# dwu4/fhe-si

Measured on AMD Instinct MI355X. Metric: homomorphic ciphertext-mults/sec (incl. relinearize) at n=2^14, logQ=512, higher is better.
Workload: dtype u32 (every transformed row is a row of 4-byte residues modulo a prime below 2^30: tensor half over primes of 30 bits, key switch over four of 30; coefficients are u64 limbs)

## Files before the change

fhe-si_amd/binding.py:

```python
from __future__ import annotations

import ctypes as C
import os
import subprocess
import sys

import numpy as np

_DIR = os.path.dirname(os.path.abspath(__file__))
_CSRC = os.path.join(_DIR, "csrc")
_SO = os.environ.get("FHESI_LIB") or os.path.join(_CSRC, "libfhesi_hip.so")

OP_ADD, OP_SUB, OP_MUL, OP_DIV, OP_SET = 0, 1, 2, 3, 4

ABI_SYMBOLS = [
    "fhesi_last_error", "fhesi_device_count", "fhesi_ctx_create", "fhesi_ctx_destroy", "fhesi_ctx_m", "fhesi_ctx_phim",
    "fhesi_ctx_nprimes", "fhesi_ctx_prime", "fhesi_ctx_zms_idx", "fhesi_ctx_phi_m", "fhesi_ctx_sync", "fhesi_ctx_stream",
    "fhesi_timer_start", "fhesi_timer_stop", "fhesi_cmod_fft", "fhesi_cmod_ifft", "fhesi_dcrt_alloc", "fhesi_dcrt_free",
    "fhesi_dcrt_copy", "fhesi_dcrt_index_set", "fhesi_dcrt_equal", "fhesi_dcrt_upload_row", "fhesi_dcrt_download_row",
    "fhesi_dcrt_device_ptr", "fhesi_dcrt_from_poly", "fhesi_dcrt_to_poly", "fhesi_dcrt_op", "fhesi_dcrt_op_scalar",
    "fhesi_dcrt_automorph", "fhesi_dcrt_add_primes", "fhesi_dcrt_remove_primes", "fhesi_dcrt_from_scrt", "fhesi_dcrt_to_scrt",
    "fhesi_rows_ntt_fwd_dev", "fhesi_rows_ntt_inv_dev", "fhesi_rows_op_dev", "fhesi_ksk_create", "fhesi_ksk_free",
    "fhesi_ksk_upload", "fhesi_ksk_device_ptr", "fhesi_ksk_bytes", "fhesi_ct_mul_relin_batch", "fhesi_ct_mul_relin_batch_dev",
    "fhesi_ct_mul_dev", "fhesi_apply_key_switch_dev", "fhesi_dev_alloc", "fhesi_dev_free", "fhesi_dev_upload", "fhesi_dev_download",
    "fhesi_dev_copy", "fhesi_prof_enable", "fhesi_prof_read",
    "fhesi_ct_add_dev", "fhesi_ct_mul_long_dev", "fhesi_rows_mul_long_dev", "fhesi_ct_automorph_dev", "fhesi_ct_automorph_key_switch_dev",
    "fhesi_ct_gather_dev", "fhesi_ct_mul_sum_relin_dev", "fhesi_encrypt_batch", "fhesi_decrypt_batch", "fhesi_dcrt_exp", "fhesi_selftest_aux32",
    "fhesi_ctx_set_option", "fhesi_ctx_get_option", "fhesi_ctx_copy_options", "fhesi_host_alloc", "fhesi_host_free", "fhesi_ksk_key_bits", "fhesi_prof_kernel_name", "fhesi_ksk_mark_dirty", "fhesi_ksk_upload_dev",
    "fhesi_dcrt_add_primes_and_scale", "fhesi_dcrt_scale_down_to_set",
    "fhesi_keyswitch_init_batch", "fhesi_ksk_download", "fhesi_comm_init_all", "fhesi_comm_from_rccl", "fhesi_comm_destroy", "fhesi_comm_rank",
    "fhesi_comm_size", "fhesi_ksk_broadcast", "fhesi_comm_broadcast_dev", "fhesi_comm_exchange", "fhesi_comm_exchange_begin", "fhesi_comm_exchange_end", "fhesi_comm_allreduce_rows", "fhesi_scrt_alloc", "fhesi_scrt_from_poly", "fhesi_scrt_to_poly", "fhesi_scrt_op_scalar", "fhesi_dcrt_assign_scrt", "fhesi_scrt_assign_dcrt",
    "fhesi_ksk_form", "fhesi_ct_add_const_dev", "fhesi_ct_mul_poly_dev",
    "fhesi_encrypt_batch_seeded", "fhesi_keyswitch_init_batch_seeded", "fhesi_dcrt_sample",
    "fhesi_abi_version", "fhesi_host_stage_release",
    "fhesi_slots_plan", "fhesi_slots_create", "fhesi_slots_free", "fhesi_slots_info", "fhesi_slots_exponents", "fhesi_slots_embed", "fhesi_slots_decode",
    "fhesi_slots_embed_dev", "fhesi_slots_decode_dev", "fhesi_encrypt_slots_batch_seeded", "fhesi_decrypt_slots_batch", "fhesi_encrypt_noise_batch_seeded",
    "fhesi_slots_plan_pow2", "fhesi_slots_create_pow2", "fhesi_slots_shape", "fhesi_slots_set_path",
]
ABI_VERSION = 7
PROF_CLASSES = {"ntt_fwd": 0, "ntt_inv": 1, "rns_reduce": 2, "tensor": 3, "crt": 4, "digits": 5, "dot": 6, "ew": 7, "ntt_fwd_digits_main": 8}


class FhesiError(RuntimeError):
    pass


def library_path() -> str:
    return _SO


def build_library(force: bool = False) -> str:
    srcs = [os.path.join(_CSRC, f) for f in os.listdir(_CSRC) if f.endswith((".hip", ".cpp", ".h", ".inc"))]
    srcs.append(os.path.join(os.path.dirname(_DIR), "include", "fhesi_hip.h"))
    stale = force or not os.path.exists(_SO) or any(os.path.getmtime(s) > os.path.getmtime(_SO) for s in srcs)
    if stale:
        subprocess.check_call(["make", "-C", _CSRC, "-j8"], stdout=subprocess.DEVNULL)
    return _SO


_lib = None
_vp, _i32, _i64, _u64 = C.c_void_p, C.c_int32, C.c_int64, C.c_uint64


def _load():
    global _lib
    if _lib is not None:
        return _lib
    if not os.path.exists(_SO):
        raise FhesiError(f"HIP extension not built: {_SO} is missing (run __graft_entry__.build())")
    if "torch" not in sys.modules and not os.environ.get("FHESI_NO_TORCH_PRELOAD"):
        try:
            import torch
        except Exception:
            pass
    lib = C.CDLL(_SO)
    lib.fhesi_last_error.restype = C.c_char_p
    have = lib.fhesi_abi_version() if hasattr(lib, "fhesi_abi_version") else None
    if have != ABI_VERSION:
        raise FhesiError(f"{_SO} has ABI revision {have}, this binding was written against {ABI_VERSION}: rebuild (make -C fhe-si_amd/csrc)")
    sig = {
        "fhesi_device_count": [_vp],
        "fhesi_ctx_create": [_vp, _i64, _i32, _vp, _vp, _i32],
        "fhesi_ctx_destroy": [_vp],
        "fhesi_ctx_prime": [_vp, _i32, _vp, _vp],
        "fhesi_ctx_zms_idx": [_vp, _vp],
        "fhesi_ctx_phi_m": [_vp, _vp],
        "fhesi_ctx_sync": [_vp],
        "fhesi_timer_start": [_vp],
        "fhesi_timer_stop": [_vp, _vp],
        "fhesi_cmod_fft": [_vp, _i32, _vp, _i32, _i64, _vp],
        "fhesi_cmod_ifft": [_vp, _i32, _vp, _vp],
        "fhesi_dcrt_alloc": [_vp, _vp, _i32, _vp],
        "fhesi_dcrt_free": [_vp],
        "fhesi_dcrt_copy": [_vp, _vp],
        "fhesi_dcrt_index_set": [_vp, _vp, _vp],
        "fhesi_dcrt_equal": [_vp, _vp, _vp],
        "fhesi_dcrt_upload_row": [_vp, _i32, _vp],
        "fhesi_dcrt_download_row": [_vp, _i32, _vp],
        "fhesi_dcrt_from_poly": [_vp, _vp, _i32, _i64],
        "fhesi_dcrt_to_poly": [_vp, _vp, _i32, _i32, _vp, _i32],
        "fhesi_dcrt_op": [_vp, _vp, _i32],
        "fhesi_dcrt_op_scalar": [_vp, _vp, _i32, _i32],
        "fhesi_dcrt_automorph": [_vp, _i64],
        "fhesi_dcrt_exp": [_vp, _i64],
        "fhesi_selftest_aux32": [_vp],
        "fhesi_dcrt_add_primes": [_vp, _vp, _i32],
        "fhesi_dcrt_remove_primes": [_vp, _vp, _i32],
        "fhesi_dcrt_from_scrt": [_vp, _vp],
        "fhesi_dcrt_to_scrt": [_vp, _vp],
        "fhesi_rows_ntt_fwd_dev": [_vp, _vp, _i64],
        "fhesi_rows_ntt_inv_dev": [_vp, _vp, _i64],
        "fhesi_rows_op_dev": [_vp, _vp, _vp, _i64, _i32],
        "fhesi_ksk_create": [_vp, _i32, _i32, _vp],
        "fhesi_ksk_free": [_vp],
        "fhesi_ksk_upload": [_vp, _vp],
        "fhesi_ct_mul_relin_batch": [_vp, _vp, _i32, _u64, _i32, _vp, _vp, _vp, _i32, _i64],
        "fhesi_ct_mul_relin_batch_dev": [_vp, _vp, _i32, _u64, _i32, _vp, _vp, _vp, _i32, _i64],
        "fhesi_ct_mul_dev": [_vp, _u64, _vp, _vp, _i32, _i64, _vp],
        "fhesi_apply_key_switch_dev": [_vp, _vp, _i32, _i32, _vp, _i64, _vp, _i32],
        "fhesi_ct_add_dev": [_vp, _i32, _vp, _vp, _i32, _i32, _i64],
        "fhesi_ct_mul_long_dev": [_vp, _i32, _vp, _i64, _i32, _i32, _i64],
        "fhesi_rows_mul_long_dev": [_vp, _vp, _i64, _i64],
        "fhesi_ct_automorph_dev": [_vp, _i64, _vp, _i32, _i32, _i64, _vp, _i32],
        "fhesi_ct_automorph_key_switch_dev": [_vp, _vp, _i32, _i32, _i64, _vp, _i32, _i64, _vp, _i32],
        "fhesi_ct_gather_dev": [_vp, _vp, _vp, _i64, _i64, _vp],
        "fhesi_ct_mul_sum_relin_dev": [_vp, _vp, _i32, _u64, _i32, _vp, _i32, _vp, _vp, _vp, _i64, _vp],
        "fhesi_encrypt_batch": [_vp, _vp, _vp, _i32, _u64, _vp, _vp, _i64, _vp, _i32],
        "fhesi_decrypt_batch": [_vp, _vp, _i32, _u64, _vp, _i32, _i64, _vp],
        "fhesi_dev_alloc": [_vp, C.c_size_t, _vp],
        "fhesi_dev_free": [_vp, _vp],
        "fhesi_dev_upload": [_vp, _vp, _vp, C.c_size_t],
        "fhesi_dev_download": [_vp, _vp, _vp, C.c_size_t],
        "fhesi_dev_copy": [_vp, _vp, _vp, C.c_size_t],
        "fhesi_prof_enable": [_vp, _i32],
        "fhesi_prof_read": [_vp, _i32, _vp, _vp, _vp],
        "fhesi_prof_kernel_name": [_vp, _i32, _vp, C.c_size_t],
        "fhesi_ctx_set_option": [_vp, C.c_char_p, _i64],
        "fhesi_ctx_get_option": [_vp, C.c_char_p, _vp],
        "fhesi_ctx_copy_options": [_vp, _vp],
        "fhesi_host_alloc": [_vp, C.c_size_t, _vp],
        "fhesi_host_free": [_vp, _vp],
        "fhesi_host_stage_release": [_vp],
        "fhesi_ksk_key_bits": [_vp, _vp, _vp],
        "fhesi_ksk_mark_dirty": [_vp],
        "fhesi_comm_init_all": [_i32, _vp, _vp],
        "fhesi_comm_from_rccl": [_vp, _vp],
        "fhesi_comm_destroy": [_vp],
        "fhesi_ksk_broadcast": [_vp, _vp, _i32],
        "fhesi_comm_broadcast_dev": [_vp, _vp, _vp, C.c_size_t, _i32],
        "fhesi_comm_exchange": [_vp, _vp, _vp, _vp],
        "fhesi_comm_exchange_begin": [_vp, _vp, _vp, _vp],
        "fhesi_comm_exchange_end": [_vp, _vp],
        "fhesi_comm_allreduce_rows": [_vp, _vp, _vp, _i64],
        "fhesi_ksk_download": [_vp, _vp],
        "fhesi_keyswitch_init_batch": [_vp, _vp, _i32, _vp, _i32, _i32, _vp, _i32, _vp],
        "fhesi_scrt_alloc": [_vp, _vp, _i32, _vp],
        "fhesi_scrt_from_poly": [_vp, _vp, _i32, _i64],
        "fhesi_scrt_to_poly": [_vp, _vp, _i32, _vp, _i32],
        "fhesi_scrt_op_scalar": [_vp, _vp, _i32, _i32],
        "fhesi_dcrt_assign_scrt": [_vp, _vp],
        "fhesi_scrt_assign_dcrt": [_vp, _vp, _vp, _i32],
        "fhesi_dcrt_add_primes_and_scale": [_vp, _vp, _i32, _u64, _vp],
        "fhesi_dcrt_scale_down_to_set": [_vp, _vp, _i32, _u64],
        "fhesi_ksk_upload_dev": [_vp, _vp],
        "fhesi_ksk_form": [_vp, _vp, _vp, _vp],
        "fhesi_encrypt_batch_seeded": [_vp, _vp, _vp, _i32, _u64, _u64, _u64, _vp, _i64, _vp, _i32],
        "fhesi_keyswitch_init_batch_seeded": [_vp, _vp, _i32, _vp, _i32, _i32, _u64, _u64, _u64],
        "fhesi_dcrt_sample": [_vp, _i32, _i64, _u64, _u64],
        "fhesi_ct_add_const_dev": [_vp, _i32, _u64, _vp, _i32, _i32, _i64, _vp, _i32],
        "fhesi_ct_mul_poly_dev": [_vp, _i32, _vp, _i32, _i32, _i64, _vp, _i32],
        "fhesi_slots_plan": [_i64, _u64, _i64, _vp, _vp, _vp, _vp, _vp],
        "fhesi_slots_create": [_vp, _u64, _i64, _vp],
        "fhesi_slots_free": [_vp],
        "fhesi_slots_info": [_vp, _vp, _vp, _vp, _vp],
        "fhesi_slots_exponents": [_vp, _vp],
        "fhesi_slots_embed": [_vp, _vp, _i64, _i32, _i64, _vp],
        "fhesi_slots_decode": [_vp, _vp, _i64, _i64, _i32, _vp],
        "fhesi_slots_embed_dev": [_vp, _vp, _i64, _i32, _i64, _vp],
        "fhesi_slots_decode_dev": [_vp, _vp, _i64, _i64, _i32, _vp],
        "fhesi_encrypt_slots_batch_seeded": [_vp, _vp, _vp, _vp, _i32, _u64, _u64, _vp, _i64, _i32, _i64, _vp, _i32],
        "fhesi_decrypt_slots_batch": [_vp, _vp, _vp, _i32, _vp, _i32, _i64, _i64, _i32, _vp],
        "fhesi_encrypt_noise_batch_seeded": [_vp, _vp, _vp, _vp, _i32, _u64, _u64, _i64, _vp, _i32],
        "fhesi_slots_plan_pow2": [_i64, _u64, _i64, _vp, _vp, _vp, _vp, _vp, _vp],
        "fhesi_slots_create_pow2": [_vp, _u64, _i64, _vp],
        "fhesi_slots_shape": [_vp, _vp, _vp, _vp],
        "fhesi_slots_set_path": [_vp, _i32],
    }
    for name, args in sig.items():
        fn = getattr(lib, name)
        fn.argtypes = args
        fn.restype = C.c_int
    for name in ("fhesi_ctx_m", "fhesi_ctx_phim"):
        getattr(lib, name).argtypes = [_vp]
        getattr(lib, name).restype = _i64
    lib.fhesi_ctx_nprimes.argtypes = [_vp]
    lib.fhesi_ctx_nprimes.restype = _i32
    for name in ("fhesi_ctx_stream", "fhesi_dcrt_device_ptr", "fhesi_ksk_device_ptr"):
        getattr(lib, name).argtypes = [_vp]
        getattr(lib, name).restype = _vp
    for name in ("fhesi_comm_rank", "fhesi_comm_size"):
        getattr(lib, name).argtypes = [_vp]
        getattr(lib, name).restype = _i32
    lib.fhesi_ksk_bytes.argtypes = [_vp]
    lib.fhesi_ksk_bytes.restype = C.c_size_t
    _lib = lib
    return lib


def _ck(rc: int):
    if rc != 0:
        raise FhesiError(_load().fhesi_last_error().decode())


def _p(a: np.ndarray):
    return a.ctypes.data_as(_vp)


class Backend:
    @staticmethod
    def lib():
        return _load()

    @staticmethod
    def device_count() -> int:
        n = _i32(0)
        _ck(_load().fhesi_device_count(C.byref(n)))
        return n.value


class DevBuf:

    def __init__(self, ctx: "Context", nbytes: int):
        self.ctx, self.nbytes = ctx, nbytes
        self.ptr = _vp()
        _ck(_load().fhesi_dev_alloc(ctx.h, nbytes, C.byref(self.ptr)))

    def upload(self, arr: np.ndarray):
        arr = np.ascontiguousarray(arr)
        assert arr.nbytes <= self.nbytes
        _ck(_load().fhesi_dev_upload(self.ctx.h, self.ptr, _p(arr), arr.nbytes))
        return self

    def download(self, shape, dtype=np.uint64) -> np.ndarray:
        out = np.empty(shape, dtype=dtype)
        assert out.nbytes <= self.nbytes
        _ck(_load().fhesi_dev_download(self.ctx.h, _p(out), self.ptr, out.nbytes))
        return out

    def free(self):
        if self.ptr:
            _load().fhesi_dev_free(self.ctx.h, self.ptr)
            self.ptr = _vp()

    def __del__(self):
        try:
            self.free()
        except Exception:
            pass


class Context:

    def __init__(self, m: int, primes, roots, device: int = 0):
        q = np.array([int(x) for x in primes], dtype=np.uint64)
        r = np.array([int(x) for x in roots], dtype=np.uint64)
        self.h = _vp()
        _ck(_load().fhesi_ctx_create(C.byref(self.h), m, len(q), _p(q), _p(r), device))
        self.m, self.primes, self.roots = m, [int(x) for x in q], [int(x) for x in r]
        self.L = len(self.primes)
        self.phim = _load().fhesi_ctx_phim(self.h)

    def close(self):
        if getattr(self, "h", None):
            _load().fhesi_ctx_destroy(self.h)
            self.h = None

    def __del__(self):
        try:
            self.close()
        except Exception:
            pass

    def sync(self):
        _ck(_load().fhesi_ctx_sync(self.h))

    def zms_idx(self) -> np.ndarray:
        out = np.zeros(self.m, dtype=np.int32)
        _ck(_load().fhesi_ctx_zms_idx(self.h, _p(out)))
        return out

    def phi_m(self) -> np.ndarray:
        out = np.zeros(self.phim + 1, dtype=np.int64)
        _ck(_load().fhesi_ctx_phi_m(self.h, _p(out)))
        return out

    def timer_start(self):
        _ck(_load().fhesi_timer_start(self.h))

    def timer_stop(self) -> float:
        ms = C.c_float(0)
        _ck(_load().fhesi_timer_stop(self.h, C.byref(ms)))
        return ms.value

    def prof_enable(self, on: bool = True):
        _ck(_load().fhesi_prof_enable(self.h, int(on)))

    def prof_read(self, cls: str):
        n, u, ms = _i64(0), C.c_double(0), C.c_double(0)
        _ck(_load().fhesi_prof_read(self.h, PROF_CLASSES[cls], C.byref(n), C.byref(u), C.byref(ms)))
        return n.value, u.value, ms.value

    def prof_kernel_name(self, cls: str) -> str:
        buf = C.create_string_buffer(512)
        _ck(_load().fhesi_prof_kernel_name(self.h, PROF_CLASSES[cls], buf, 512))
        return buf.value.decode()

    def set_option(self, name: str, value: int):
        _ck(_load().fhesi_ctx_set_option(self.h, name.encode(), int(value)))

    def get_option(self, name: str) -> int:
        v = _i64(0)
        _ck(_load().fhesi_ctx_get_option(self.h, name.encode(), C.byref(v)))
        return v.value

    def selftest_aux32(self):
        _ck(_load().fhesi_selftest_aux32(self.h))

    def dev_copy(self, dst_ptr: int, src_ptr: int, nbytes: int):
        _ck(_load().fhesi_dev_copy(self.h, _vp(dst_ptr), _vp(src_ptr), nbytes))

    def cmod_fft(self, prime: int, limbs: np.ndarray) -> np.ndarray:
        limbs = np.ascontiguousarray(limbs, dtype=np.uint64)
        y = np.zeros(self.phim, dtype=np.uint64)
        _ck(_load().fhesi_cmod_fft(self.h, prime, _p(limbs), limbs.shape[1], limbs.shape[0], _p(y)))
        return y

    def cmod_ifft(self, prime: int, y: np.ndarray) -> np.ndarray:
        y = np.ascontiguousarray(y, dtype=np.uint64)
        x = np.zeros(self.phim, dtype=np.uint64)
        _ck(_load().fhesi_cmod_ifft(self.h, prime, _p(y), _p(x)))
        return x

    def alloc(self, nbytes: int) -> DevBuf:
        return DevBuf(self, nbytes)

    def upload(self, arr: np.ndarray) -> DevBuf:
        arr = np.ascontiguousarray(arr)
        return DevBuf(self, max(arr.nbytes, 8)).upload(arr)

    def rows_ntt_fwd(self, buf: DevBuf, count: int):
        _ck(_load().fhesi_rows_ntt_fwd_dev(self.h, buf.ptr, count))

    def rows_ntt_inv(self, buf: DevBuf, count: int):
        _ck(_load().fhesi_rows_ntt_inv_dev(self.h, buf.ptr, count))

    def rows_op(self, dst: DevBuf, src: DevBuf, count: int, op: int):
        _ck(_load().fhesi_rows_op_dev(self.h, dst.ptr, src.ptr, count, op))

    def ct_mul_dev(self, p: int, a: DevBuf, b: DevBuf, nlimbs: int, count: int, tprod: DevBuf):
        _ck(_load().fhesi_ct_mul_dev(self.h, p, a.ptr, b.ptr, nlimbs, count, tprod.ptr))

    def apply_key_switch_dev(self, ksk: "KeySwitchMatrix", logQ: int, tprod: DevBuf, count: int, out: DevBuf, nlimbs: int, decomp_bytes: int = 3):
        _ck(_load().fhesi_apply_key_switch_dev(self.h, ksk.h, logQ, decomp_bytes, tprod.ptr, count, out.ptr, nlimbs))

    def encrypt_batch(self, pk0: "DoubleCRT", pk1: "DoubleCRT", logQ: int, p: int, rand: np.ndarray, msg: np.ndarray, out: DevBuf, nlimbs: int):
        rand = np.ascontiguousarray(rand, dtype=np.int64)
        msg = np.ascontiguousarray(msg, dtype=np.int64)
        assert rand.shape[0] == msg.shape[0] and rand.shape[1] == 3
        _ck(_load().fhesi_encrypt_batch(self.h, pk0.h, pk1.h, logQ, p, _p(rand), _p(msg), msg.shape[0], out.ptr, nlimbs))

    def encrypt_batch_seeded(self, pk0: "DoubleCRT", pk1: "DoubleCRT", logQ: int, p: int, seed: int, first_index: int, msg: np.ndarray, out: DevBuf, nlimbs: int):
        msg = np.ascontiguousarray(msg, dtype=np.int64)
        _ck(_load().fhesi_encrypt_batch_seeded(self.h, pk0.h, pk1.h, logQ, p, seed, first_index, _p(msg), msg.shape[0], out.ptr, nlimbs))

    def decrypt_batch(self, sk1: "DoubleCRT", logQ: int, p: int, ct: DevBuf, nlimbs: int, count: int) -> np.ndarray:
        msg = np.zeros((count, self.phim), dtype=np.int64)
        _ck(_load().fhesi_decrypt_batch(self.h, sk1.h, logQ, p, ct.ptr, nlimbs, count, _p(msg)))
        return msg

    def ct_add_dev(self, logQ: int, dst: DevBuf, src: DevBuf, nparts: int, nlimbs: int, count: int):
        _ck(_load().fhesi_ct_add_dev(self.h, logQ, dst.ptr, src.ptr, nparts, nlimbs, count))

    def ct_mul_long_dev(self, logQ: int, ct: DevBuf, l: int, nparts: int, nlimbs: int, count: int):
        _ck(_load().fhesi_ct_mul_long_dev(self.h, logQ, ct.ptr, l, nparts, nlimbs, count))

    def ct_add_const_dev(self, logQ: int, p: int, ct: DevBuf, nparts: int, nlimbs: int, count: int, poly: np.ndarray):
        poly = np.ascontiguousarray(poly, dtype=np.int64).reshape(-1, self.phim)
        _ck(_load().fhesi_ct_add_const_dev(self.h, logQ, p, ct.ptr, nparts, nlimbs, count, _p(poly), poly.shape[0]))

    def ct_mul_poly_dev(self, logQ: int, ct: DevBuf, nparts: int, nlimbs: int, count: int, poly: np.ndarray):
        poly = np.ascontiguousarray(poly, dtype=np.int64).reshape(-1, self.phim)
        _ck(_load().fhesi_ct_mul_poly_dev(self.h, logQ, ct.ptr, nparts, nlimbs, count, _p(poly), poly.shape[0]))

    def rows_mul_long_dev(self, rows: DevBuf, l: int, count: int):
        _ck(_load().fhesi_rows_mul_long_dev(self.h, rows.ptr, l, count))

    def ct_automorph_dev(self, k: int, src: DevBuf, nparts: int, nlimbs_in: int, count: int, out: DevBuf, nlimbs_out: int):
        _ck(_load().fhesi_ct_automorph_dev(self.h, k, src.ptr, nparts, nlimbs_in, count, out.ptr, nlimbs_out))

    def ct_automorph_key_switch_dev(self, ksk: "KeySwitchMatrix", logQ: int, k: int, src: DevBuf, nlimbs_in: int, count: int, out: DevBuf,
                                    nlimbs: int, decomp_bytes: int = 3):
        _ck(_load().fhesi_ct_automorph_key_switch_dev(self.h, ksk.h, logQ, decomp_bytes, k, src.ptr, nlimbs_in, count, out.ptr, nlimbs))

    def ct_gather_dev(self, pool: DevBuf, idx, words: int, out: DevBuf):
        ia = np.ascontiguousarray(idx, dtype=np.int32)
        _ck(_load().fhesi_ct_gather_dev(self.h, pool.ptr, _p(ia), len(ia), words, out.ptr))

    def ct_mul_sum_relin_dev(self, ksk: "KeySwitchMatrix", logQ: int, p: int, pool: DevBuf, nlimbs: int, a_idx, b_idx, seg, out: DevBuf,
                             decomp_bytes: int = 3):
        ia, ib = np.ascontiguousarray(a_idx, dtype=np.int32), np.ascontiguousarray(b_idx, dtype=np.int32)
        sg = np.ascontiguousarray(seg, dtype=np.int32)
        assert len(ia) == len(ib) == int(sg[-1]) and sg[0] == 0
        _ck(_load().fhesi_ct_mul_sum_relin_dev(self.h, ksk.h, logQ, p, decomp_bytes, pool.ptr, nlimbs, _p(ia), _p(ib), _p(sg), len(sg) - 1, out.ptr))

    def ct_mul_relin_dev(self, ksk: "KeySwitchMatrix", logQ: int, p: int, a: DevBuf, b: DevBuf, out: DevBuf, nlimbs: int, count: int, decomp_bytes: int = 3):
        _ck(_load().fhesi_ct_mul_relin_batch_dev(self.h, ksk.h, logQ, p, decomp_bytes, a.ptr, b.ptr, out.ptr, nlimbs, count))

    def ct_mul_relin(self, ksk: "KeySwitchMatrix", logQ: int, p: int, a: np.ndarray, b: np.ndarray, decomp_bytes: int = 3, out: np.ndarray = None) -> np.ndarray:
        a = np.ascontiguousarray(a, dtype=np.uint64)
        b = np.ascontiguousarray(b, dtype=np.uint64)
        if out is None:
            out = np.empty_like(a)
        elif out.shape != a.shape or out.dtype != np.uint64 or not out.flags.c_contiguous:
            raise ValueError("out must be a C-contiguous uint64 array of the operands' shape")
        _ck(_load().fhesi_ct_mul_relin_batch(self.h, ksk.h, logQ, p, decomp_bytes, _p(a), _p(b), _p(out), a.shape[-1], a.shape[0]))
        return out

    def host_array(self, shape, dtype=np.uint64) -> np.ndarray:
        n = int(np.prod(shape)) * np.dtype(dtype).itemsize
        ptr = _vp()
        _ck(_load().fhesi_host_alloc(self.h, n, C.byref(ptr)))
        buf = (C.c_char * max(n, 1)).from_address(ptr.value)
        arr = np.frombuffer(buf, dtype=dtype, count=int(np.prod(shape))).reshape(shape)
        import weakref
        lib, addr = _load(), ptr.value
        weakref.finalize(buf, lambda: lib.fhesi_host_free(None, C.c_void_p(addr)))
        return arr

    def release_host_staging(self):
        _ck(_load().fhesi_host_stage_release(self.h))


def slots_plan(m: int, p: int, generator: int) -> dict:
    total, usable, rho0, naux = _i64(0), _i64(0), _u64(0), _i32(0)
    _ck(_load().fhesi_slots_plan(m, p, generator, C.byref(total), C.byref(usable), C.byref(rho0), C.byref(naux), None))
    e = np.zeros(total.value, dtype=np.int32)
    _ck(_load().fhesi_slots_plan(m, p, generator, None, None, None, None, _p(e)))
    return {"total": total.value, "usable": usable.value, "rho0": rho0.value, "aux_primes": naux.value, "exps": e}


def slots_plan_pow2(m: int, p: int, generator: int) -> dict:
    total, rows, cols, rho0, path = _i64(0), _i64(0), _i64(0), _u64(0), _i32(0)
    _ck(_load().fhesi_slots_plan_pow2(m, p, generator, C.byref(total), C.byref(rows), C.byref(cols), C.byref(rho0), C.byref(path), None))
    e = np.zeros(total.value, dtype=np.int32)
    _ck(_load().fhesi_slots_plan_pow2(m, p, generator, None, None, None, None, None, _p(e)))
    return {"total": total.value, "rows": rows.value, "cols": cols.value, "rho0": rho0.value, "path": path.value, "exps": e}


class SlotSpace:

    def __init__(self, ctx: "Context", p: int, generator: int, _two_rows: bool = False):
        self.ctx, self.p, self.generator = ctx, p, generator
        self.h = _vp()
        _ck((_load().fhesi_slots_create_pow2 if _two_rows else _load().fhesi_slots_create)(ctx.h, p, generator, C.byref(self.h)))
        total, usable, rho0, naux = _i64(0), _i64(0), _u64(0), _i32(0)
        _ck(_load().fhesi_slots_info(self.h, C.byref(total), C.byref(usable), C.byref(rho0), C.byref(naux)))
        self.total, self.usable, self.rho0, self.aux_primes = total.value, usable.value, rho0.value, naux.value
        self._shape()

    @classmethod
    def pow2(cls, ctx: "Context", p: int, generator: int) -> "SlotSpace":
        return cls(ctx, p, generator, _two_rows=True)

    def _shape(self):
        rows, cols, path = _i64(0), _i64(0), _i32(0)
        _ck(_load().fhesi_slots_shape(self.h, C.byref(rows), C.byref(cols), C.byref(path)))
        self.rows, self.cols, self.path = rows.value, cols.value, path.value

    def set_path(self, path: int):
        _ck(_load().fhesi_slots_set_path(self.h, path))
# ... 363 lines not shown
```

fhe-si_amd/csrc/capi_ctx.hip:

```cpp
#include "capi_common.h"

int ws_reserve(fhesi_ctx* ctx, int slot, size_t bytes, void** out) {
  if (ctx->ws_bytes[slot] < bytes) {
    if (ctx->ws[slot]) { HIP_TRY(hipStreamSynchronize(ctx->stream)); HIP_TRY(hipFree(ctx->ws[slot])); ctx->ws[slot] = nullptr; ctx->ws_bytes[slot] = 0; }
    size_t want = bytes + (bytes >> 3) + 4096;
    if (hipMalloc(&ctx->ws[slot], want) != hipSuccess) {
      (void)hipGetLastError();
      ctx->ws[slot] = nullptr;
      if (hipMalloc(&ctx->ws[slot], bytes) != hipSuccess) {
        (void)hipGetLastError();
        ctx->ws[slot] = nullptr;
        ctx->ws_oom = true;
        FHESI_FAIL("workspace slot %d: hipMalloc of %zu bytes failed", slot, bytes);
      }
      want = bytes;
    }
    ctx->ws_bytes[slot] = want;
  }
  *out = ctx->ws[slot];
  if (ctx->ws_poison && bytes) HIP_TRY(hipMemsetAsync(ctx->ws[slot], 0xA5, bytes, ctx->stream));
  return 0;
}

int upload_idx(fhesi_ctx* ctx, const std::vector<int>& idx, int** d_out) {
  bool identity = (int)idx.size() == ctx->L;
  for (size_t i = 0; identity && i < idx.size(); ++i) identity = idx[i] == (int)i;
  if (identity) { *d_out = nullptr; return 0; }
  void* p;
  FHESI_TRY(ws_reserve(ctx, 3, idx.size() * sizeof(int) + 64, &p));
  HIP_TRY(hipMemcpyAsync(p, idx.data(), idx.size() * sizeof(int), hipMemcpyHostToDevice, ctx->stream));
  HIP_TRY(hipStreamSynchronize(ctx->stream));
  *d_out = (int*)p;
  return 0;
}

extern "C" int32_t fhesi_abi_version(void) { return FHESI_ABI_VERSION; }
extern "C" int fhesi_device_count(int32_t* count) {
  int c = 0;
  hipError_t e = hipGetDeviceCount(&c);
  if (e != hipSuccess) { *count = 0; FHESI_FAIL("hipGetDeviceCount failed: %s", hipGetErrorString(e)); }
  *count = c;
  return 0;
}

static void build_tile_order(const std::vector<Shoup2>& tw, int logn, std::vector<Shoup2>& twt) {
  const i64 n = 1ll << logn;
  const int R = logn - 10;
  twt.assign(n, Shoup2{0, 0});
  for (int i = 0; i < 32; ++i) twt[i] = tw[i];
  for (int u = 0; u < 5; ++u)
    for (int x = 0; x < (1 << u); ++x)
      for (int p1 = 0; p1 < 32; ++p1) twt[32 + ((1 << u) - 1 + x) * 32 + p1] = tw[(1 << (5 + u)) + (p1 << u) + x];
  for (int u = 0; u < R; ++u)
    for (int x = 0; x < (1 << u); ++x)
      for (int jl = 0; jl < 1024; ++jl) twt[1024 + (i64)((1 << u) - 1 + x) * 1024 + jl] = tw[(1 << (10 + u)) + ((i64)hm::brv(jl, 10) << u) + x];
}
static void to_q63(std::vector<Shoup2>& t, u64 q) {
  for (auto& e : t) e.wp = hm::shoup63(e.w, q);
}

thread_local bool g_fhesi_internal_ctx = false;

struct OptDesc { const char* name; const char* env; size_t off; bool wide; };
static const OptDesc kOptions[] = {
  {"ks_direct", "FHESI_KS_DIRECT", offsetof(CtxOptions, ks_direct), false},
  {"ks_residues", "FHESI_KS_RESIDUES", offsetof(CtxOptions, ks_residues), false},
  {"ks_aux60", "FHESI_KS_AUX60", offsetof(CtxOptions, ks_aux60), false},
  {"crt_exact", "FHESI_CRT_EXACT", offsetof(CtxOptions, crt_exact), false},
  {"crt_skip_cleanup", "FHESI_CRT_SKIP_CLEANUP", offsetof(CtxOptions, crt_skip_cleanup), false},
  {"lanes", "FHESI_LANES", offsetof(CtxOptions, lanes), false},
  {"stagger", "FHESI_STAGGER", offsetof(CtxOptions, stagger), false},
  {"batch_chunk", "FHESI_BATCH_CHUNK", offsetof(CtxOptions, batch_chunk), true},
  {"wave_operands", "FHESI_WAVE_OPERANDS", offsetof(CtxOptions, wave_operands), true},
  {"wave_single", "FHESI_WAVE_SINGLE", offsetof(CtxOptions, wave_single), false},
  {"tensor32", "FHESI_TENSOR32", offsetof(CtxOptions, tensor32), false},
  {"tensor_bits", "FHESI_TENSOR_BITS", offsetof(CtxOptions, tensor_bits), false},
  {"dot32_k4", "FHESI_DOT32_K4", offsetof(CtxOptions, dot32_k4), false},
  {"parts_words", "FHESI_PARTS_WORDS", offsetof(CtxOptions, parts_words), false},
  {"automorph_rows", "FHESI_AUTOMORPH_ROWS", offsetof(CtxOptions, automorph_rows), false},
  {"ks_long_keys", "FHESI_KS_LONG_KEYS", offsetof(CtxOptions, ks_long_keys), false},
  {"host_chunk", "FHESI_HOST_CHUNK", offsetof(CtxOptions, host_chunk), true},
  {"host_threads", "FHESI_HOST_THREADS", offsetof(CtxOptions, host_threads), false},
};
static void opt_store(CtxOptions* o, const OptDesc& d, long long v) {
  if (d.wide) *(long long*)((char*)o + d.off) = v; else *(int*)((char*)o + d.off) = (int)v;
}
static long long opt_load(const CtxOptions* o, const OptDesc& d) {
  return d.wide ? *(const long long*)((const char*)o + d.off) : (long long)*(const int*)((const char*)o + d.off);
}
extern "C" int fhesi_ctx_set_option(fhesi_ctx* c, const char* name, int64_t value) {
  if (!c || !name) FHESI_FAIL("set_option: null argument");
  for (const OptDesc& d : kOptions)
    if (!strcmp(d.name, name)) { opt_store(&c->opt, d, value); return 0; }
  FHESI_FAIL("set_option: unknown option '%s'", name);
}
extern "C" int fhesi_ctx_get_option(const fhesi_ctx* c, const char* name, int64_t* value) {
  if (!c || !name || !value) FHESI_FAIL("get_option: null argument");
  for (const OptDesc& d : kOptions)
    if (!strcmp(d.name, name)) { *value = opt_load(&c->opt, d); return 0; }
  FHESI_FAIL("get_option: unknown option '%s'", name);
}
extern "C" int fhesi_ctx_copy_options(fhesi_ctx* dst, const fhesi_ctx* src) {
  if (!dst || !src) FHESI_FAIL("copy_options: null argument");
  dst->opt = src->opt;
  return 0;
}

extern "C" int fhesi_ctx_create(fhesi_ctx** out, int64_t m, int32_t nprimes, const uint64_t* q, const uint64_t* root, int32_t device) {
  if (!out) FHESI_FAIL("null output pointer");
  *out = nullptr;
  if (m < 2 || m > (g_fhesi_internal_ctx ? (1 << 23) : (1 << 20))) FHESI_FAIL("FHEcontext: m undefined or larger than 2^20");
  if (nprimes < 1 || nprimes > 64) FHESI_FAIL("FHEcontext: number of primes %d outside [1,64]", nprimes);
  for (int i = 0; i < nprimes; ++i) {
    if (q[i] >= (1ull << 60)) FHESI_FAIL("AddPrime: prime %d does not fit 60 bits (NTL_SP_NBITS)", i);
    if (!hm::is_prime(q[i])) FHESI_FAIL("AddPrime: modulus %d (%llu) is not prime", i, (unsigned long long)q[i]);
    if (q[i] % (2 * (u64)m) != 1) FHESI_FAIL("AddPrime: prime %d (%llu) is not 1 mod 2m", i, (unsigned long long)q[i]);
    for (int j = 0; j < i; ++j)
      if (q[j] == q[i]) FHESI_FAIL("AddPrime: prime %d (%llu) already in chain", i, (unsigned long long)q[i]);
    if (!hm::is_primitive_2m_root(root[i], m, q[i])) FHESI_FAIL("Cmodulus: root %d is not a primitive 2m-th root of unity mod q", i);
  }
  int ndev = 0;
  HIP_TRY(hipGetDeviceCount(&ndev));
  if (device < 0 || device >= ndev) FHESI_FAIL("device %d not available (%d visible)", device, ndev);
  HIP_TRY(hipSetDevice(device));

  fhesi_ctx* c = new fhesi_ctx();
  for (const OptDesc& d : kOptions)
    if (const char* e = getenv(d.env)) opt_store(&c->opt, d, atoll(e));
  c->device = device;
  c->m = m;
  c->L = nprimes;
  c->q.assign(q, q + nprimes);
  c->root.assign(root, root + nprimes);
  c->zms_idx = hm::zms_idx(m, &c->phim);
  c->phi = hm::cyclotomic(m);
  c->pow2 = (m & (m - 1)) == 0 && m >= 4;
  c->logn = c->pow2 ? hm::ilog2_ceil(c->phim) : 0;
  if (!c->pow2 && 2 * c->phim - 1 <= 64 * kAux32N) {
    if (m % 2 == 0 && (m / 2) % 2 == 1 && hm::is_prime((u64)(m / 2))) c->lin_q = m / 2;
    else if (m % 2 == 1 && m > 2 && hm::is_prime((u64)m)) { c->lin_q = m; c->lin_prime = true; }
    if (c->lin_q) {
      c->lin_lg = 14;
      while (((i64)1 << c->lin_lg) < 2 * c->phim - 1) ++c->lin_lg;
      if (const char* e = getenv("FHESI_LIN_LG")) { const int want = atoi(e); if (want > c->lin_lg && want <= 20) c->lin_lg = want; }
    }
  }
  if (const char* e = getenv("FHESI_WS_POISON")) c->ws_poison = atoi(e) != 0;
  HIP_TRY(hipStreamCreateWithFlags(&c->stream, hipStreamNonBlocking));
  HIP_TRY(hipStreamCreateWithFlags(&c->lane_stream, hipStreamNonBlocking));
  HIP_TRY(hipEventCreateWithFlags(&c->ev_fork, hipEventDisableTiming));
  HIP_TRY(hipEventCreateWithFlags(&c->ev_join, hipEventDisableTiming));
  HIP_TRY(hipEventCreateWithFlags(&c->ev_mid, hipEventDisableTiming));
  HIP_TRY(hipEventCreate(&c->ev0));
  HIP_TRY(hipEventCreate(&c->ev1));

  const i64 n = c->phim;
  c->pc.resize(nprimes);
  for (int i = 0; i < nprimes; ++i) {
    PrimeConst& pc = c->pc[i];
    const u64 Q = q[i];
    pc.q = Q;
    pc.two_q = 2 * Q;
    int k = 64 - __builtin_clzll(Q);
    pc.bar_k = (u32)k;
    pc.bar_mu = (u64)((((u128)1) << (2 * k)) / Q);
    pc.r64 = (u64)(((u128)1 << 64) % Q);
    pc.r64_sh = hm::shoup(pc.r64, Q);
    pc.one_sh = hm::shoup(1, Q);
    pc.q_tile = Q >= (1ull << 48) ? Q : Q * (((1ull << 60) - 1) / Q);
    pc.one_q63 = hm::shoup63(1, pc.q_tile);
    {
      const u64 qh = pc.q_tile >> 32;
      const int b = 64 - __builtin_clzll(qh);
      pc.norm_m = (u32)((((u128)1) << (31 + b)) / (qh + 1));
    }
    if (Q < (1ull << 48)) c->has_small_prime = true; else c->n_big_primes++;
    pc.ninv = pc.ninv_sh = pc.ninv_w = pc.ninv_w_sh = 0;
  }
  if (c->pow2) {
    const int lg = c->logn;
    std::vector<Shoup2> twf((size_t)nprimes * n), twi((size_t)nprimes * n);
    for (int i = 0; i < nprimes; ++i) {
      const u64 Q = q[i];
      const u64 psi = hm::mulmod(root[i], root[i], Q), ipsi = hm::invmod(psi, Q);
      std::vector<u64> pw(n), ipw(n);
      pw[0] = ipw[0] = 1;
      for (i64 e = 1; e < n; ++e) { pw[e] = hm::mulmod(pw[e - 1], psi, Q); ipw[e] = hm::mulmod(ipw[e - 1], ipsi, Q); }
      for (i64 j = 0; j < n; ++j) {
        const u64 e = hm::brv((u64)j, lg);
        twf[(size_t)i * n + j] = {pw[e], hm::shoup(pw[e], Q)};
        twi[(size_t)i * n + j] = {ipw[e], hm::shoup(ipw[e], Q)};
      }
      PrimeConst& pc = c->pc[i];
      pc.ninv = hm::invmod((u64)n % Q, Q);
      pc.ninv_sh = hm::shoup(pc.ninv, Q);
      pc.ninv_w = hm::mulmod(pc.ninv, n > 1 ? twi[(size_t)i * n + 1].w : 1, Q);
      pc.ninv_w_sh = hm::shoup(pc.ninv_w, Q);
      pc.ninv_q63 = hm::shoup63(pc.ninv, pc.q_tile);
      pc.ninv_w_q63 = hm::shoup63(pc.ninv_w, pc.q_tile);
    }
    const size_t tb = twf.size() * sizeof(Shoup2);
    HIP_TRY(hipMalloc(&c->d_tw_fwd, tb));
    HIP_TRY(hipMalloc(&c->d_tw_inv, tb));
    HIP_TRY(hipMemcpy(c->d_tw_fwd, twf.data(), tb, hipMemcpyHostToDevice));
    HIP_TRY(hipMemcpy(c->d_tw_inv, twi.data(), tb, hipMemcpyHostToDevice));
    if (lg >= 11 && lg <= 14) {
      std::vector<Shoup2> all_f((size_t)nprimes * n), all_i((size_t)nprimes * n), one, tmp;
      for (int i = 0; i < nprimes; ++i) {
        one.assign(twf.begin() + (size_t)i * n, twf.begin() + (size_t)(i + 1) * n);
        build_tile_order(one, lg, tmp);
        to_q63(tmp, c->pc[i].q_tile);
        std::copy(tmp.begin(), tmp.end(), all_f.begin() + (size_t)i * n);
        one.assign(twi.begin() + (size_t)i * n, twi.begin() + (size_t)(i + 1) * n);
        build_tile_order(one, lg, tmp);
        to_q63(tmp, c->pc[i].q_tile);
        std::copy(tmp.begin(), tmp.end(), all_i.begin() + (size_t)i * n);
      }
      HIP_TRY(hipMalloc(&c->d_twt_fwd, tb));
      HIP_TRY(hipMalloc(&c->d_twt_inv, tb));
      HIP_TRY(hipMemcpy(c->d_twt_fwd, all_f.data(), tb, hipMemcpyHostToDevice));
      HIP_TRY(hipMemcpy(c->d_twt_inv, all_i.data(), tb, hipMemcpyHostToDevice));
    }
    if (lg >= 15 && lg <= 17) {
      const int s0 = lg - 14, nsub = 1 << s0;
      const i64 n1 = 1 << 14;
      std::vector<Shoup2> all_f((size_t)nprimes * n1), all_i((size_t)nprimes * n), all_fs((size_t)nprimes * n), tail((size_t)nprimes * n, Shoup2{0, 0}),
          fold((size_t)nprimes * nsub), one(n1), tmp;
      for (int i = 0; i < nprimes; ++i) {
        const u64 Q = q[i];
// ... 187 lines not shown
```

fhe-si_amd/csrc/fhesi_internal.h:

```cpp
#pragma once
#include <hip/hip_runtime.h>
#include <cstdint>
#include <cstdio>
#include <map>
#include <string>
#include <atomic>
#include <vector>

typedef uint64_t u64;
typedef int64_t i64;
typedef unsigned int u32;
typedef unsigned __int128 u128;

void fhesi_set_error(const char* fmt, ...);
#define FHESI_FAIL(...) do { fhesi_set_error(__VA_ARGS__); return 1; } while (0)
#define HIP_TRY(expr) do { hipError_t e__ = (expr); if (e__ != hipSuccess) { fhesi_set_error("%s failed: %s (%s:%d)", #expr, hipGetErrorString(e__), __FILE__, __LINE__); return 1; } } while (0)
#define FHESI_OP_SET_ 4
#define FHESI_WS_SLOTS 13
#define FHESI_TRY(expr) do { int r__ = (expr); if (r__) return r__; } while (0)

struct PrimeConst {
  u64 q;
  u64 two_q;
  u64 bar_mu;
  u32 bar_k;
  u32 norm_m;
  u64 one_sh;
  u64 ninv, ninv_sh;
  u64 ninv_w, ninv_w_sh;
  u64 r64, r64_sh;
  u64 one_q63;
  u64 ninv_q63, ninv_w_q63;
  u64 q_tile;
};

struct Shoup2 { u64 w, wp; };

struct CrtTables {
  int nidx = 0, W = 0;
  std::vector<int> idx;
  u64* d_blob = nullptr;
  int* d_idx = nullptr;
  Shoup2* d_pow64 = nullptr;
  Shoup2* d_pinv = nullptr;
  u64* d_P = nullptr;
  u64* d_halfP = nullptr;
  u64* d_M = nullptr;
  u64* d_cinv = nullptr;
  mutable unsigned char* d_flags = nullptr;
  mutable size_t flags_cap = 0;
};

struct BluesteinTables;
struct fhesi_aux32;

enum { PROF_NTT_FWD = 0, PROF_NTT_INV = 1, PROF_RNS = 2, PROF_TENSOR = 3, PROF_CRT = 4, PROF_DIGITS = 5, PROF_DOT = 6, PROF_EW = 7, PROF_NTT_FWD_DIGITS_MAIN = 8, PROF_NCLASS = 9 };
struct ProfRec { int cls; double units; hipEvent_t e0, e1; };

struct CtxOptions {
  long long host_chunk = 0;
  int host_threads = 0;
  int ks_long_keys = 0;
  int ks_direct = 0;
  int ks_residues = 0;
  int ks_aux60 = 0;
  int crt_exact = 0;
  int crt_skip_cleanup = 0;
  int lanes = 1;
  int stagger = 0;
  long long batch_chunk = 0;
  long long wave_operands = 0;
  int wave_single = 1;
  int automorph_rows = 0;
  int tensor32 = 1;
  int tensor_bits = 30;
  int dot32_k4 = 1;
  int parts_words = 1;
};

struct fhesi_ctx {
  CtxOptions opt;
  int live_handles = 0;
  int device = 0;
  hipStream_t stream = nullptr;
  hipEvent_t ev0 = nullptr, ev1 = nullptr;
  i64 m = 0, phim = 0;
  int L = 0;
  bool pow2 = false;
  int n_big_primes = 0;
  bool has_small_prime = false;
  int logn = 0;
  i64 lin_q = 0;
  bool lin_prime = false;
  int lin_lg = 0;
  std::vector<u64> q, root;
  std::vector<int> zms_idx;
  std::vector<i64> phi;
  std::vector<PrimeConst> pc;
  PrimeConst* d_pc = nullptr;
  Shoup2* d_tw_fwd = nullptr;
  Shoup2* d_tw_inv = nullptr;
  Shoup2* d_twt_fwd = nullptr;
  Shoup2* d_twt_inv = nullptr;
  Shoup2* d_twt_fwd_sub = nullptr;
  Shoup2* d_head_tw = nullptr;
  Shoup2* d_tail_fwd = nullptr;
  Shoup2* d_sub_fold = nullptr;
  int* d_zms_idx = nullptr;
  int* d_zms_list = nullptr;
  BluesteinTables* blue = nullptr;
  fhesi_aux32* aux32 = nullptr;
  struct fhesi_tensor32* tensor32 = nullptr;
  std::map<std::vector<long long>, std::pair<int, std::vector<uint32_t>>> t32_memo;
  std::map<std::vector<int>, CrtTables*> crt_cache;
  std::map<int, Shoup2*> pow64_cache;
  std::map<std::vector<u64>, u64*> scalar_cache;
  hipStream_t lane_stream = nullptr;
  void* lane_ws[FHESI_WS_SLOTS] = {};
  size_t lane_ws_bytes[FHESI_WS_SLOTS] = {};
  hipEvent_t ev_fork = nullptr, ev_join = nullptr, ev_mid = nullptr;
  bool ws_poison = false;
  bool ws_oom = false;
  const int* op_idx = nullptr;
  long long op_idx_n = 0, op_idx_done = 0;
  bool mark_mid = false;
  struct HostStage* host_stage = nullptr;
  bool prof_on = false;
  std::vector<ProfRec> prof;
  const void* prof_fn[16] = {};
  void* ws[FHESI_WS_SLOTS] = {};
  size_t ws_bytes[FHESI_WS_SLOTS] = {};
};

struct fhesi_dcrt {
  fhesi_ctx* ctx = nullptr;
  std::vector<int> idx;
  u64* d_rows = nullptr;
  bool coeff_form = false;
};

struct fhesi_ksk {
  fhesi_ctx* ctx = nullptr;
  int ncomp = 0, ndigits = 0;
  u64* d_rows = nullptr;
  size_t bytes = 0;
  u64* d_aux = nullptr;
  size_t aux_bytes = 0;
  u64* d_aux_consts = nullptr;
  bool aux_valid = false, aux_suborder = false;
  int aux_mode = 0;
  int last_form = -1;
  int aux_rows = 0, aux_limb_bits = 0, aux_logQ = 0;
  bool aux_centred = false;
  int aux_key_bits = 0;
  int aux_long_opt = 0;
  bool aux32 = false;
  i64 aux_fold = 0;
  u64* d_limb_consts = nullptr;
};
struct KsLimbPlan { int W = 0, LQ = 0, B = 0, NLB = 0, mbits = 0; bool a32 = false; };
bool ks_limb_plan(const fhesi_ctx* ctx, const CrtTables* t, int ncol, int digit_bits, int logQ, KsLimbPlan* plan, const u32* p32 );
int launch_ks_recombine(fhesi_ctx* ctx, const CrtTables* t, const fhesi_ksk* k, const u64* d_o , i64 npolys, u64* d_out, int nl_out, bool tail_pending = false);
bool ks_recombine_takes_tail(const fhesi_ctx* ctx, const CrtTables* t, const fhesi_ksk* k);
int aux32_tail_consts(fhesi_ctx* ctx, uint32_t (*tw)[2], uint32_t (*twp)[2]);
void aux32_free(fhesi_ctx* ctx);
void tensor32_free(fhesi_ctx* ctx);
void host_stage_free(fhesi_ctx* ctx);
bool tensor32_applies(const fhesi_ctx* ctx, u64 p, int nlimbs, int logQ);
int launch_tensor32(fhesi_ctx* ctx, u64 p, const u64* d_a, const u64* d_b, int nlimbs, int logQ, i64 count, u64* d_parts , bool parts_wm = false);
bool tensor32_sum_applies(const fhesi_ctx* ctx, u64 p, int nlimbs, int logQ, i64 gmax);
int tensor32_sum_begin(fhesi_ctx* ctx, u64 p, int nlimbs, int logQ, i64 gmax);
size_t tensor32_sum_bytes(const fhesi_ctx* ctx, i64 ngroups);
int tensor32_sum_pass(fhesi_ctx* ctx, const u64* d_ops, i64 nua, i64 nub, const int* d_slot_a, const int* d_slot_b, const int* d_seg, i64 ng, i64 nterms, bool accumulate, void* d_sum);
int tensor32_sum_finish(fhesi_ctx* ctx, void* d_sum, i64 ng, u64* d_parts, bool parts_wm = false);
const u32* aux32_primes(fhesi_ctx* ctx);
int launch_ntt32_fwd(fhesi_ctx* ctx, u32* d_rows, i64 count, int nslots, int a0);
int launch_ntt32_inv(fhesi_ctx* ctx, u32* d_rows, i64 count, int nslots, int a0, bool mont , bool tail = true );
constexpr i64 kDigitSubCt = 64;
int launch_ntt32_fwd_digits(fhesi_ctx* ctx, const u64* d_parts, int nl, int digit_bits, int nd, i64 npolys, u32* d_out ,
                            i64 sub_units , bool wm = false );
int ks32_build(fhesi_ctx* ctx, fhesi_ksk* k, const u64* d_kint, int W, int B, int NLB, void* d_tmp , bool centred = false );
int ks32_key_bits(fhesi_ctx* ctx, const u64* d_kint , i64 count, int W, int* nbits );
bool aux32_applies(const fhesi_ctx* ctx);
i64 aux32_row_len(const fhesi_ctx* ctx);
static const i64 kAux32N = 1 << 14;
int launch_dot32(fhesi_ctx* ctx, fhesi_ksk* k, const u32* d_dig , int ncol, i64 count, u32* d_out , bool* mont );
enum { KS_MODE_DIRECT = 0, KS_MODE_LIMB32 = 1 , KS_MODE_LIMB60 = 2 , KS_MODE_RESIDUE60 = 3  };
int ksaux_mode(fhesi_ctx* ctx, const CrtTables* t, int ncol, int digit_bits, int logQ);
int ksaux_build(fhesi_ctx* ctx, fhesi_ksk* k, int digit_bits, int logQ, int mode);
int launch_dot_aux(fhesi_ctx* ctx, const fhesi_ksk* k, const u64* d_dig , int ncol, i64 count, u64* d_out );
int launch_aux_crt(fhesi_ctx* ctx, const fhesi_ksk* k, const u64* d_o , u64* d_dst , i64 nrows);

int ws_reserve(fhesi_ctx* ctx, int slot, size_t bytes, void** out);

struct ProfScope {
  fhesi_ctx* c; int idx = -1;
  ProfScope(fhesi_ctx* ctx, int cls, double units) : c(ctx) {
    if (!c->prof_on) return;
    ProfRec r; r.cls = cls; r.units = units;
    if (hipEventCreate(&r.e0) != hipSuccess || hipEventCreate(&r.e1) != hipSuccess) return;
    hipEventRecord(r.e0, c->stream);
    c->prof.push_back(r); idx = (int)c->prof.size() - 1;
  }
  ~ProfScope() { if (idx >= 0) hipEventRecord(c->prof[idx].e1, c->stream); }
};

static inline void prof_kernel(fhesi_ctx* ctx, int cls, const void* host_stub) { if (ctx->prof_on) ctx->prof_fn[cls] = host_stub; }
#define PROF_KERNEL(ctx, cls, ...) prof_kernel((ctx), (cls), (const void*)&__VA_ARGS__)

namespace hm {
u64 mulmod(u64 a, u64 b, u64 q);
u64 powmod(u64 a, u64 e, u64 q);
u64 invmod(u64 a, u64 q);
bool is_prime(u64 n);
u64 shoup(u64 w, u64 q);
u64 shoup63(u64 w, u64 q);
u64 brv(u64 x, int bits);
int ilog2_ceil(i64 n);
std::vector<int> zms_idx(i64 m, i64* phim);
std::vector<i64> cyclotomic(i64 m);
std::vector<i64> cyclotomic_cofactor(i64 m);
bool is_primitive_2m_root(u64 root, i64 m, u64 q);
u64 bn_mod(const u64* limbs, int nlimbs, u64 q);
std::vector<u64> bn_mul_small(const std::vector<u64>& a, u64 b);
struct SlotSpace {
  i64 m = 0, phim = 0, usable = 0;
  u64 p = 0, g = 0, rho0 = 0;
  int kind = 0;
  i64 q = 0, s = 0;
  int naux = 1;
  std::vector<int> exps, slot_of_exp;
  int rows = 1;
  bool direct = false;
};
const char* slot_space(i64 m, u64 p, i64 g, SlotSpace* out);
const char* slot_space_pow2(i64 m, u64 p, i64 g, SlotSpace* out);
}

struct fhesi_slots {
  fhesi_ctx* ctx = nullptr;
  hm::SlotSpace S;
  fhesi_ctx* aux = nullptr;
  i64 N = 0;
  u64 P[2] = {0, 0};
  Shoup2* d_pre = nullptr;
  Shoup2* d_post = nullptr;
  u64* d_bhat = nullptr;
  int* d_exps = nullptr;
  int* d_slot_of_exp = nullptr;
  bool orderfree = false;
  struct Tw { u32 w, wp; };
  Tw* d_p2tw = nullptr;
  u32* d_p2pos = nullptr;
  Tw p2ninv = {0, 0}, p2ninv_w1 = {0, 0};
};
int slots_build(fhesi_slots* s);
void slots_release(fhesi_slots* s);
int slots_pow2_build(fhesi_slots* s);
int slots_pow2_run(fhesi_slots* s, bool embed, const i64* d_in, i64* d_out, i64 nvals, i64 take, i64 count);
int slots_embed_rows(fhesi_slots* s, const i64* d_vals, i64 nvals, bool only_usable, i64 count, i64* d_msg);
int slots_decode_rows(fhesi_slots* s, const i64* d_msg, i64 count, i64 nvals, bool only_usable, i64* d_vals);
int slots_noise_rows(fhesi_slots* s, u64 seed, u64 first, i64 count, i64* d_vals );

int launch_ntt_fwd(fhesi_ctx* ctx, u64* d_rows, i64 count, int nslots, const int* d_prime_of_slot, bool bitrev = true);
int launch_ntt_inv(fhesi_ctx* ctx, u64* d_rows, i64 count, int nslots, const int* d_prime_of_slot, bool bitrev = true);
bool ntt_orderfree_two_pass(const fhesi_ctx* ctx);
int launch_ntt_fwd_head(fhesi_ctx* ctx, u64* d_rows, i64 count, int nslots, const int* d_prime_of_slot);
int launch_ntt_sub(fhesi_ctx* ctx, bool fwd, u64* d_rows, i64 count, int nslots, const int* d_prime_of_slot);
int launch_ntt_inv_tail_inplace(fhesi_ctx* ctx, u64* d_rows, i64 count, int nslots, const int* d_prime_of_slot);
int launch_ntt_fwd_digits(fhesi_ctx* ctx, const u64* d_parts_limbmajor, int nl, int logQ, int digit_bits, int nd, i64 npolys,
                          u64* d_out_rows , int slot0 = 0, int nslot = 0 , int layout_slots = 0 );

int launch_ew_op(fhesi_ctx* ctx, u64* d_dst, const u64* d_src, i64 count, int nslots, const int* d_prime_of_slot, int op);
int launch_ew_exp(fhesi_ctx* ctx, u64* d_dst, const u64* d_exps , i64 count, int nslots, const int* d_prime_of_slot, unsigned* d_zero_flag );
int launch_ew_scalar(fhesi_ctx* ctx, u64* d_dst, const u64* d_scalars , i64 count, int nslots, const int* d_prime_of_slot, int op);
int launch_tensor2x2(fhesi_ctx* ctx, const u64* d_a , const u64* d_b , u64* d_t , i64 count);
int launch_dot_accum(fhesi_ctx* ctx, const u64* d_key , const u64* d_dig , int ncol, i64 count,
                     u64* d_out , int slot0 = 0, int nslot = 0 , bool dig_suborder = false);
bool ntt_digits_suborder(const fhesi_ctx* ctx, int digit_bits);
int launch_tensor_sum(fhesi_ctx* ctx, const u64* d_ca, const u64* d_cb, const int* d_slot_a, const int* d_slot_b, const int* d_seg, i64 ngroups, bool accumulate,
                      u64* d_out , double nproducts);
int launch_scrt_const(fhesi_ctx* ctx, u64* d_rows, const u64* d_scalars , int nslots, const int* d_prime_of_slot, int op );
int launch_automorph(fhesi_ctx* ctx, u64* d_dst, const u64* d_src, i64 nrows, i64 k);
int launch_rows_equal(fhesi_ctx* ctx, const u64* a, const u64* b, i64 nwords, int* equal);

int launch_ct_add(fhesi_ctx* ctx, u64* d_dst, const u64* d_src, i64 ncoeffs, int nl, int logQ);
int launch_ct_mul_long(fhesi_ctx* ctx, u64* d_ct, i64 ncoeffs, int nl, int logQ, i64 l);
int launch_sample_encrypt(fhesi_ctx* ctx, i64* d_rnd , i64 count, u64 seed, u64 first);
int launch_sample_keygen(fhesi_ctx* ctx, u64* d_a, i64* d_err, i64 ncol, int nl, int logQ, u64 seed, u64 pub_seed, u64 first);
int launch_sample_poly(fhesi_ctx* ctx, i64* d_poly , int kind , i64 param, u64 seed, u64 obj);
int launch_ct_add_const(fhesi_ctx* ctx, u64* d_ct , const i64* d_poly , int npoly, int nparts, int nl, int logQ, u64 p, i64 count);
int launch_ct_automorph_parts(fhesi_ctx* ctx, const u64* d_in , int nl_in, i64 npolys, i64 kk, int logQ, u64* d_parts , int nlq);
int launch_gather(fhesi_ctx* ctx, const u64* d_pool, const int* d_idx, i64 count, i64 words, u64* d_out);
int launch_segment_sum(fhesi_ctx* ctx, const u64* d_in, const int* d_seg, i64 ngroups, int ncomp, u64* d_out);
int launch_encrypt_combine(fhesi_ctx* ctx, const u64* d_rows , const u64* d_pk , i64 count, u64* d_out );
int launch_add_scaled_msg(fhesi_ctx* ctx, u64* d_ct, const i64* d_msg, const u64* d_delta, i64 count, int nl, int logQ);
int launch_decrypt_dot(fhesi_ctx* ctx, const u64* d_rows , const u64* d_t , i64 count, u64* d_out );
int launch_decrypt_round(fhesi_ctx* ctx, const u64* d_z, i64 total, int nw, int logQ, u64 p, i64* d_out);

int launch_rows_mul_bcast(fhesi_ctx* ctx, u64* d_dst , const u64* d_a , const u64* d_t , i64 ncols);
int launch_keygen_combine(fhesi_ctx* ctx, const u64* d_bcoef, int wb, const u64* d_scoef, int ws, const i64* d_err, i64 ncols, int nd, int digit_bits, int nl, int logQ, u64* d_out);

int get_crt_tables(fhesi_ctx* ctx, const std::vector<int>& idx, CrtTables** out);
int launch_rns_reduce(fhesi_ctx* ctx, const u64* d_limbs, int nlimbs, i64 ncoeffs, i64 count, int npoly, const u64* scalar_mul,
                      u64* d_rows, int nslots, const int* d_prime_of_slot);
int launch_crt(fhesi_ctx* ctx, const CrtTables* t, const u64* d_rows, int nslots_layout, const int* d_slot_of, i64 npolys, int mode, int positive,
               int logQ, u64* d_out, int nl_out);
int launch_modswitch_delta(fhesi_ctx* ctx, const u64* d_delta, int W, const u64* consts_host , u64 p, u64 u, u64* d_e);
int launch_digits(fhesi_ctx* ctx, const u64* d_parts, int nl, int logQ, int digit_bits, int nd, i64 npolys, u64* d_rows, u64 only_below_q = 0);

int bluestein_init(fhesi_ctx* ctx);
void bluestein_destroy(fhesi_ctx* ctx);
int launch_bluestein_fwd(fhesi_ctx* ctx, u64* d_rows, i64 count, int nslots, const int* prime_of_slot_host);
int launch_bluestein_inv(fhesi_ctx* ctx, u64* d_rows, i64 count, int nslots, const int* prime_of_slot_host);

#if defined(__HIPCC__)
__device__ __forceinline__ u64 d_mulhi(u64 a, u64 b) { return __umul64hi(a, b); }

__device__ __forceinline__ u64 d_shoup_lazy(u64 y, u64 w, u64 wp, u64 q) {
  u64 Q = d_mulhi(y, wp);
  return y * w - Q * q;
}
// ... 23 lines not shown
```

fhe-si_amd/csrc/kernels_tensor32.hip:

```cpp
#include "fhesi_internal.h"
#include "ntt32_core.inc"
#include <cmath>

struct T32Config {
  u64 lift = 0;
  int nl = 0, logQ = 0, NP = 0, R = 28, WT = 0;
  bool generic = false;
  T32Primes pr;
  u32* d_rns = nullptr;
  Tw32* d_cinv = nullptr;
  u32* d_inv57 = nullptr;
  u32* d_Mw = nullptr;
  ~T32Config() { hipFree(d_rns); hipFree(d_cinv); hipFree(d_inv57); hipFree(d_Mw); }
};
struct fhesi_tensor32 {
  int S = 0;
  int bits = 30;
  std::vector<u32> primes;
  std::vector<Tw32> head, tail;
  std::vector<Tw32> head1;
  Tw32* d_fwd = nullptr;
  Tw32* d_inv = nullptr;
  Tw32* d_ht = nullptr;
  u32* d_p = nullptr;
  Tw32* d_hs = nullptr;
  std::vector<T32Config*> cfgs;
  T32Config* cur = nullptr;
};

void tensor32_free(fhesi_ctx* ctx) {
  fhesi_tensor32* x = ctx->tensor32;
  if (!x) return;
  for (T32Config* c : x->cfgs) delete c;
  hipFree(x->d_fwd); hipFree(x->d_inv); hipFree(x->d_ht); hipFree(x->d_p); hipFree(x->d_hs);
  delete x;
  ctx->tensor32 = nullptr;
}

typedef std::vector<u64> Big;
static Big big_mul_small(const Big& a, u64 b) { return hm::bn_mul_small(a, b); }
static u64 big_mod_small(const Big& a, u64 q) { u128 r = 0; for (size_t i = a.size(); i-- > 0;) r = ((r << 64) | a[i]) % q; return (u64)r; }
static u32 big_word(const Big& a, int l, int R) {
  const int bit = R * l, w = bit >> 6, o = bit & 63;
  u64 v = (size_t)w < a.size() ? a[w] >> o : 0;
  if (o + R > 64 && (size_t)w + 1 < a.size()) v |= a[w + 1] << (64 - o);
  return (u32)(v & (((u64)1 << R) - 1));
}

static constexpr int T32_WT_512 = 38, T32_R_512 = 28;
static constexpr int T32_WT_1024 = 82, T32_R_1024 = 26;
static constexpr int T32_GEN_NW = 24, T32_GEN_NWX = 40;

struct T32Plan { int NP = 0; bool generic = false; };
static T32Plan t32_plan_search(const fhesi_ctx* ctx, u64 p, int nlimbs, int logQ, i64 gmax, std::vector<u32>* primes);
static T32Plan t32_plan(const fhesi_ctx* ctx, u64 p, int nlimbs, int logQ, i64 gmax, std::vector<u32>* primes) {
  int gbits = 0;
  while (((i64)1 << gbits) < gmax) ++gbits;
  auto& memo = const_cast<fhesi_ctx*>(ctx)->t32_memo;
  const std::vector<long long> key{(long long)p, nlimbs, logQ, gbits, ctx->opt.tensor32, ctx->opt.tensor_bits};
  auto it = memo.find(key);
  if (it == memo.end()) {
    std::vector<u32> pr;
    const T32Plan pl = t32_plan_search(ctx, p, nlimbs, logQ, gmax, &pr);
    it = memo.emplace(key, std::make_pair(pl.NP * 2 + (pl.generic ? 1 : 0), std::move(pr))).first;
  }
  if (primes) *primes = it->second.second;
  T32Plan pl;
  pl.NP = it->second.first >> 1; pl.generic = it->second.first & 1;
  return pl;
}
static T32Plan t32_plan_search(const fhesi_ctx* ctx, u64 p, int nlimbs, int logQ, i64 gmax, std::vector<u32>* primes) {
  T32Plan pl;
  if (!ctx->opt.tensor32 || p < 2 || nlimbs < 1 || nlimbs > 16 || 64 * nlimbs < logQ || gmax < 1) return pl;
  const bool lin = ctx->lin_q != 0;
  if (!lin && !(ctx->pow2 && (ctx->logn == A32_LOGN || ctx->logn == A32_LOGN + 1))) return pl;
  const int lg = lin ? ctx->lin_lg : ctx->logn;
  const bool compiled = !lin && (logQ == 512 || logQ == 1024);
  if (!compiled && (logQ < 64 || logQ > 512)) return pl;
  int pbits = 0, gbits = 0, cbits = 0;
  while (pbits < 64 && (p >> pbits)) ++pbits;
  while (((i64)1 << gbits) < gmax) ++gbits;
  while (((i64)1 << cbits) < ctx->phim) ++cbits;
  const double TB = 2.0 * (logQ - 1) + pbits + cbits + 1 + gbits + (lin ? 2 : 0);
  double chain = 0;
  for (int i = 0; i < ctx->L; ++i) chain += std::log2((double)ctx->q[i]);
  if (chain < TB + 1.5) return pl;
  const int maxp = (compiled && logQ == 1024) ? T32_MAXP : 62;
  const int pb = ctx->opt.tensor_bits == 29 ? 29 : 30;
  const double margin = pb == 29 ? 1.5 : 3.5;
  double have = 0;
  int np = 0;
  for (u64 k = ((u64)1 << (pb - 1 - lg)) - 1; k > ((u64)1 << (pb - 2 - lg)) && have < TB + margin; --k) {
    const u64 cand = (k << (lg + 1)) + 1;
    if (cand > ((u64)1 << pb) - ((u64)1 << 15) + 1 || !hm::is_prime(cand)) continue;
    if (np == maxp) return pl;
    if (primes) primes->push_back((u32)cand);
    have += std::log2((double)cand);
    ++np;
  }
  if (have < TB + margin) return pl;
  const double room = compiled ? (logQ == 512 ? (double)T32_R_512 * T32_WT_512 : (double)T32_R_1024 * T32_WT_1024) : 28.0 * ((have + 8) / 28 + 2);
  if (have > room - 8) return pl;
  pl.NP = np;
  pl.generic = !compiled;
  return pl;
}
bool tensor32_applies(const fhesi_ctx* ctx, u64 p, int nlimbs, int logQ) { return t32_plan(ctx, p, nlimbs, logQ, 1, nullptr).NP > 0; }
bool tensor32_sum_applies(const fhesi_ctx* ctx, u64 p, int nlimbs, int logQ, i64 gmax) {
  return t32_plan(ctx, p, nlimbs, logQ, gmax, nullptr).NP > 0;
}

static int t32_ring(fhesi_ctx* ctx, const std::vector<u32>& primes) {
  fhesi_tensor32* x = ctx->tensor32;
  const int pb = !primes.empty() && primes[0] < (1u << 29) ? 29 : 30;
  if (x && x->bits != pb) {
    HIP_TRY(hipStreamSynchronize(ctx->stream));
    if (ctx->lane_stream) HIP_TRY(hipStreamSynchronize(ctx->lane_stream));
    tensor32_free(ctx);
    x = nullptr;
  }
  if (!x) { x = new fhesi_tensor32(); x->S = (ctx->lin_q ? ctx->lin_lg : ctx->logn) - A32_LOGN; x->bits = pb; ctx->tensor32 = x; }
  if (x->primes.size() >= primes.size()) return 0;
  HIP_TRY(hipStreamSynchronize(ctx->stream));
  if (ctx->lane_stream) HIP_TRY(hipStreamSynchronize(ctx->lane_stream));
  const int S = x->S, lg = A32_LOGN + S, NP = (int)primes.size(), NS = 1 << S;
  if (S < 0 || S > 6) FHESI_FAIL("tensor32: rows of 2^%d", lg);
  const int HSN = A32_HSN(S);
  std::vector<Tw32> hs(S >= 3 ? (size_t)NP * 2 * HSN : 0, Tw32{0, 0});
  const i64 n = (i64)A32_N << S;
  const size_t per_prime = (size_t)A32_N << S;
  std::vector<Tw32> hf((size_t)NP * per_prime, Tw32{0, 0}), hi((size_t)NP * per_prime, Tw32{0, 0}), ff((size_t)n), fi((size_t)n), ht((size_t)NP * A32_HT, Tw32{0, 0});
  x->head.assign(NP, Tw32{0, 0}); x->tail.assign(NP, Tw32{0, 0}); x->head1.assign((size_t)NP * 2, Tw32{0, 0});
  for (int a = 0; a < NP; ++a) {
    const u64 p = primes[a];
    u64 psi = 0;
    for (u64 gq = 2; gq < 1000 && !psi; ++gq) {
      const u64 cand = hm::powmod(gq, (p - 1) / (2 * (u64)n), p);
      if (hm::powmod(cand, (u64)n, p) == p - 1) psi = cand;
    }
    if (!psi) FHESI_FAIL("tensor32: no 2n-th root");
    const u64 ipsi = hm::invmod(psi, p);
    auto tw = [&](u64 w) { return Tw32{(u32)w, (u32)((w << 32) / p)}; };
    auto fwd_form = [](Tw32 t) { return Tw32{0u - t.w, t.wp}; };
    a32_bitrev_powers(p, psi, lg, ff); a32_bitrev_powers(p, ipsi, lg, fi);
    if (!S) {
      std::transform(ff.begin(), ff.end(), hf.begin() + (size_t)a * per_prime, fwd_form);
      std::copy(fi.begin(), fi.end(), hi.begin() + (size_t)a * per_prime);
    } else {
      for (int h = 0; h < NS; ++h)
        for (u64 mp = 1; mp < (u64)A32_N; mp <<= 1)
          for (u64 ip = 0; ip < mp; ++ip) {
            hf[((size_t)a * NS + h) * A32_N + mp + ip] = fwd_form(ff[(mp << S) + h * mp + ip]);
            hi[((size_t)a * NS + h) * A32_N + mp + ip] = fi[(mp << S) + h * mp + ip];
          }
      x->head[a] = ff[1]; x->tail[a] = fi[1];
      if (S == 2) {
        x->head1[(size_t)a * 2] = ff[2]; x->head1[(size_t)a * 2 + 1] = ff[3];
        const u64 inv2 = (p + 1) / 2;
        Tw32* c = &ht[(size_t)a * A32_HT];
        c[0] = ff[1]; c[1] = ff[2]; c[2] = ff[3];
        c[4] = tw(inv2); c[5] = tw(hm::mulmod(fi[2].w, inv2, p)); c[6] = tw(hm::mulmod(fi[3].w, inv2, p)); c[7] = tw(hm::mulmod(fi[1].w, inv2, p));
      }
      if (S >= 3) {
        Tw32* f = &hs[(size_t)a * 2 * HSN];
        Tw32* b = f + HSN;
        for (int idx = 1; idx < NS; ++idx) { f[idx] = ff[idx]; b[idx] = fi[idx]; }
        const u64 c = hm::invmod((u64)NS % p, p), cm = hm::mulmod(c, ((u64)1 << 32) % p, p);
        b[NS] = tw(c); b[NS + 1] = tw(hm::mulmod(fi[1].w, c, p)); b[NS + 2] = tw(cm); b[NS + 3] = tw(hm::mulmod(fi[1].w, cm, p));
      }
    }
  }
  for (size_t a = 0; a < primes.size(); ++a) {
    const u64 p = primes[a], ninv = hm::invmod((u64)A32_N % p, p);
    for (int h = 0; h < NS; ++h) {
      Tw32* t0 = &hi[(a * NS + h) * A32_N];
      const u64 wn = hm::mulmod(t0[1].w, ninv, p);
      t0[0] = Tw32{(u32)ninv, (u32)((ninv << 32) / p)}; t0[1] = Tw32{(u32)wn, (u32)((wn << 32) / p)};
    }
  }
  hipFree(x->d_fwd); hipFree(x->d_inv); hipFree(x->d_ht); hipFree(x->d_p); hipFree(x->d_hs);
  x->d_fwd = x->d_inv = x->d_ht = x->d_hs = nullptr; x->d_p = nullptr;
  if (S >= 2) {
    if (hipMalloc(&x->d_ht, ht.size() * sizeof(Tw32)) != hipSuccess || hipMalloc(&x->d_p, (size_t)NP * sizeof(u32)) != hipSuccess) FHESI_FAIL("tensor32: hipMalloc failed");
    HIP_TRY(hipMemcpy(x->d_ht, ht.data(), ht.size() * sizeof(Tw32), hipMemcpyHostToDevice));
    HIP_TRY(hipMemcpy(x->d_p, primes.data(), (size_t)NP * sizeof(u32), hipMemcpyHostToDevice));
  }
  if (S >= 3) {
    if (hipMalloc(&x->d_hs, hs.size() * sizeof(Tw32)) != hipSuccess) FHESI_FAIL("tensor32: hipMalloc failed");
    HIP_TRY(hipMemcpy(x->d_hs, hs.data(), hs.size() * sizeof(Tw32), hipMemcpyHostToDevice));
  }
  a32_permute_phase_c(hf); a32_permute_phase_c(hi);
  if (hipMalloc(&x->d_fwd, hf.size() * sizeof(Tw32)) != hipSuccess || hipMalloc(&x->d_inv, hi.size() * sizeof(Tw32)) != hipSuccess) FHESI_FAIL("tensor32: hipMalloc failed");
  HIP_TRY(hipMemcpy(x->d_fwd, hf.data(), hf.size() * sizeof(Tw32), hipMemcpyHostToDevice));
  HIP_TRY(hipMemcpy(x->d_inv, hi.data(), hi.size() * sizeof(Tw32), hipMemcpyHostToDevice));
  x->primes = primes;
  return 0;
}

static int t32_config(fhesi_ctx* ctx, u64 lift, int nlimbs, int logQ, i64 gmax, T32Config** out) {
  std::vector<u32> primes;
  const T32Plan pl = t32_plan(ctx, lift, nlimbs, logQ, gmax, &primes);
  if (!pl.NP) FHESI_FAIL("tensor32: shape not supported");
  FHESI_TRY(t32_ring(ctx, primes));
  fhesi_tensor32* x = ctx->tensor32;
  for (T32Config* c : x->cfgs)
    if (c->lift == lift && c->nl == nlimbs && c->logQ == logQ && c->NP == pl.NP && c->generic == pl.generic) { *out = c; return 0; }
  const int NP = pl.NP, S = x->S;
  double have = 0;
  for (int a = 0; a < NP; ++a) have += std::log2((double)primes[a]);
  T32Config* c = new T32Config();
  c->lift = lift; c->nl = nlimbs; c->logQ = logQ; c->NP = NP; c->generic = pl.generic;
  c->R = pl.generic ? 28 : (logQ == 512 ? T32_R_512 : T32_R_1024);
  c->WT = pl.generic ? (int)((have + 8) / 28) + 2 : (logQ == 512 ? T32_WT_512 : T32_WT_1024);
  const int R = c->R, WT = c->WT, stride = (2 * nlimbs + 8 + 7) & ~7;
  std::vector<u32> rns((size_t)2 * NP * stride);
  for (int a = 0; a < NP; ++a) {
    const u64 p = primes[a];
    const u64 ninv = hm::invmod((u64)A32_N % p, p);
    c->pr.p[a] = (u32)p;
    c->pr.ninv[a] = (u32)ninv;
    c->pr.ninv_p[a] = (u32)((ninv << 32) / p);
    c->pr.mu61[a] = (u32)(((u64)1 << (32 + t32_shift((u32)p))) / p);
    for (int cls = 0; cls < 2; ++cls) {
      u32* e = &rns[((size_t)cls * NP + a) * stride];
      const u64 b32 = ((u64)1 << 32) % p;
      u64 cur = cls == 0 ? lift % p : 1;
      for (int k = 0; k < 2 * nlimbs; ++k) { e[k] = (u32)cur; cur = hm::mulmod(cur, b32, p); }
      e[2 * nlimbs] = (u32)((p - cur) % p);
      e[2 * nlimbs + 1] = (u32)b32;
      e[2 * nlimbs + 2] = c->pr.mu61[a];
      e[2 * nlimbs + 3] = (u32)p;
      e[2 * nlimbs + 4] = S == 2 ? x->head1[(size_t)a * 2].w : (S ? x->head[a].w : 0);
      e[2 * nlimbs + 5] = S == 2 ? x->head1[(size_t)a * 2].wp : (S ? x->head[a].wp : 0);
      e[2 * nlimbs + 6] = S == 2 ? x->head1[(size_t)a * 2 + 1].w : 0;
      e[2 * nlimbs + 7] = S == 2 ? x->head1[(size_t)a * 2 + 1].wp : 0;
    }
  }
  Big M{1};
  for (int a = 0; a < NP; ++a) M = big_mul_small(M, primes[a]);
  std::vector<Tw32> cinv((size_t)NP * 2);
  std::vector<u32> inv57(NP), Mw((size_t)(NP + 1) * WT + 64);
  for (int a = 0; a < NP; ++a) {
    Big Mi{1};
    for (int b = 0; b < NP; ++b) if (b != a) Mi = big_mul_small(Mi, primes[b]);
    const u64 p = primes[a];
    const u64 ci = hm::invmod(big_mod_small(Mi, p), p);
    auto tw = [&](u64 w) { return Tw32{(u32)w, (u32)((w << 32) / p)}; };
    if (S != 1) cinv[(size_t)a * 2] = cinv[(size_t)a * 2 + 1] = tw(ci);
    else {
      const u64 inv2 = (p + 1) / 2;
      cinv[(size_t)a * 2] = tw(hm::mulmod(ci, inv2, p));
      cinv[(size_t)a * 2 + 1] = tw(hm::mulmod(ci, hm::mulmod(x->tail[a].w, inv2, p), p));
    }
    inv57[a] = (u32)(((u64)1 << 57) / p);
    for (int l = 0; l < WT; ++l) Mw[(size_t)a * WT + l] = big_word(Mi, l, R);
  }
  {
    Big N(M);
    N.resize((R * WT + 63) / 64 + 1, 0);
    u64 carry = 1;
    for (auto& w : N) { const u64 v = ~w + carry; carry = (carry && v == 0) ? 1 : 0; w = v; }
    for (int l = 0; l < WT; ++l) Mw[(size_t)NP * WT + l] = big_word(N, l, R);
  }
  auto up = [&](void** d, const void* h, size_t bytes) -> bool {
    return hipMalloc(d, bytes) == hipSuccess && hipMemcpy(*d, h, bytes, hipMemcpyHostToDevice) == hipSuccess;
  };
  if (!up((void**)&c->d_rns, rns.data(), rns.size() * 4) || !up((void**)&c->d_cinv, cinv.data(), cinv.size() * sizeof(Tw32)) ||
      !up((void**)&c->d_inv57, inv57.data(), inv57.size() * 4) || !up((void**)&c->d_Mw, Mw.data(), Mw.size() * 4)) {
    delete c;
    FHESI_FAIL("tensor32: table upload failed");
  }
  x->cfgs.push_back(c);
  *out = c;
  return 0;
}

__device__ __forceinline__ u64 mad64s(u32 a, u32 b_uniform, u64 c) {
  u64 r, carry;
  asm("v_mad_u64_u32 %0, %1, %2, %3, %4" : "=v"(r), "=s"(carry) : "v"(a), "s"(b_uniform), "v"(c));
  return r;
}
template <int NL>
__device__ __forceinline__ u32 rns32_one(const u32 (&x)[2 * NL], u32 neg, const u32* __restrict__ t) {
  const u32 r32 = t[2 * NL + 1], mu = t[2 * NL + 2], p = t[2 * NL + 3];
  u64 acc = 0;
  int room = 4;
#pragma unroll
  for (int k = 0; k < 2 * NL; ++k) {
    if (room == 0) { acc = mad64s((u32)(acc >> 32), r32, (u64)(u32)acc); room = 3; }
    acc = mad64s(x[k], t[k], acc);
    --room;
  }
  acc = mad64s(neg, t[2 * NL], acc);
  acc = mad64s((u32)(acc >> 32), r32, (u64)(u32)acc);
  const u32 sh = t32_shift(p);
  if (r32 >= (1u << (sh - 1))) acc = mad64s((u32)(acc >> 32), r32, (u64)(u32)acc);
  const u32 q = __umulhi((u32)(acc >> sh), mu);
  return (u32)acc - q * p;
}
template <int NL, int HEAD, bool PAIRED>
__global__ void __launch_bounds__(256) rns32_reduce_kernel(const u64* __restrict__ a, const u64* __restrict__ b, i64 na2, i64 n_src, i64 nrow, u32* __restrict__ rows, int NP,
                                                            const u32* __restrict__ tab, const int* __restrict__ idx_a = nullptr, const int* __restrict__ idx_b = nullptr, int dup = 0) {
  __shared__ __attribute__((aligned(16))) u64 sl[NL * 256];
  const i64 poly = blockIdx.y;
  int cls;
  const u64* __restrict__ src;
  if (PAIRED) {
    const i64 ct = poly >> 2; const int jp = (int)(poly & 3); cls = jp >> 1;
    const i64 cs = idx_a ? (i64)(cls ? idx_b : idx_a)[ct] : ct;
    src = (cls ? b : a) + (cs * 2 + (jp & 1)) * n_src * NL;
  }
  else { cls = poly >= na2; src = cls ? b + (poly - na2) * n_src * NL : a + poly * n_src * NL; }
  const i64 j0 = (i64)blockIdx.x * 256;
  const int tid = threadIdx.x;
  u32* __restrict__ o = rows + poly * NP * nrow + j0 + tid;
  const int i_first = (int)((i64)blockIdx.z * NP / gridDim.z), i_last = (int)((i64)(blockIdx.z + 1) * NP / gridDim.z);
  if (j0 >= n_src) {
    for (int i = i_first; i < i_last; ++i) {
      o[(i64)i * nrow] = 0;
      if (dup || HEAD != 0) o[(i64)i * nrow + A32_N] = 0;
      if constexpr (HEAD == 2) { o[(i64)i * nrow + 2 * A32_N] = 0; o[(i64)i * nrow + 3 * A32_N] = 0; }
    }
    return;
  }
  const i64 avail = (n_src - j0) * NL;
  u32 x[2 * NL], x1[HEAD != 0 ? 2 * NL : 1];
  const u64* __restrict__ sblk = src + j0 * NL;
  if (avail >= 256 * NL) {
#pragma unroll
    for (int it = 0; it < NL; ++it) {
      const int e = it * 256 + tid;
      sl[(e % NL) * 256 + e / NL] = sblk[e];
    }
  } else {
#pragma unroll
    for (int it = 0; it < NL; ++it) {
      const int e = it * 256 + tid;
      sl[(e % NL) * 256 + e / NL] = e < avail ? sblk[e] : 0;
    }
  }
  __syncthreads();
#pragma unroll
  for (int k = 0; k < NL; ++k) { const u64 v = sl[k * 256 + tid]; x[2 * k] = (u32)v; x[2 * k + 1] = (u32)(v >> 32); }
  if constexpr (HEAD != 0) {
    __syncthreads();
    const i64 avail1 = HEAD == 2 ? (n_src - (j0 + A32_N)) * NL : (i64)256 * NL;
#pragma unroll
    for (int it = 0; it < NL; ++it) {
      const int e = it * 256 + tid;
      sl[(e % NL) * 256 + e / NL] = e < avail1 ? src[(j0 + A32_N) * NL + e] : 0;
    }
    __syncthreads();
#pragma unroll
    for (int k = 0; k < NL; ++k) { const u64 v = sl[k * 256 + tid]; x1[2 * k] = (u32)v; x1[2 * k + 1] = (u32)(v >> 32); }
  }
  const u32 neg = x[2 * NL - 1] >> 31;
  u32 neg1 = 0;
  if constexpr (HEAD != 0) neg1 = x1[2 * NL - 1] >> 31;
  constexpr int STRIDE = (2 * NL + 8 + 7) & ~7;
#pragma unroll 2
  for (int i = i_first; i < i_last; ++i) {
    const u32* __restrict__ t = tab + ((i64)cls * NP + i) * STRIDE;
    const u32 r0 = rns32_one<NL>(x, neg, t);
    if constexpr (HEAD == 0) {
      __builtin_nontemporal_store(r0, &o[(i64)i * nrow]);
      if (dup) __builtin_nontemporal_store(r0, &o[(i64)i * nrow + A32_N]);
    }
    else {
      const u32 p = t[2 * NL + 3], twop = 2 * p;
      const u32 r1 = rns32_one<NL>(x1, neg1, t);
      const u32 X = r0 >= twop ? r0 - twop : r0;
      const u32 T = mul_lazy32(r1, Tw32{t[2 * NL + 4], t[2 * NL + 5]}, p);
      o[(i64)i * nrow] = X + T;
      o[(i64)i * nrow + A32_N] = X + twop - T;
      if constexpr (HEAD == 2) {
        const u32 Tb = mul_lazy32(r1, Tw32{t[2 * NL + 6], t[2 * NL + 7]}, p);
        o[(i64)i * nrow + 2 * A32_N] = X + Tb;
        o[(i64)i * nrow + 3 * A32_N] = X + twop - Tb;
      }
    }
  }
}

__global__ void __launch_bounds__(256) tensor_sum32_kernel(const u32* __restrict__ ra, const u32* __restrict__ rb, const int* __restrict__ slot_a,
                                                           const int* __restrict__ slot_b, const int* __restrict__ seg, int accumulate, u32* __restrict__ out,
                                                           i64 nrow, int NP, T32Primes pr) {
  const int g = blockIdx.z, l = blockIdx.y;
  const u32 p = pr.p[l], mu = pr.mu61[l], twop = 2 * p, sh = t32_shift(p);
  const u32 r32 = (u32)((((u64)1) << 32) % p);
  const i64 rs = (i64)NP * nrow;
  const i64 j = (i64)blockIdx.x * blockDim.x + threadIdx.x;
  u32* o0 = out + (((i64)g * 3 + 0) * NP + l) * nrow + j;
  const int t0 = seg[g], t1 = seg[g + 1];
  auto red = [&](u64 v) -> u32 {
    v = (u64)(u32)(v >> 32) * r32 + (u32)v;
    v = (u64)(u32)(v >> 32) * r32 + (u32)v;
    const u32 q = __umulhi((u32)(v >> sh), mu);
    const u32 r = (u32)v - q * p;
    return r >= twop ? r - twop : r;
  };
  u64 r0 = 0, r1 = 0, r2 = 0;
  if (accumulate) { r0 = o0[0]; r1 = o0[rs]; r2 = o0[2 * rs]; }
  int t = t0;
  for (; t + 4 <= t1; t += 4) {
    u32 a0[4], a1[4], b0[4], b1[4];
#pragma unroll
    for (int u = 0; u < 4; ++u) {
      const u32* a = ra + (((i64)slot_a[t + u] * 2) * NP + l) * nrow + j;
      const u32* b = rb + (((i64)slot_b[t + u] * 2) * NP + l) * nrow + j;
      a0[u] = a[0]; a1[u] = a[rs]; b0[u] = b[0]; b1[u] = b[rs];
    }
#pragma unroll
    for (int u = 0; u < 4; ++u) {
      r0 += (u64)a0[u] * b0[u];
      r1 += (u64)a0[u] * b1[u] + (u64)a1[u] * b0[u];
      r2 += (u64)a1[u] * b1[u];
    }
    r0 = red(r0); r1 = red(r1); r2 = red(r2);
  }
  for (; t < t1; ++t) {
    const u32* a = ra + (((i64)slot_a[t] * 2) * NP + l) * nrow + j;
    const u32* b = rb + (((i64)slot_b[t] * 2) * NP + l) * nrow + j;
    const u32 a0 = a[0], a1 = a[rs], b0 = b[0], b1 = b[rs];
    r0 += (u64)a0 * b0;
// ... 57 lines not shown
  int undecided = 0;
  if (!EXACT) undecided = (G == 0x7fffffffffffffffull) ? 1 : 0;
  u64 c = G >> 63;
  u64* __restrict__ o = out + poly * (LQ / 64) * n + j;
  u32* __restrict__ o32 = reinterpret_cast<u32*>(out) + poly * (LQ / 32) * n + j;
#pragma unroll
  for (int i = 0; i < LQ / 64; ++i) {
    u64 v = limb(LQ + 64 * i);
    v += c;
    c = (c && v == 0) ? 1 : 0;
    if (wm) { o32[(i64)(2 * i) * n] = (u32)v; o32[(i64)(2 * i + 1) * n] = (u32)(v >> 32); }
    else o[(i64)i * n] = v;
  }
  if (!EXACT) {
    const int any = __syncthreads_or(undecided);
    if (threadIdx.x == 0) flags[wg] = any ? 1 : 0;
  }
}

template <int NWMAX, bool EXACT, int S, int FOLD>
__global__ void __launch_bounds__(128) crt32_scale_generic_kernel(const u32* __restrict__ rows, i64 nrow, i64 n_out, i64 fold_off, int NP, int LQ, int J0, int NW, int WT,
                                                                   T32Primes pr, const Tw32* __restrict__ cinv, const u32* __restrict__ inv57, const u32* __restrict__ Mw,
                                                                   u64* __restrict__ out, unsigned char* __restrict__ flags, int wm) {
  constexpr int R = 28;
  __shared__ u32 xs[NWMAX * 128];
  const size_t wg = (size_t)blockIdx.y * gridDim.x + blockIdx.x;
  if (EXACT && !flags[wg]) return;
  const i64 poly = blockIdx.y;
  const i64 j = (i64)blockIdx.x * blockDim.x + threadIdx.x;
  const bool active = j < n_out;
  const u32* __restrict__ src = rows + poly * NP * nrow;
  u64 acc[NWMAX];
#pragma unroll
  for (int l = 0; l < NWMAX; ++l) acc[l] = 0;
  u32 fsum = 0;
  if (active) {
    constexpr int NT = FOLD ? 3 : 1;
    u32 eb[NT];
    bool up[NT], ok[NT], neg[NT];
    {
      const i64 e[3] = {j, j + fold_off, fold_off - 1};
      const bool ng[3] = {false, FOLD == 1, FOLD == 2 || !(j & 1)};
#pragma unroll
      for (int k = 0; k < NT; ++k) {
        ok[k] = e[k] < nrow;
        const u32 idx = ok[k] ? (u32)e[k] : 0u;
        up[k] = S && idx >= (u32)A32_N;
        eb[k] = S ? (idx & (u32)(A32_N - 1)) : idx;
        neg[k] = ng[k];
      }
    }
#pragma unroll 2
    for (int i = 0; i < NP; ++i) {
      const u32 p = pr.p[i], twop = 2 * p;
      const u32* __restrict__ ri = src + (i64)i * nrow;
      u32 y;
      if (S) {
        u32 A[NT], B[NT];
#pragma unroll
        for (int k = 0; k < NT; ++k) { A[k] = ri[eb[k]]; B[k] = ri[eb[k] + A32_N]; }
        auto red2 = [&](u32 v) -> u32 { return min(v, v - twop); };
        u32 lo = 0, hi = 0;
#pragma unroll
        for (int k = 0; k < NT; ++k) {
          const u32 t = up[k] ? A[k] + p - B[k] : A[k] + B[k];
          const u32 v = ok[k] ? (neg[k] ? twop - t : t) : 0u;
          if (k == 0) { lo = up[0] ? 0u : v; hi = up[0] ? v : 0u; }
          else { lo = red2(lo + (up[k] ? 0u : v)); hi = red2(hi + (up[k] ? v : 0u)); }
        }
        if (NT == 1) { lo = red2(lo); hi = red2(hi); }
        y = mul_lazy32(lo, cinv[2 * i], p) + mul_lazy32(hi, cinv[2 * i + 1], p);
        y = min(y, y - twop);
        y = min(y, y - p);
      } else {
        u32 r = ri[eb[0]];
        if (FOLD) {
          const u32 b = ok[1] ? ri[eb[1]] : 0u, c = ri[eb[2]];
          if (FOLD == 1) r = r + (p - b) + (neg[2] ? p - c : c);
          else r = r + b + (p - c);
        }
        y = mul_lazy32(r, cinv[2 * i], p);
        y = y >= p ? y - p : y;
      }
      fsum += __umulhi(y, inv57[i]);
      const u32* __restrict__ Mi = Mw + (i64)i * WT + J0;
#pragma unroll
      for (int l = 0; l < NWMAX; ++l) acc[l] += (u64)y * Mi[l];
    }
    const u32 kappa = (fsum + (1u << 24)) >> 25;
    const u32* __restrict__ Nm = Mw + (i64)NP * WT + J0;
    u64 carry = 0;
#pragma unroll
    for (int l = 0; l < NWMAX; ++l)
      if (l < NW) {
        const u64 v = acc[l] + (u64)kappa * Nm[l] + carry;
        xs[l * 128 + threadIdx.x] = (u32)(v & 0xfffffffull);
        carry = v >> R;
      }
  }
  int undecided = 0;
  if (active) {
    auto word = [&](int l) -> u64 { return (l >= 0 && l < NW) ? (u64)xs[l * 128 + threadIdx.x] : 0ull; };
    auto limb = [&](int B) -> u64 {
      const int l0 = B / R - J0, o = B % R;
      u64 v = word(l0) >> o;
      v |= word(l0 + 1) << (R - o);
      v |= word(l0 + 2) << (2 * R - o);
      if (3 * R - o < 64) v |= word(l0 + 3) << (3 * R - o);
      return v;
    };
    const u64 G = limb(LQ - 64);
    if (!EXACT) undecided = (G == 0x7fffffffffffffffull) ? 1 : 0;
    u64 c = G >> 63;
    const int nlq = (LQ + 63) >> 6;
    u64* __restrict__ o = out + poly * nlq * n_out + j;
    u32* __restrict__ o32 = reinterpret_cast<u32*>(out) + poly * (2 * nlq) * n_out + j;
    for (int i = 0; i < nlq; ++i) {
      u64 v = limb(LQ + 64 * i);
      v += c;
      c = (c && v == 0) ? 1 : 0;
      const int bits_left = LQ - 64 * i;
      if (bits_left < 64) v &= ((u64)1 << bits_left) - 1;
      if (wm) { o32[(i64)(2 * i) * n_out] = (u32)v; o32[(i64)(2 * i + 1) * n_out] = (u32)(v >> 32); }
      else o[(i64)i * n_out] = v;
    }
  }
  if (!EXACT) {
    const int any = __syncthreads_or(undecided);
    if (threadIdx.x == 0) flags[wg] = any ? 1 : 0;
  }
}

static i64 t32_nrow(const fhesi_ctx* ctx) { return (i64)A32_N << ctx->tensor32->S; }
template <int NL>
static int t32_launch_rns(fhesi_ctx* ctx, const T32Config* c, const u64* d_a, const u64* d_b, i64 npolys, i64 na2, bool paired, u32* d_r) {
  const int S = ctx->tensor32->S;
  const i64 nrow = t32_nrow(ctx), n_src = ctx->phim;
  const unsigned zs = npolys * (A32_N / 256) >= 2048 ? 1u : (npolys * (A32_N / 256) >= 1024 ? 2u : 5u);
  const dim3 grid((unsigned)((S >= 3 ? nrow : (i64)A32_N) / 256), (unsigned)npolys, zs);
  const int* ia = paired && ctx->op_idx ? ctx->op_idx + ctx->op_idx_done : nullptr;
  const int* ib = ia ? ia + ctx->op_idx_n : nullptr;
  const int dup = S == 1 && ctx->lin_q ? 1 : 0;
  if (S >= 2 && !ctx->lin_q) FHESI_FAIL("tensor32: rows of 2^16 and longer exist for the padded linear-convolution rings only");
#define T32_GO(HEAD, PAIRED) do { PROF_KERNEL(ctx, PROF_RNS, rns32_reduce_kernel<NL, HEAD, PAIRED>); \
    rns32_reduce_kernel<NL, HEAD, PAIRED><<<grid, 256, 0, ctx->stream>>>(d_a, d_b, na2, n_src, nrow, d_r, c->NP, c->d_rns, ia, ib, dup); } while (0)
  if (S >= 3) { if (paired) T32_GO(0, true); else T32_GO(0, false); }
  else if (S == 2) { if (paired) T32_GO(2, true); else T32_GO(2, false); }
  else if (S && !dup) { if (paired) T32_GO(1, true); else T32_GO(1, false); }
  else { if (paired) T32_GO(0, true); else T32_GO(0, false); }
#undef T32_GO
  HIP_TRY(hipGetLastError());
  return 0;
}
static int t32_rns(fhesi_ctx* ctx, const T32Config* c, const u64* d_a, const u64* d_b, i64 npolys, i64 na2, bool paired, u32* d_r) {
  ProfScope prof(ctx, PROF_RNS, (double)npolys);
#define T32_RNS(NL) case NL: return t32_launch_rns<NL>(ctx, c, d_a, d_b, npolys, na2, paired, d_r);
  switch (c->nl) {
    T32_RNS(1) T32_RNS(2) T32_RNS(3) T32_RNS(4) T32_RNS(5) T32_RNS(6) T32_RNS(7) T32_RNS(8) T32_RNS(9) T32_RNS(10) T32_RNS(11) T32_RNS(12)
    T32_RNS(13) T32_RNS(14) T32_RNS(15) T32_RNS(16)
    default: break;
  }
#undef T32_RNS
  FHESI_FAIL("tensor32: %d limbs", c->nl);
}
static int t32_fwd(fhesi_ctx* ctx, const T32Config* c, u32* d_r, i64 npolys) {
  const fhesi_tensor32* x = ctx->tensor32;
  ProfScope prof(ctx, PROF_NTT_FWD, (double)(npolys * c->NP));
  if (npolys > 0x7fffffff) FHESI_FAIL("tensor32: too many rows per launch");
  const dim3 grid((unsigned)npolys, (unsigned)(c->NP << x->S));
#define T32_FWD_GO(SS, PB) do { PROF_KERNEL(ctx, PROF_NTT_FWD, (ntt32_fwd_kernel3<false, SS, false, T32Primes, true, false, PB>)); \
    ntt32_fwd_kernel3<false, SS, false, T32Primes, true, false, PB><<<grid, A32_T, 0, ctx->stream>>>(d_r, npolys, c->NP, 0, c->pr, x->d_fwd, Dig32Src{}, Aux32Head{}); } while (0)
  if (x->S >= 3) {
    const i64 nr = npolys * c->NP, step = (65535 / c->NP) * (i64)c->NP;
    for (i64 r0 = 0; r0 < nr; r0 += step) {
      const dim3 hg(A32_N / 256, (unsigned)std::min(step, nr - r0));
      u32* rp = d_r + (r0 << (A32_LOGN + x->S));
      if (x->S == 3) ntt32_headS_kernel<3><<<hg, 256, 0, ctx->stream>>>(rp, c->NP, 0, x->d_p, x->d_hs);
      else if (x->S == 4) ntt32_headS_kernel<4><<<hg, 256, 0, ctx->stream>>>(rp, c->NP, 0, x->d_p, x->d_hs);
      else if (x->S == 5) ntt32_headS_kernel<5><<<hg, 256, 0, ctx->stream>>>(rp, c->NP, 0, x->d_p, x->d_hs);
      else ntt32_headS_kernel<6><<<hg, 256, 0, ctx->stream>>>(rp, c->NP, 0, x->d_p, x->d_hs);
    }
    HIP_TRY(hipGetLastError());
  }
#define T32_FWD_S(PB) do { switch (x->S) { case 0: T32_FWD_GO(0, PB); break; case 1: T32_FWD_GO(1, PB); break; case 2: T32_FWD_GO(2, PB); break; case 3: T32_FWD_GO(3, PB); break; \
    case 4: T32_FWD_GO(4, PB); break; case 5: T32_FWD_GO(5, PB); break; default: T32_FWD_GO(6, PB); break; } } while (0)
  if (x->bits == 29) T32_FWD_S(29); else T32_FWD_S(30);
#undef T32_FWD_S
#undef T32_FWD_GO
  HIP_TRY(hipGetLastError());
  return 0;
}
template <int LQ, int R, int WT, int S>
static int t32_launch_crt(fhesi_ctx* ctx, const T32Config* c, const u32* d_t, i64 npolys, u64* d_parts, bool wm) {
  const i64 n = (i64)A32_N << S;
  const dim3 grid((unsigned)(n / 128), (unsigned)npolys);
  void* d_fl;
  FHESI_TRY(ws_reserve(ctx, 6, (size_t)grid.x * grid.y, &d_fl));
  unsigned char* fl = (unsigned char*)d_fl;
  PROF_KERNEL(ctx, PROF_CRT, (crt32_scale_kernel<LQ, false, R, WT, S>));
  crt32_scale_kernel<LQ, false, R, WT, S><<<grid, 128, 0, ctx->stream>>>(d_t, n, c->NP, c->pr, c->d_cinv, c->d_inv57, c->d_Mw, d_parts, fl, wm ? 1 : 0);
  HIP_TRY(hipGetLastError());
  if (!ctx->opt.crt_skip_cleanup) {
    crt32_scale_kernel<LQ, true, R, WT, S><<<grid, 128, 0, ctx->stream>>>(d_t, n, c->NP, c->pr, c->d_cinv, c->d_inv57, c->d_Mw, d_parts, fl, wm ? 1 : 0);
    HIP_TRY(hipGetLastError());
  }
  return 0;
}
static int t32_crt(fhesi_ctx* ctx, const T32Config* c, const u32* d_t, i64 npolys, u64* d_parts, bool wm) {
  const int S = ctx->tensor32->S, logQ = c->logQ;
  ProfScope prof(ctx, PROF_CRT, (double)npolys);
  if (!c->generic) {
    if (logQ == 512 && !S) return t32_launch_crt<512, T32_R_512, T32_WT_512, 0>(ctx, c, d_t, npolys, d_parts, wm);
    if (logQ == 512 && S) return t32_launch_crt<512, T32_R_512, T32_WT_512, 1>(ctx, c, d_t, npolys, d_parts, wm);
    if (logQ == 1024 && !S) return t32_launch_crt<1024, T32_R_1024, T32_WT_1024, 0>(ctx, c, d_t, npolys, d_parts, wm);
    return t32_launch_crt<1024, T32_R_1024, T32_WT_1024, 1>(ctx, c, d_t, npolys, d_parts, wm);
  }
  const i64 n_out = ctx->phim, nrow = t32_nrow(ctx);
  const int WU = (2 * logQ + 27) / 28;
  int J0 = (logQ - 64 - 38) / 28;
  if (logQ < 64 + 38) J0 = 0;
  const int NW = WU - J0;
  if (NW > T32_GEN_NW || WU > T32_GEN_NWX || WU > c->WT) FHESI_FAIL("tensor32: logQ=%d outside the generic CRT window", logQ);
  const dim3 grid((unsigned)((n_out + 127) / 128), (unsigned)npolys);
  void* d_fl;
  FHESI_TRY(ws_reserve(ctx, 6, (size_t)grid.x * grid.y, &d_fl));
  unsigned char* fl = (unsigned char*)d_fl;
  const int fold = !ctx->lin_q ? 0 : (ctx->lin_prime ? 2 : 1);
  const i64 off = ctx->lin_q;
#define T32_GEN_GO(NWM, SS, FF) do { \
    PROF_KERNEL(ctx, PROF_CRT, (crt32_scale_generic_kernel<NWM, false, SS, FF>)); \
    crt32_scale_generic_kernel<NWM, false, SS, FF><<<grid, 128, 0, ctx->stream>>>(d_t, nrow, n_out, off, c->NP, logQ, J0, NW, c->WT, c->pr, c->d_cinv, c->d_inv57, c->d_Mw, d_parts, fl, wm ? 1 : 0); \
    HIP_TRY(hipGetLastError()); \
    if (!ctx->opt.crt_skip_cleanup) { \
      crt32_scale_generic_kernel<T32_GEN_NWX, true, SS, FF><<<grid, 128, 0, ctx->stream>>>(d_t, nrow, n_out, off, c->NP, logQ, 0, WU, c->WT, c->pr, c->d_cinv, c->d_inv57, c->d_Mw, d_parts, fl, wm ? 1 : 0); \
      HIP_TRY(hipGetLastError()); \
    } } while (0)
  if (S >= 2) {
    const fhesi_tensor32* x = ctx->tensor32;
    const i64 nr = npolys * c->NP, step = (65535 / c->NP) * (i64)c->NP;
    for (i64 r0 = 0; r0 < nr; r0 += step) {
      const unsigned ny = (unsigned)std::min(step, nr - r0);
      u32* rp = const_cast<u32*>(d_t) + (r0 << (A32_LOGN + S));
      if (S == 2) ntt32_tail2_kernel<<<dim3(16, ny), 256, 0, ctx->stream>>>(rp, c->NP, 0, x->d_p, x->d_ht);
      else if (S == 3) ntt32_tailS_kernel<3><<<dim3(A32_N / 256, ny), 256, 0, ctx->stream>>>(rp, c->NP, 0, x->d_p, x->d_hs, 0);
      else if (S == 4) ntt32_tailS_kernel<4><<<dim3(A32_N / 256, ny), 256, 0, ctx->stream>>>(rp, c->NP, 0, x->d_p, x->d_hs, 0);
      else if (S == 5) ntt32_tailS_kernel<5><<<dim3(A32_N / 256, ny), 256, 0, ctx->stream>>>(rp, c->NP, 0, x->d_p, x->d_hs, 0);
      else ntt32_tailS_kernel<6><<<dim3(A32_N / 256, ny), 256, 0, ctx->stream>>>(rp, c->NP, 0, x->d_p, x->d_hs, 0);
    }
    HIP_TRY(hipGetLastError());
  }
#define T32_GEN_SF(NWM) do { \
    if (S != 1) { if (fold == 0) T32_GEN_GO(NWM, 0, 0); else if (fold == 1) T32_GEN_GO(NWM, 0, 1); else T32_GEN_GO(NWM, 0, 2); } \
    else { if (fold == 0) T32_GEN_GO(NWM, 1, 0); else if (fold == 1) T32_GEN_GO(NWM, 1, 1); else T32_GEN_GO(NWM, 1, 2); } } while (0)
  if (NW <= 16) T32_GEN_SF(16); else T32_GEN_SF(T32_GEN_NW);
#undef T32_GEN_SF
#undef T32_GEN_GO
  return 0;
}

int launch_tensor32(fhesi_ctx* ctx, u64 p, const u64* d_a, const u64* d_b, int nlimbs, int logQ, i64 count, u64* d_parts, bool parts_wm) {
  T32Config* c;
  FHESI_TRY(t32_config(ctx, p, nlimbs, logQ, 1, &c));
  if (!count) return 0;
  const fhesi_tensor32* x = ctx->tensor32;
  const int NP = c->NP, S = x->S;
  const i64 nrow = t32_nrow(ctx);
  void *d_r, *d_t;
  FHESI_TRY(ws_reserve(ctx, 5, (size_t)count * 4 * NP * nrow * 4, &d_r));
  FHESI_TRY(ws_reserve(ctx, 1, (size_t)count * 3 * NP * nrow * 4, &d_t));
  FHESI_TRY(t32_rns(ctx, c, d_a, d_b, count * 4, 0, true, (u32*)d_r));
  FHESI_TRY(t32_fwd(ctx, c, (u32*)d_r, count * 4));
  {
    ProfScope prof(ctx, PROF_NTT_INV, (double)(count * 3 * NP));
    const dim3 grid((unsigned)(count >= 8 ? ((count + 7) / 8) * 24 : count * 3), (unsigned)(NP << S));
    if (x->bits == 29) {
      PROF_KERNEL(ctx, PROF_NTT_INV, (ntt32_inv_kernel3<false, true, T32Primes, 29>));
      ntt32_inv_kernel3<false, true, T32Primes, 29><<<grid, A32_T, 0, ctx->stream>>>((u32*)d_t, count * 3, NP, 0, c->pr, x->d_inv, S, (const u32*)d_r);
    } else {
      PROF_KERNEL(ctx, PROF_NTT_INV, (ntt32_inv_kernel3<false, true, T32Primes>));
      ntt32_inv_kernel3<false, true, T32Primes><<<grid, A32_T, 0, ctx->stream>>>((u32*)d_t, count * 3, NP, 0, c->pr, x->d_inv, S, (const u32*)d_r);
    }
    HIP_TRY(hipGetLastError());
  }
  return t32_crt(ctx, c, (const u32*)d_t, count * 3, d_parts, parts_wm);
}

int tensor32_sum_begin(fhesi_ctx* ctx, u64 p, int nlimbs, int logQ, i64 gmax) {
  T32Config* c;
  FHESI_TRY(t32_config(ctx, p, nlimbs, logQ, gmax, &c));
  ctx->tensor32->cur = c;
  return 0;
}
size_t tensor32_sum_bytes(const fhesi_ctx* ctx, i64 ngroups) { return (size_t)ngroups * 3 * ctx->tensor32->cur->NP * t32_nrow(ctx) * 4; }
int tensor32_sum_pass(fhesi_ctx* ctx, const u64* d_ops, i64 nua, i64 nub, const int* d_slot_a, const int* d_slot_b, const int* d_seg, i64 ng, i64 nterms, bool accumulate, void* d_sum) {
  const T32Config* c = ctx->tensor32->cur;
  const i64 nrow = t32_nrow(ctx), n = ctx->phim;
  void* d_r;
  FHESI_TRY(ws_reserve(ctx, 0, (size_t)(nua + nub) * 2 * c->NP * nrow * 4, &d_r));
  const u64* d_b = d_ops + (size_t)nua * 2 * n * c->nl;
  FHESI_TRY(t32_rns(ctx, c, d_ops, d_b, (nua + nub) * 2, nua * 2, false, (u32*)d_r));
  FHESI_TRY(t32_fwd(ctx, c, (u32*)d_r, (nua + nub) * 2));
  const u32* ra = (const u32*)d_r;
  const u32* rb = ra + (size_t)nua * 2 * c->NP * nrow;
  ProfScope prof(ctx, PROF_TENSOR, (double)nterms);
  PROF_KERNEL(ctx, PROF_TENSOR, tensor_sum32_kernel);
  for (i64 done = 0; done < ng; done += 65535) {
    const i64 cnt = ng - done < 65535 ? ng - done : 65535;
    dim3 grid((unsigned)(nrow / 256), (unsigned)c->NP, (unsigned)cnt);
    tensor_sum32_kernel<<<grid, 256, 0, ctx->stream>>>(ra, rb, d_slot_a, d_slot_b, d_seg + done, accumulate ? 1 : 0, (u32*)d_sum + (size_t)done * 3 * c->NP * nrow, nrow, c->NP, c->pr);
  }
  HIP_TRY(hipGetLastError());
  return 0;
}
int tensor32_sum_finish(fhesi_ctx* ctx, void* d_sum, i64 ng, u64* d_parts, bool parts_wm) {
  const T32Config* c = ctx->tensor32->cur;
  const fhesi_tensor32* x = ctx->tensor32;
  {
    ProfScope prof(ctx, PROF_NTT_INV, (double)(ng * 3 * c->NP));
    const dim3 grid((unsigned)(ng * 3), (unsigned)(c->NP << x->S));
    if (x->bits == 29) {
      PROF_KERNEL(ctx, PROF_NTT_INV, (ntt32_inv_kernel3<false, false, T32Primes, 29>));
      ntt32_inv_kernel3<false, false, T32Primes, 29><<<grid, A32_T, 0, ctx->stream>>>((u32*)d_sum, ng * 3, c->NP, 0, c->pr, x->d_inv, x->S, nullptr);
    } else {
      PROF_KERNEL(ctx, PROF_NTT_INV, (ntt32_inv_kernel3<false, false, T32Primes>));
      ntt32_inv_kernel3<false, false, T32Primes><<<grid, A32_T, 0, ctx->stream>>>((u32*)d_sum, ng * 3, c->NP, 0, c->pr, x->d_inv, x->S, nullptr);
    }
    HIP_TRY(hipGetLastError());
  }
  return t32_crt(ctx, c, (const u32*)d_sum, ng * 3, d_parts, parts_wm);
}
```

fhe-si_amd/csrc/ntt32_core.inc:

```
#pragma once

struct Tw32 { u32 w, wp; };
struct Aux32Primes { u32 p[4]; u32 ninv[4], ninv_p[4]; u64 pinv64[4] , r64[4] , r48[4] ;
                     u32 mont[4] , ninv_m[4], ninv_m_p[4] ;
                     u32 ninv_mw[4][4], ninv_mw_p[4][4] ; };

struct Aux32Head { Tw32 head[4], tail_sum[4], tail_dif[4];
                   Tw32 head1[4][2]; };
static constexpr int A32_HT = 8;
static constexpr int T32_MAXP = 76;
struct T32Primes { u32 p[T32_MAXP], ninv[T32_MAXP], ninv_p[T32_MAXP], mu61[T32_MAXP]; };
__host__ __device__ __forceinline__ u32 t32_shift(u32 p) { return (p >> 29) ? 29u : 28u; }
struct fhesi_aux32 {
  Aux32Primes pr;
  Aux32Head hd;
  int S = 0;
  Tw32* d_fwd = nullptr;
  Tw32* d_inv = nullptr;
  Tw32* d_ht = nullptr;
  u32* d_p = nullptr;
  Tw32* d_hs = nullptr;
};

static constexpr int A32_LOGN = 14, A32_N = 1 << A32_LOGN, A32_T = 512, A32_P = 592;
// ... 98 lines not shown
#pragma unroll
      for (int j = 0; j < t; ++j) {
        const int h = 2 * i * t + j;
        const u32 x = v[h] >= twop ? v[h] - twop : v[h];
        const u32 T = mul_lazy32(v[h + t], w, p);
        v[h] = x + T; v[h + t] = x + twop - T;
      }
    }
  }
}
template <int S>
static __global__ void __launch_bounds__(256) ntt32_headS_kernel(u32* __restrict__ rows, int nslots, int a0, const u32* __restrict__ p_arr, const Tw32* __restrict__ hs) {
  const i64 row = blockIdx.y;
  const int a = a0 + (int)(row % nslots);
  const u32 p = p_arr[a];
  u32* g = rows + (row << (A32_LOGN + S));
  const i64 e = (i64)blockIdx.x * blockDim.x + threadIdx.x;
  u32 v[1 << S];
#pragma unroll
  for (int h = 0; h < (1 << S); ++h) v[h] = g[(i64)h * A32_N + e];
  a32_head_net<S>(v, hs + (i64)a * 2 * A32_HSN(S), p);
#pragma unroll
  for (int h = 0; h < (1 << S); ++h) g[(i64)h * A32_N + e] = v[h];
}
template <int S>
static __global__ void __launch_bounds__(256) ntt32_tailS_kernel(u32* __restrict__ rows, int nslots, int a0, const u32* __restrict__ p_arr, const Tw32* __restrict__ hs, int mont) {
  const i64 row = blockIdx.y;
  const int a = a0 + (int)(row % nslots);
  const u32 p = p_arr[a], twop = 2 * p;
  const Tw32* __restrict__ tw = hs + ((i64)a * 2 + 1) * A32_HSN(S);
  u32* g = rows + (row << (A32_LOGN + S));
  const i64 e = (i64)blockIdx.x * blockDim.x + threadIdx.x;
  u32 v[1 << S];
#pragma unroll
  for (int h = 0; h < (1 << S); ++h) v[h] = g[(i64)h * A32_N + e];
#pragma unroll
  for (int s = S - 1; s >= 1; --s) {
    const int t = 1 << (S - 1 - s);
#pragma unroll
    for (int i = 0; i < (1 << s); ++i) {
      const Tw32 w = tw[(1 << s) + i];
#pragma unroll
      for (int j = 0; j < t; ++j) {
        const int h = 2 * i * t + j;
        const u32 x = v[h], y = v[h + t];
        const u32 sm = x + y;
        v[h] = min(sm, sm - twop);
        v[h + t] = mul_lazy32(x + twop - y, w, p);
      }
    }
  }
  const Tw32 c = tw[(1 << S) + (mont ? 2 : 0)], wc = tw[(1 << S) + (mont ? 3 : 1)];
#pragma unroll
  for (int j = 0; j < (1 << (S - 1)); ++j) {
    const u32 x = v[j], y = v[j + (1 << (S - 1))];
    u32 r0 = mul_lazy32(x + y, c, p), r1 = mul_lazy32(x + twop - y, wc, p);
    v[j] = min(r0, r0 - p); v[j + (1 << (S - 1))] = min(r1, r1 - p);
  }
#pragma unroll
  for (int h = 0; h < (1 << S); ++h) g[(i64)h * A32_N + e] = v[h];
}

__device__ __forceinline__ u32 ld32(const u32* __restrict__ base, u32 boff) { asm("" : "+v"(boff)); return *(const u32*)((const char*)base + boff); }
__device__ __forceinline__ void st32(u32* __restrict__ base, u32 boff, u32 v) {
  asm("" : "+v"(boff));
  __builtin_nontemporal_store(v, (u32*)((char*)base + boff));
}
struct Dig32Src { const u64* parts; int nl, digit_bits, nd; u32 n_src; u32 sub_units = 0 ;
                  u32 nd_inv = 0, sub_inv = 0 ; };

__host__ __device__ __forceinline__ u32 div32_inv(u32 d) { return d > 1 ? (u32)(((u64)1 << 32) / d) : 0xffffffffu; }
__device__ __forceinline__ u32 div32(u32 x, u32 d, u32 inv) {
  const u32 q = (u32)(((u64)x * inv) >> 32);
  return x - q * d >= d ? q + 1 : q;
}

template <int S, bool WM>
static __global__ void __launch_bounds__(256) dig32_headS_kernel(Dig32Src ds, u32* __restrict__ dst, Aux32Primes pr, const Tw32* __restrict__ hs) {
  const i64 c = blockIdx.y;
  const i64 e = (i64)blockIdx.x * blockDim.x + threadIdx.x;
  const i64 poly = div32((u32)c, (u32)ds.nd, ds.nd_inv);
  const u32 d = (u32)c - (u32)poly * (u32)ds.nd;
  const u32 bit = d * (u32)ds.digit_bits, g0 = bit >> 5, sh = bit & 31;
  const u32 nbyt = (u32)ds.digit_bits >> 3, bo = sh >> 3;
  u32 sel = 0;
#pragma unroll
  for (u32 i = 0; i < 4; ++i) sel |= (i < nbyt ? bo + i : 0x0cu) << (8 * i);
  const u32* __restrict__ p32 = reinterpret_cast<const u32*>(ds.parts);
  constexpr u32 ES = WM ? 1 : 2;
  auto wrow = [&](u32 g) -> const u32* { return WM ? p32 + (poly * (2 * ds.nl) + g) * (i64)ds.n_src : p32 + (((poly * ds.nl + (g >> 1)) * (i64)ds.n_src) << 1) + (g & 1); };
  const u32* __restrict__ w0 = wrow(g0);
  const bool two = (sh + ds.digit_bits > 32) && (int)((g0 + 1) >> 1) < ds.nl;
  const u32* __restrict__ w1 = two ? wrow(g0 + 1) : w0;
  u32 dig[1 << S];
#pragma unroll
  for (int h = 0; h < (1 << S); ++h) {
    const i64 el = (i64)h * A32_N + e;
    u32 v = 0;
    if (el < (i64)ds.n_src) v = __builtin_amdgcn_perm(two ? w1[el * ES] : 0u, w0[el * ES], sel);
    dig[h] = v;
  }
#pragma unroll 1
  for (int a = 0; a < 4; ++a) {
    u32 v[1 << S];
#pragma unroll
    for (int h = 0; h < (1 << S); ++h) v[h] = dig[h];
    a32_head_net<S>(v, hs + (i64)a * 2 * A32_HSN(S), pr.p[a]);
    u32* g = dst + ((c * 4 + a) << (A32_LOGN + S));
#pragma unroll
    for (int h = 0; h < (1 << S); ++h) g[(i64)h * A32_N + e] = v[h];
  }
}
static constexpr int A32_HR = 16;
static inline void a32_bitrev_powers(u64 p, u64 psi, int lg, std::vector<Tw32>& out) {
  const u64 n = (u64)1 << lg;
  u64 w = 1;
  for (u64 e = 0; e < n; ++e) { out[hm::brv(e, lg)] = Tw32{(u32)w, (u32)((w << 32) / p)}; w = w * psi % p; }
}
static inline void a32_permute_phase_c(std::vector<Tw32>& t) {
  std::vector<Tw32> tmp;
  for (size_t base = 0; base + ((size_t)1 << 14) <= t.size(); base += (size_t)1 << 14)
    for (int v = 0; v < 4; ++v) {
      const size_t off = base + ((size_t)1024 << v), nq = (size_t)1 << v;
      tmp.assign(t.begin() + off, t.begin() + off + ((size_t)1024 << v));
      for (size_t tid = 0; tid < 512; ++tid)
        for (size_t q = 0; q < nq; ++q) {
          const size_t src = tid * nq + q, dst = ((tid >> 6) * nq + q) * 64 + (tid & 63);
          t[off + 2 * dst] = tmp[2 * src]; t[off + 2 * dst + 1] = tmp[2 * src + 1];
        }
    }
}
static constexpr int A32_TBL = 992;
__device__ __forceinline__ u32 a32_tbl_pos(u32 e) {
  return e;
}
__device__ __forceinline__ void a32_stage_tbl(Tw32* __restrict__ tbl, const Tw32* __restrict__ tab, u32 tid) {
  tbl[a32_tbl_pos(tid)] = tab[32 + tid];
  if (tid < 992 - 512) tbl[a32_tbl_pos(512 + tid)] = tab[32 + 512 + tid];
}
__device__ __forceinline__ u32 a32_tbl_idx(int u, u32 kq, int i) {
  return (32 << u) - 32 + (kq << u) + i;
}
typedef unsigned int a32_v4u __attribute__((ext_vector_type(4)));
#define A32_LOAD_TC(tc, tab, v, tid, wv, lane)                                                                              \
  {                                                                                                                         \
    const u32 so_ = ((1024u << (v)) * 8u) + (((wv) << (v)) * 1024u);                                                        \
    _Pragma("unroll") for (int q_ = 0; q_ < (1 << (v)); ++q_) {                                                             \
      const a32_v4u x_ = __builtin_amdgcn_raw_buffer_load_b128(tab, lane, so_ + q_ * 1024u, 0);                             \
      const int i0_ = 2 * q_, i1_ = 2 * q_ + 1;                                                                             \
      tc[i0_ >> (v)][i0_ & ((1 << (v)) - 1)] = Tw32{x_.x, x_.y};                                                  \
      tc[i1_ >> (v)][i1_ & ((1 << (v)) - 1)] = Tw32{x_.z, x_.w};                                                  \
    }                                                                                                                       \
  }
template <bool DIGITS, int S, bool PAD = false, class PR = Aux32Primes, bool NEGW = true, bool WM = false, int PB = 30>
#ifndef A32_FWD_WAVES
#define A32_FWD_WAVES 6
#endif
#ifndef A32_FWD_WAVES_S1
#define A32_FWD_WAVES_S1 6
#endif
__global__ void __launch_bounds__(A32_T, (DIGITS && ((S == 1 && !PAD) || S == 2)) ? A32_FWD_WAVES_S1 : A32_FWD_WAVES) ntt32_fwd_kernel3(
    u32* __restrict__ rows, i64 count, int nslots, int a0, PR pr, const Tw32* __restrict__ tabs,
                                                              Dig32Src ds, Aux32Head hd) {
  static_assert(PB == 30 || (PB == 29 && !DIGITS && NEGW), "primes below 2^29: plain rows of the tensor half");
  __shared__ u32 lds[A32_HR * A32_P];
  __shared__ Tw32 tbl[A32_TBL];
  const u32 tid = threadIdx.x;
  i64 c = blockIdx.x;
  int ps = (int)blockIdx.y;
  if (DIGITS) {
    const u32 bid = blockIdx.x;
    ps = (int)((bid >> 3) & ((4u << S) - 1));
    c = (i64)(bid >> (5 + S)) * 8 + (bid & 7);
    if (c >= count) return;
  }
  const int slot = ps >> S, h = ps & ((1 << S) - 1);
  const int a = a0 + slot;
  const u32 p = pr.p[a];
  const Tw32* __restrict__ tab = tabs + (((i64)a << S) + h) * A32_N;
  u32* __restrict__ g = rows + ((((c * nslots + slot)) << S) + h) * A32_N;
  a32_stage_tbl(tbl, tab, tid);
  u32 r[32];
  if constexpr (DIGITS && S >= 3) {
    const u32* __restrict__ srow = reinterpret_cast<const u32*>(ds.parts) + ((((c * 4 + slot)) << S) + h) * (i64)A32_N;
#pragma unroll
    for (int k = 0; k < 32; ++k) r[k] = srow[k * A32_T + tid];
  } else if (DIGITS) {
    const i64 poly = div32((u32)c, (u32)ds.nd, ds.nd_inv);
    const u32 d = (u32)c - (u32)poly * (u32)ds.nd;
    const u32 bit = d * (u32)ds.digit_bits, g0 = bit >> 5, sh = bit & 31;
    const u32 nbyt = (u32)ds.digit_bits >> 3, bo = sh >> 3;
    u32 sel = 0;
#pragma unroll
    for (u32 i = 0; i < 4; ++i) sel |= (i < nbyt ? bo + i : 0x0cu) << (8 * i);
    const u32* __restrict__ p32 = reinterpret_cast<const u32*>(ds.parts);
    constexpr u32 ES = WM ? 4 : 8;
    auto wrow = [&](u32 g) -> const u32* { return WM ? p32 + (poly * (2 * ds.nl) + g) * (i64)ds.n_src : p32 + (((poly * ds.nl + (g >> 1)) * (i64)ds.n_src) << 1) + (g & 1); };
    const u32* __restrict__ w0 = wrow(g0);
    const bool two = (sh + ds.digit_bits > 32) && (int)((g0 + 1) >> 1) < ds.nl;
    const u32 ns = ds.n_src;
    static_assert(!(DIGITS && S >= 2 && !PAD), "digit rows of 2^16 and longer exist for the padded linear-convolution rings only");
    if (S == 0 || (PAD && S == 1)) {
      if (two) {
        const u32* __restrict__ w1 = wrow(g0 + 1);
#pragma unroll
        for (int k = 0; k < 32; ++k) {
          const u32 el = k * A32_T + tid, e = ES * (PAD ? (el < ns ? el : 0u) : el);
          const u32 v = __builtin_amdgcn_perm(ld32(w1, e), ld32(w0, e), sel);
          r[k] = (!PAD || el < ns) ? v : 0u;
        }
      } else {
#pragma unroll
        for (int k = 0; k < 32; ++k) {
          const u32 el = k * A32_T + tid;
          const u32 v = __builtin_amdgcn_perm(0u, ld32(w0, ES * (PAD ? (el < ns ? el : 0u) : el)), sel);
          r[k] = (!PAD || el < ns) ? v : 0u;
        }
      }
    } else {
      const Tw32 hw = S == 2 ? hd.head1[a][h >> 1] : hd.head[a];
      const u32* __restrict__ w1 = wrow(g0 + 1);
      auto body = [&](auto TWO) {
        constexpr bool two_c = decltype(TWO)::value;
        constexpr int NB = two_c ? 8 : 16;
        auto dig = [&](u32 el) -> u32 {
          const u32 e = ES * (PAD ? (el < ns ? el : 0u) : el);
          const u32 v = two_c ? __builtin_amdgcn_perm(ld32(w1, e), ld32(w0, e), sel) : __builtin_amdgcn_perm(0u, ld32(w0, e), sel);
          return (!PAD || el < ns) ? v : 0u;
        };
#pragma unroll
        for (int k0 = 0; k0 < 32; k0 += NB) {
          u32 y[NB];
#pragma unroll
          for (int k = 0; k < NB; ++k) y[k] = dig((k0 + k) * A32_T + tid + A32_N);
#pragma unroll
          for (int k = 0; k < NB; ++k) r[k0 + k] = mul_lazy32(y[k], hw, p);
        }
#pragma unroll
        for (int k0 = 0; k0 < 32; k0 += NB) {
          u32 x[NB];
#pragma unroll
          for (int k = 0; k < NB; ++k) x[k] = dig((k0 + k) * A32_T + tid);
#pragma unroll
          for (int k = 0; k < NB; ++k) r[k0 + k] = (h & 1) == 0 ? x[k] + r[k0 + k] : x[k] + 2 * p - r[k0 + k];
        }
      };
      if (two) body(std::true_type{}); else body(std::false_type{});
    }
  } else {
#pragma unroll
    for (int k = 0; k < 32; ++k) r[k] = g[k * A32_T + tid];
  }
#pragma unroll
  for (int s = 0; s < 5; ++s) {
    const int h = 16 >> s;
#pragma unroll
    for (int b = 0; b < 16; ++b) {
      const int k = a32_bfly_k(b, h);
      if (DIGITS && (S == 0 || (PAD && S == 1)) && NEGW && s == 0) a32_ct<NEGW, true, true>(r[k], r[k + h], tab[(1 << s) + (k >> (5 - s))], p);
      else a32_ct<NEGW, true>(r[k], r[k + h], tab[(1 << s) + (k >> (5 - s))], p, PB == 29 ? a32_fwd_step29(s) : 1);
    }
  }
  const u32 kq = tid >> 4, lo = tid & 15;
  const bool upper = kq >= A32_HR;
#pragma unroll
  for (int k = 0; k < 16; ++k) lds[k * A32_P + a32_f(tid)] = r[k];
  __syncthreads();
  u32 t[16];
#pragma unroll
  for (int k = 0; k < 16; ++k) t[k] = r[16 + k];
  if (!upper) {
#pragma unroll
    for (int k2 = 0; k2 < 32; ++k2) r[k2] = lds[kq * A32_P + a32_f(k2 * 16 + lo)];
  }
  __syncthreads();
#pragma unroll
  for (int k = 0; k < 16; ++k) lds[k * A32_P + a32_f(tid)] = t[k];
  __syncthreads();
  if (upper) {
#pragma unroll
    for (int k2 = 0; k2 < 32; ++k2) r[k2] = lds[(kq - A32_HR) * A32_P + a32_f(k2 * 16 + lo)];
  }
#pragma unroll
  for (int u = 0; u < 5; ++u) {
    const int h = 16 >> u;
    Tw32 tb[16];
#pragma unroll
    for (int i = 0; i < (1 << u); ++i) tb[i] = tbl[a32_tbl_idx(u, kq, i)];
#pragma unroll
    for (int b = 0; b < 16; ++b) {
      const int k2 = a32_bfly_k(b, h);
      a32_ct<NEGW>(r[k2], r[k2 + h], tb[k2 >> (5 - u)], p, PB == 29 ? a32_fwd_step29(5 + u) : 1);
    }
  }
  const u32 wv = __builtin_amdgcn_readfirstlane(tid >> 6), sub = kq & 3;
  __syncthreads();
  u32* __restrict__ row = lds + (2 * wv + (sub & 1)) * A32_P;
#pragma unroll
  for (int hh = 0; hh < 2; ++hh) {
    if ((int)(sub >> 1) == hh) {
#pragma unroll
      for (int k2 = 0; k2 < 32; ++k2) row[a32_f(k2 * 16 + lo)] = r[k2];
    }
    __builtin_amdgcn_wave_barrier();
    if ((int)(sub >> 1) == hh) {
#pragma unroll
      for (int i = 0; i < 32; ++i) r[i] = row[lo * 36 + i];
    }
    __builtin_amdgcn_wave_barrier();
  }
  const u32 tcb = (tid & 63) * 16;
  const __amdgpu_buffer_rsrc_t tabr = __builtin_amdgcn_make_buffer_rsrc(const_cast<Tw32*>(tab), 0, A32_N * 8, 0x00020000);
#define A32_TABC tabr
#pragma unroll
  for (int v = 0; v < 4; ++v) {
    const int h = 8 >> v;
    Tw32 tc[2][8];
    A32_LOAD_TC(tc, A32_TABC, v, tid, wv, tcb);
#pragma unroll
    for (int gq = 0; gq < 2; ++gq) {
#pragma unroll
      for (int b = 0; b < 8; ++b) {
        const int x = a32_bfly_k(b, h);
        a32_ct<NEGW>(r[gq * 16 + x], r[gq * 16 + x + h], tc[gq][x >> (4 - v)], p, PB == 29 ? a32_fwd_step29(10 + v) : 1);
      }
    }
  }
  const u32 lane = tid & 63;
  u32* __restrict__ stage = lds + 2 * wv * A32_P;
#pragma unroll
  for (int hh = 0; hh < 2; ++hh) {
    __builtin_amdgcn_wave_barrier();
    if ((int)(sub >> 1) == hh) {
      u32* w = stage + ((sub & 1) * 8 + (lo >> 1)) * 72 + (lo & 1) * 36;
#pragma unroll
      for (int i = 0; i < 32; ++i) {
        u32 v = r[i];
        if (!DIGITS) {
          const u32 twop = 2 * p;
          if (PB == 29) v = min(v, v - 2 * twop);
          v = v >= twop ? v - twop : v; v = v >= p ? v - p : v;
        }
        w[i] = v;
      }
    }
    __builtin_amdgcn_wave_barrier();
    const u32 pos = lane < 32 ? lane : lane + 4;
    i64 cnt_s = count, c_s = c, base_s = 0;
    if (DIGITS && ds.sub_units) {
      const i64 sub = div32((u32)c, ds.sub_units, ds.sub_inv), rest = count - sub * ds.sub_units;
      c_s = c - sub * ds.sub_units;
      cnt_s = rest < (i64)ds.sub_units ? rest : (i64)ds.sub_units;
      base_s = sub * ds.sub_units * (((i64)4 << (A32_LOGN - 6 + S)) * 64);
    }
    const i64 stride = DIGITS ? cnt_s * 64 : 64;
    u32* __restrict__ sp = (DIGITS ? rows + base_s + ((((i64)a << (A32_LOGN - 6 + S)) + ((i64)h << (A32_LOGN - 6)) + (32 * wv + 16 * hh)) * cnt_s + c_s) * 64 : g + (32 * wv + 16 * hh) * 64);
    const u32 lboff = lane * 4;
#pragma unroll
    for (int t = 0; t < 16; ++t) {
      const u32 v = stage[t * 72 + pos];
      st32(sp, lboff, v);
      sp += stride;
    }
  }
}

template <bool MONT, bool TENSOR = false, class PR = Aux32Primes, int PB = 30>
__global__ void __launch_bounds__(A32_T, A32_INV_WAVES) ntt32_inv_kernel3(u32* __restrict__ rows, i64 count, int nslots, int a0, PR pr, const Tw32* __restrict__ tabs, int S,
                                                              const u32* __restrict__ tsrc) {
  static_assert(PB == 30 || (PB == 29 && !MONT), "primes below 2^29: the rows of the tensor half");
  __shared__ u32 lds[A32_HR * A32_P];
  __shared__ Tw32 tbl[A32_TBL];
  const u32 tid = threadIdx.x;
  i64 c = blockIdx.x;
  const int ps = (int)blockIdx.y;
  if (TENSOR && count >= 24) {
    const u32 bid = blockIdx.x;
    const u32 grp = bid / 24, in = bid % 24;
    const i64 ct = (i64)grp * 8 + (in & 7);
    c = ct * 3 + (in >> 3);
    if (ct * 3 >= count) return;
  }
  const int slot = ps >> S, h = ps & ((1 << S) - 1), a = a0 + slot;
  const u32 p = pr.p[a];
  const Tw32* __restrict__ tab = tabs + (((i64)a << S) + h) * A32_N;
  u32* __restrict__ g = rows + (((c * nslots + slot) << S) + h) * A32_N;
  const u32 kq = tid >> 4, lo = tid & 15, wv = TENSOR ? tid >> 6 : __builtin_amdgcn_readfirstlane(tid >> 6), sub = kq & 3, lane = tid & 63;
  const bool upper = kq >= A32_HR;
  a32_stage_tbl(tbl, tab, tid);
  u32 r[32];
  u32* __restrict__ stage = lds + 2 * wv * A32_P;
#pragma unroll
  for (int hh = 0; hh < 2; ++hh) {
    const u32 pos = lane < 32 ? lane : lane + 4;
    u32 v[16];
    if constexpr (TENSOR) {
      const i64 ct = c / 3;
      const int comp = (int)(c - ct * 3);
      auto srow = [&](int jj) { return tsrc + (((((ct * 4 + jj) * nslots + slot)) << S) + h) * A32_N; };
      const u32* __restrict__ sa = srow(comp == 2 ? 1 : 0);
      const u32* __restrict__ sb = srow(comp == 0 ? 2 : 3);
      const u32 mu = pr.mu61[a], twop = 2 * p;
      auto red = [&](u64 x) -> u32 {
        const u32 q = __umulhi((u32)(x >> (PB == 29 ? 28 : 29)), mu);
        const u32 r = (u32)x - q * p;
        return r >= twop ? r - twop : r;
      };
      if (comp == 1) {
        const u32* __restrict__ sc = srow(1);
        const u32* __restrict__ sd = srow(2);
#pragma unroll
        for (int t0 = 0; t0 < 16; t0 += 8) {
          u32 x0[8], y1[8], x1[8], y0[8];
#pragma unroll
          for (int t = 0; t < 8; ++t) {
            const u32 off = ((4 * wv + 2 * hh + ((t0 + t) >> 3)) * 8 + ((t0 + t) & 7)) * 64 + lane;
            x0[t] = sa[off]; y1[t] = sb[off]; x1[t] = sc[off]; y0[t] = sd[off];
          }
#pragma unroll
          for (int t = 0; t < 8; ++t) v[t0 + t] = red((u64)x0[t] * y1[t] + (u64)x1[t] * y0[t]);
        }
      } else {
        u32 x[16], y[16];
#pragma unroll
        for (int t = 0; t < 16; ++t) {
          const u32 off = ((4 * wv + 2 * hh + (t >> 3)) * 8 + (t & 7)) * 64 + lane;
          x[t] = sa[off]; y[t] = sb[off];
        }
#pragma unroll
        for (int t = 0; t < 16; ++t) v[t] = red((u64)x[t] * y[t]);
      }
    } else {
#pragma unroll
      for (int t = 0; t < 16; ++t) v[t] = g[((4 * wv + 2 * hh + (t >> 3)) * 8 + (t & 7)) * 64 + lane];
    }
    __builtin_amdgcn_wave_barrier();
#pragma unroll
    for (int t = 0; t < 16; ++t) stage[t * 72 + pos] = v[t];
    __builtin_amdgcn_wave_barrier();
    if ((int)(sub >> 1) == hh) {
      const u32* w = stage + ((sub & 1) * 8 + (lo >> 1)) * 72 + (lo & 1) * 36;
#pragma unroll
      for (int i = 0; i < 32; ++i) r[i] = w[i];
    }
  }
  const u32 tcb = lane * 16, wvs = __builtin_amdgcn_readfirstlane(tid >> 6);
  const __amdgpu_buffer_rsrc_t tabr = __builtin_amdgcn_make_buffer_rsrc(const_cast<Tw32*>(tab), 0, A32_N * 8, 0x00020000);
#pragma unroll
  for (int v = 3; v >= 0; --v) {
    const int h = 8 >> v;
    Tw32 tc[2][8];
    A32_LOAD_TC(tc, A32_TABC, v, tid, wvs, tcb);
#pragma unroll
    for (int gq = 0; gq < 2; ++gq) {
#pragma unroll
      for (int b = 0; b < 8; ++b) {
        const int x = a32_bfly_k(b, h);
        if (MONT && !TENSOR && v == 3) a32_gs<true>(r[gq * 16 + x], r[gq * 16 + x + h], tc[gq][x >> (4 - v)], p);
        else if (PB == 29) a32_gs29(r[gq * 16 + x], r[gq * 16 + x + h], tc[gq][x >> (4 - v)], p, v == 3 || (x & (h >> 1)) != 0);
        else a32_gs(r[gq * 16 + x], r[gq * 16 + x + h], tc[gq][x >> (4 - v)], p);
      }
    }
  }
  {
    u32* __restrict__ row = lds + (2 * wv + (sub & 1)) * A32_P;
#pragma unroll
    for (int hh = 0; hh < 2; ++hh) {
      __builtin_amdgcn_wave_barrier();
      if ((int)(sub >> 1) == hh) {
#pragma unroll
        for (int i = 0; i < 32; ++i) row[lo * 36 + i] = r[i];
      }
      __builtin_amdgcn_wave_barrier();
      if ((int)(sub >> 1) == hh) {
#pragma unroll
        for (int k2 = 0; k2 < 32; ++k2) r[k2] = row[a32_f(k2 * 16 + lo)];
      }
    }
  }
  __syncthreads();
#pragma unroll
  for (int u = 4; u >= 0; --u) {
    const int h = 16 >> u;
    Tw32 tb[16];
#pragma unroll
    for (int i = 0; i < (1 << u); ++i) tb[i] = tbl[a32_tbl_idx(u, kq, i)];
#pragma unroll
    for (int b = 0; b < 16; ++b) {
      const int k2 = a32_bfly_k(b, h);
      if (PB == 29) a32_gs29(r[k2], r[k2 + h], tb[k2 >> (5 - u)], p, u != 4 && (k2 & (h >> 1)) != 0);
      else a32_gs(r[k2], r[k2 + h], tb[k2 >> (5 - u)], p);
    }
  }
  u32 t[16];
  if (!upper) {
#pragma unroll
    for (int k2 = 0; k2 < 32; ++k2) lds[kq * A32_P + a32_f(k2 * 16 + lo)] = r[k2];
  }
  __syncthreads();
#pragma unroll
  for (int k = 0; k < 16; ++k) t[k] = lds[k * A32_P + a32_f(tid)];
  __syncthreads();
  if (upper) {
#pragma unroll
    for (int k2 = 0; k2 < 32; ++k2) lds[(kq - A32_HR) * A32_P + a32_f(k2 * 16 + lo)] = r[k2];
  }
  __syncthreads();
#pragma unroll
  for (int k = 0; k < 16; ++k) r[16 + k] = lds[k * A32_P + a32_f(tid)];
#define R(k) ((k) < 16 ? t[(k)] : r[(k)])
#pragma unroll
  for (int s2 = 4; s2 >= 1; --s2) {
    const int h = 16 >> s2;
#pragma unroll
    for (int b = 0; b < 16; ++b) {
      const int k = a32_bfly_k(b, h);
      if (PB == 29) a32_gs29<true>(R(k), R(k + h), tab[(1 << s2) + (k >> (5 - s2))], p, s2 != 4 && (k & (h >> 1)) != 0);
      else a32_gs<false, true>(R(k), R(k + h), tab[(1 << s2) + (k >> (5 - s2))], p);
// ... 19 lines not shown
```

include/fhesi_hip.h:

```cpp
#ifndef FHESI_HIP_H_
#define FHESI_HIP_H_

#include <stddef.h>
#include <stdint.h>

#ifdef __cplusplus
extern "C" {
#endif

typedef struct fhesi_ctx fhesi_ctx;
typedef struct fhesi_dcrt fhesi_dcrt;
typedef struct fhesi_ksk fhesi_ksk;
typedef struct fhesi_slots fhesi_slots;
typedef struct fhesi_comm fhesi_comm;

enum { FHESI_OP_ADD = 0, FHESI_OP_SUB = 1, FHESI_OP_MUL = 2, FHESI_OP_DIV = 3, FHESI_OP_SET = 4 };

const char* fhesi_last_error(void);
int fhesi_device_count(int32_t* count);
#define FHESI_ABI_VERSION 7
int32_t fhesi_abi_version(void);

int fhesi_ctx_create(fhesi_ctx** out, int64_t m, int32_t nprimes, const uint64_t* q, const uint64_t* root, int32_t device);
int fhesi_ctx_destroy(fhesi_ctx* ctx);
int64_t fhesi_ctx_m(const fhesi_ctx* ctx);
int64_t fhesi_ctx_phim(const fhesi_ctx* ctx);
int32_t fhesi_ctx_nprimes(const fhesi_ctx* ctx);
int fhesi_ctx_prime(const fhesi_ctx* ctx, int32_t i, uint64_t* q, uint64_t* root);
int fhesi_ctx_zms_idx(const fhesi_ctx* ctx, int32_t* out_m);
int fhesi_ctx_phi_m(const fhesi_ctx* ctx, int64_t* out_phim_plus_1);
int fhesi_ctx_sync(fhesi_ctx* ctx);
void* fhesi_ctx_stream(fhesi_ctx* ctx);
int fhesi_ctx_set_option(fhesi_ctx* ctx, const char* name, int64_t value);
int fhesi_ctx_get_option(const fhesi_ctx* ctx, const char* name, int64_t* value);
int fhesi_ctx_copy_options(fhesi_ctx* dst, const fhesi_ctx* src);
int fhesi_timer_start(fhesi_ctx* ctx);
int fhesi_timer_stop(fhesi_ctx* ctx, float* elapsed_ms);

enum { FHESI_PROF_NTT_FWD = 0, FHESI_PROF_NTT_INV = 1, FHESI_PROF_RNS = 2, FHESI_PROF_TENSOR = 3, FHESI_PROF_CRT = 4,
       FHESI_PROF_DIGITS = 5, FHESI_PROF_DOT = 6, FHESI_PROF_EW = 7,
       FHESI_PROF_NTT_FWD_DIGITS_MAIN = 8  };
int fhesi_prof_enable(fhesi_ctx* ctx, int32_t on);
int fhesi_prof_read(fhesi_ctx* ctx, int32_t kernel_class, int64_t* launches, double* units, double* total_ms);
int fhesi_prof_kernel_name(fhesi_ctx* ctx, int32_t kernel_class, char* name_out, size_t name_cap);

int fhesi_cmod_fft(fhesi_ctx* ctx, int32_t prime, const uint64_t* coeff_limbs, int32_t nlimbs, int64_t ncoeffs, uint64_t* y_out);
int fhesi_cmod_ifft(fhesi_ctx* ctx, int32_t prime, const uint64_t* y, uint64_t* x_out );

int fhesi_dcrt_alloc(fhesi_ctx* ctx, const int32_t* prime_idx, int32_t nidx, fhesi_dcrt** out);
int fhesi_dcrt_free(fhesi_dcrt* d);
int fhesi_dcrt_copy(fhesi_dcrt* dst, const fhesi_dcrt* src);
int fhesi_dcrt_index_set(const fhesi_dcrt* d, int32_t* idx_out, int32_t* nidx);
int fhesi_dcrt_equal(const fhesi_dcrt* a, const fhesi_dcrt* b, int32_t* equal);
int fhesi_dcrt_upload_row(fhesi_dcrt* d, int32_t prime, const uint64_t* row);
int fhesi_dcrt_download_row(const fhesi_dcrt* d, int32_t prime, uint64_t* row);
void* fhesi_dcrt_device_ptr(fhesi_dcrt* d);
int fhesi_dcrt_from_poly(fhesi_dcrt* d, const uint64_t* coeff_limbs, int32_t nlimbs, int64_t ncoeffs);
int fhesi_dcrt_to_poly(const fhesi_dcrt* d, const int32_t* prime_idx, int32_t nidx, int32_t positive,
                       uint64_t* coeff_limbs_out, int32_t nlimbs);
int fhesi_dcrt_op(fhesi_dcrt* dst, const fhesi_dcrt* src, int32_t op);
int fhesi_dcrt_op_scalar(fhesi_dcrt* d, const uint64_t* num_limbs, int32_t nlimbs, int32_t op);
int fhesi_dcrt_exp(fhesi_dcrt* d, int64_t e);
int fhesi_dcrt_automorph(fhesi_dcrt* d, int64_t k);
int fhesi_dcrt_add_primes(fhesi_dcrt* d, const int32_t* prime_idx, int32_t nidx);
int fhesi_dcrt_remove_primes(fhesi_dcrt* d, const int32_t* prime_idx, int32_t nidx);
int fhesi_dcrt_add_primes_and_scale(fhesi_dcrt* d, const int32_t* prime_idx, int32_t nidx, uint64_t p, double* log_factor_out);
int fhesi_dcrt_scale_down_to_set(fhesi_dcrt* d, const int32_t* prime_idx, int32_t nidx, uint64_t p);
int fhesi_dcrt_from_scrt(fhesi_dcrt* d, const uint64_t* coeff_rows);
int fhesi_dcrt_to_scrt(const fhesi_dcrt* d, uint64_t* coeff_rows_out);

int fhesi_scrt_alloc(fhesi_ctx* ctx, const int32_t* prime_idx, int32_t nidx, fhesi_dcrt** out);
int fhesi_scrt_from_poly(fhesi_dcrt* s, const uint64_t* coeff_limbs, int32_t nlimbs, int64_t ncoeffs);
int fhesi_scrt_to_poly(const fhesi_dcrt* s, const int32_t* prime_idx, int32_t nidx, uint64_t* coeff_limbs_out, int32_t nlimbs);
int fhesi_scrt_op_scalar(fhesi_dcrt* s, const uint64_t* num_limbs, int32_t nlimbs, int32_t op);
int fhesi_dcrt_assign_scrt(fhesi_dcrt* d, const fhesi_dcrt* s);
int fhesi_scrt_assign_dcrt(fhesi_dcrt* s, const fhesi_dcrt* d, const int32_t* prime_idx, int32_t nidx);

int fhesi_rows_ntt_fwd_dev(fhesi_ctx* ctx, uint64_t* rows_dev, int64_t count);
int fhesi_rows_ntt_inv_dev(fhesi_ctx* ctx, uint64_t* rows_dev, int64_t count);
int fhesi_rows_op_dev(fhesi_ctx* ctx, uint64_t* dst_dev, const uint64_t* src_dev, int64_t count, int32_t op);

int fhesi_ksk_create(fhesi_ctx* ctx, int32_t ncomp, int32_t ndigits, fhesi_ksk** out);
int fhesi_ksk_free(fhesi_ksk* k);
int fhesi_ksk_upload(fhesi_ksk* k, const uint64_t* rows_host);
void* fhesi_ksk_device_ptr(fhesi_ksk* k);
int fhesi_ksk_mark_dirty(fhesi_ksk* k);
int fhesi_ksk_upload_dev(fhesi_ksk* k, const uint64_t* rows_dev);
size_t fhesi_ksk_bytes(const fhesi_ksk* k);
int fhesi_ksk_form(const fhesi_ksk* k, int32_t* form, int32_t* rows, int32_t* limb_bits);
int fhesi_ksk_key_bits(const fhesi_ksk* k, int32_t* centred, int32_t* key_bits);

int fhesi_selftest_aux32(fhesi_ctx* c);

int fhesi_ct_mul_relin_batch(fhesi_ctx* ctx, const fhesi_ksk* k, int32_t logQ, uint64_t p, int32_t decomp_bytes,
                             const uint64_t* a_host, const uint64_t* b_host, uint64_t* out_host, int32_t nlimbs, int64_t count);
int fhesi_host_alloc(fhesi_ctx* ctx, size_t bytes, void** out);
int fhesi_host_free(fhesi_ctx* ctx, void* p);
int fhesi_host_stage_release(fhesi_ctx* ctx);
int fhesi_ct_mul_relin_batch_dev(fhesi_ctx* ctx, const fhesi_ksk* k, int32_t logQ, uint64_t p, int32_t decomp_bytes,
                                 const uint64_t* a_dev, const uint64_t* b_dev, uint64_t* out_dev, int32_t nlimbs, int64_t count);
int fhesi_ct_mul_dev(fhesi_ctx* ctx, uint64_t p, const uint64_t* a_dev, const uint64_t* b_dev, int32_t nlimbs, int64_t count,
                     uint64_t* tprod_dev );
int fhesi_apply_key_switch_dev(fhesi_ctx* ctx, const fhesi_ksk* k, int32_t logQ, int32_t decomp_bytes,
                               const uint64_t* tprod_dev, int64_t count, uint64_t* out_dev, int32_t nlimbs);

int fhesi_ct_add_dev(fhesi_ctx* ctx, int32_t logQ, uint64_t* dst_dev, const uint64_t* src_dev, int32_t nparts, int32_t nlimbs, int64_t count);
int fhesi_ct_add_const_dev(fhesi_ctx* ctx, int32_t logQ, uint64_t p, uint64_t* ct_dev, int32_t nparts, int32_t nlimbs, int64_t count,
                           const int64_t* poly_host , int32_t npoly );
int fhesi_ct_mul_poly_dev(fhesi_ctx* ctx, int32_t logQ, uint64_t* ct_dev, int32_t nparts, int32_t nlimbs, int64_t count,
                          const int64_t* poly_host , int32_t npoly);
int fhesi_ct_mul_long_dev(fhesi_ctx* ctx, int32_t logQ, uint64_t* ct_dev, int64_t l, int32_t nparts, int32_t nlimbs, int64_t count);
int fhesi_rows_mul_long_dev(fhesi_ctx* ctx, uint64_t* rows_dev, int64_t l, int64_t count);
int fhesi_ct_automorph_dev(fhesi_ctx* ctx, int64_t k, const uint64_t* in_dev, int32_t nparts, int32_t nlimbs_in, int64_t count,
                           uint64_t* out_dev, int32_t nlimbs_out);
int fhesi_ct_automorph_key_switch_dev(fhesi_ctx* ctx, const fhesi_ksk* k_matrix, int32_t logQ, int32_t decomp_bytes, int64_t k,
                                      const uint64_t* in_dev, int32_t nlimbs_in, int64_t count, uint64_t* out_dev, int32_t nlimbs);
int fhesi_ct_gather_dev(fhesi_ctx* ctx, const uint64_t* pool_dev, const int32_t* idx_host, int64_t count, int64_t words, uint64_t* out_dev);
int fhesi_ct_mul_sum_relin_dev(fhesi_ctx* ctx, const fhesi_ksk* k, int32_t logQ, uint64_t p, int32_t decomp_bytes, const uint64_t* pool_dev,
                               int32_t nlimbs, const int32_t* a_idx, const int32_t* b_idx, const int32_t* seg, int64_t ngroups, uint64_t* out_dev);

int fhesi_encrypt_batch(fhesi_ctx* ctx, const fhesi_dcrt* pk0, const fhesi_dcrt* pk1, int32_t logQ, uint64_t p, const int64_t* rand_host,
                        const int64_t* msg_host, int64_t count, uint64_t* out_dev, int32_t nlimbs);
int fhesi_decrypt_batch(fhesi_ctx* ctx, const fhesi_dcrt* sk1, int32_t logQ, uint64_t p, const uint64_t* ct_dev, int32_t nlimbs, int64_t count,
                        int64_t* msg_host);

int fhesi_keyswitch_init_batch(fhesi_ksk* k, const fhesi_dcrt* const* src, int32_t nsrc, const fhesi_dcrt* dst_t, int32_t logQ, int32_t decomp_bytes,
                               const uint64_t* a_host, int32_t nlimbs, const int64_t* err_host);
int fhesi_ksk_download(const fhesi_ksk* k, uint64_t* rows_host);

int fhesi_encrypt_batch_seeded(fhesi_ctx* ctx, const fhesi_dcrt* pk0, const fhesi_dcrt* pk1, int32_t logQ, uint64_t p, uint64_t seed, uint64_t first_index,
                               const int64_t* msg_host, int64_t count, uint64_t* out_dev, int32_t nlimbs);
int fhesi_keyswitch_init_batch_seeded(fhesi_ksk* k, const fhesi_dcrt* const* src, int32_t nsrc, const fhesi_dcrt* dst_t, int32_t logQ, int32_t decomp_bytes,
                                      uint64_t seed, uint64_t public_seed, uint64_t first_index);
int fhesi_dcrt_sample(fhesi_dcrt* d, int32_t kind, int64_t param, uint64_t seed, uint64_t index);

int fhesi_slots_plan(int64_t m, uint64_t p, int64_t generator, int64_t* total, int64_t* usable, uint64_t* rho0, int32_t* aux_primes,
                     int32_t* e_out );
int fhesi_slots_create(fhesi_ctx* ctx, uint64_t p, int64_t generator, fhesi_slots** out);
int fhesi_slots_free(fhesi_slots* s);
int fhesi_slots_info(const fhesi_slots* s, int64_t* total, int64_t* usable, uint64_t* rho0, int32_t* aux_primes_used);
int fhesi_slots_exponents(const fhesi_slots* s, int32_t* e_out );
int fhesi_slots_embed(fhesi_slots* s, const int64_t* vals_host , int64_t nvals, int32_t only_usable, int64_t count,
                      int64_t* msg_host );
int fhesi_slots_decode(fhesi_slots* s, const int64_t* msg_host , int64_t count, int64_t nvals, int32_t only_usable,
                       int64_t* vals_host );
int fhesi_slots_embed_dev(fhesi_slots* s, const int64_t* vals_dev, int64_t nvals, int32_t only_usable, int64_t count, int64_t* msg_dev);
int fhesi_slots_decode_dev(fhesi_slots* s, const int64_t* msg_dev, int64_t count, int64_t nvals, int32_t only_usable, int64_t* vals_dev);
int fhesi_encrypt_slots_batch_seeded(fhesi_ctx* ctx, fhesi_slots* s, const fhesi_dcrt* pk0, const fhesi_dcrt* pk1, int32_t logQ, uint64_t seed, uint64_t first_index,
                                     const int64_t* vals_host , int64_t nvals, int32_t only_usable, int64_t count, uint64_t* out_dev, int32_t nlimbs);
int fhesi_decrypt_slots_batch(fhesi_ctx* ctx, fhesi_slots* s, const fhesi_dcrt* sk1, int32_t logQ, const uint64_t* ct_dev, int32_t nlimbs, int64_t count,
                              int64_t nvals, int32_t only_usable, int64_t* vals_host );
int fhesi_encrypt_noise_batch_seeded(fhesi_ctx* ctx, fhesi_slots* s, const fhesi_dcrt* pk0, const fhesi_dcrt* pk1, int32_t logQ, uint64_t seed, uint64_t first_index,
                                     int64_t count, uint64_t* out_dev, int32_t nlimbs);

int fhesi_slots_plan_pow2(int64_t m, uint64_t p, int64_t generator, int64_t* total, int64_t* rows, int64_t* cols, uint64_t* rho0,
                          int32_t* path , int32_t* e_out );
int fhesi_slots_create_pow2(fhesi_ctx* ctx, uint64_t p, int64_t generator, fhesi_slots** out);
int fhesi_slots_shape(const fhesi_slots* s, int64_t* rows, int64_t* cols, int32_t* path);
int fhesi_slots_set_path(fhesi_slots* s, int32_t path);

int fhesi_comm_init_all(int32_t ndev, const int32_t* devices, fhesi_comm** comms_out);
int fhesi_comm_from_rccl(void* nccl_comm, fhesi_comm** out);
int fhesi_comm_destroy(fhesi_comm* comm);
int32_t fhesi_comm_rank(const fhesi_comm* comm);
int32_t fhesi_comm_size(const fhesi_comm* comm);
int fhesi_ksk_broadcast(fhesi_ksk* k, fhesi_comm* comm, int32_t root);
int fhesi_comm_broadcast_dev(fhesi_ctx* ctx, fhesi_comm* comm, void* buf_dev, size_t bytes, int32_t root);
int fhesi_comm_exchange(fhesi_ctx* ctx, fhesi_comm* comm, uint64_t* base_dev, const int64_t* offsets_words);
int fhesi_comm_exchange_begin(fhesi_ctx* ctx, fhesi_comm* comm, uint64_t* base_dev, const int64_t* offsets_words);
int fhesi_comm_exchange_end(fhesi_ctx* ctx, fhesi_comm* comm);
int fhesi_comm_allreduce_rows(fhesi_ctx* ctx, fhesi_comm* comm, uint64_t* rows_dev, int64_t count);

int fhesi_dev_alloc(fhesi_ctx* ctx, size_t bytes, void** out_dev);
int fhesi_dev_free(fhesi_ctx* ctx, void* dev);
int fhesi_dev_upload(fhesi_ctx* ctx, void* dst_dev, const void* src_host, size_t bytes);
int fhesi_dev_download(fhesi_ctx* ctx, void* dst_host, const void* src_dev, size_t bytes);
int fhesi_dev_copy(fhesi_ctx* ctx, void* dst_dev, const void* src_dev, size_t bytes);

#ifdef __cplusplus
}
#endif
#endif
```

Baseline: 32830.

## Compute RNS base conversion with int8 MFMA and fuse first NTT stages

Adds a phase-A kernel that converts the 64-bit limb coefficients into residues for every 30-bit prime. It does this with int8 16x16x64 MFMA matrix multiplies against precomputed balanced-byte tables, followed by a Barrett-style reduction. The same kernel runs the first four forward-NTT butterfly stages in registers, and the forward NTT launch switches to a skip variant that starts after those stages. The path is on by default when inputs have 8 limbs and the setup is single-ring, paired, with phim = 2^14. It aims to replace scalar multiply-reduce work in the RNS reduction and to save a memory round trip for the early NTT stages. In exchange it adds table setup and a new correctness-sensitive arithmetic path.

Measured after the change: 33270, median of 6. +1.3%, better.

```diff
diff --git a/fhe-si_amd/binding.py b/fhe-si_amd/binding.py
--- a/fhe-si_amd/binding.py
+++ b/fhe-si_amd/binding.py
@@ -36,6 +36,7 @@
     "fhesi_slots_plan", "fhesi_slots_create", "fhesi_slots_free", "fhesi_slots_info", "fhesi_slots_exponents", "fhesi_slots_embed", "fhesi_slots_decode",
     "fhesi_slots_embed_dev", "fhesi_slots_decode_dev", "fhesi_encrypt_slots_batch_seeded", "fhesi_decrypt_slots_batch", "fhesi_encrypt_noise_batch_seeded",
     "fhesi_slots_plan_pow2", "fhesi_slots_create_pow2", "fhesi_slots_shape", "fhesi_slots_set_path",
+    "fhesi_mfma_i8_tile",
 ]
 ABI_VERSION = 7
 PROF_CLASSES = {"ntt_fwd": 0, "ntt_inv": 1, "rns_reduce": 2, "tensor": 3, "crt": 4, "digits": 5, "dot": 6, "ew": 7, "ntt_fwd_digits_main": 8}
@@ -104,6 +105,7 @@
         "fhesi_dcrt_automorph": [_vp, _i64],
         "fhesi_dcrt_exp": [_vp, _i64],
         "fhesi_selftest_aux32": [_vp],
+        "fhesi_mfma_i8_tile": [_vp, _vp, _vp, _vp],
         "fhesi_dcrt_add_primes": [_vp, _vp, _i32],
         "fhesi_dcrt_remove_primes": [_vp, _vp, _i32],
         "fhesi_dcrt_from_scrt": [_vp, _vp],
@@ -326,6 +328,14 @@
     def selftest_aux32(self):
         _ck(_load().fhesi_selftest_aux32(self.h))
 
+    def mfma_i8_tile(self, a, b):
+        import numpy as np
+        a = np.ascontiguousarray(a, dtype=np.int8).reshape(16, 64)
+        b = np.ascontiguousarray(b, dtype=np.int8).reshape(64, 16)
+        c = np.zeros((16, 16), dtype=np.int32)
+        _ck(_load().fhesi_mfma_i8_tile(self.h, _vp(a.ctypes.data), _vp(b.ctypes.data), _vp(c.ctypes.data)))
+        return c
+
     def dev_copy(self, dst_ptr: int, src_ptr: int, nbytes: int):
         _ck(_load().fhesi_dev_copy(self.h, _vp(dst_ptr), _vp(src_ptr), nbytes))
 
diff --git a/fhe-si_amd/csrc/capi_ctx.hip b/fhe-si_amd/csrc/capi_ctx.hip
--- a/fhe-si_amd/csrc/capi_ctx.hip
+++ b/fhe-si_amd/csrc/capi_ctx.hip
@@ -75,6 +75,7 @@
   {"wave_single", "FHESI_WAVE_SINGLE", offsetof(CtxOptions, wave_single), false},
   {"tensor32", "FHESI_TENSOR32", offsetof(CtxOptions, tensor32), false},
   {"tensor_bits", "FHESI_TENSOR_BITS", offsetof(CtxOptions, tensor_bits), false},
+  {"conv_mfma", "FHESI_CONV_MFMA", offsetof(CtxOptions, conv_mfma), false},
   {"dot32_k4", "FHESI_DOT32_K4", offsetof(CtxOptions, dot32_k4), false},
   {"parts_words", "FHESI_PARTS_WORDS", offsetof(CtxOptions, parts_words), false},
   {"automorph_rows", "FHESI_AUTOMORPH_ROWS", offsetof(CtxOptions, automorph_rows), false},
diff --git a/fhe-si_amd/csrc/fhesi_internal.h b/fhe-si_amd/csrc/fhesi_internal.h
--- a/fhe-si_amd/csrc/fhesi_internal.h
+++ b/fhe-si_amd/csrc/fhesi_internal.h
@@ -75,6 +75,7 @@
   int tensor32 = 1;
   int tensor_bits = 30;
   int dot32_k4 = 1;
+  int conv_mfma = 1;
   int parts_words = 1;
 };
 
@@ -168,6 +169,9 @@
 void host_stage_free(fhesi_ctx* ctx);
 bool tensor32_applies(const fhesi_ctx* ctx, u64 p, int nlimbs, int logQ);
 int launch_tensor32(fhesi_ctx* ctx, u64 p, const u64* d_a, const u64* d_b, int nlimbs, int logQ, i64 count, u64* d_parts , bool parts_wm = false);
+static constexpr int CONV_MFMA_STAGES = 4;
+int conv_mfma_tables(const u32* primes, int NP, u64 lift, void** d_tab, void** d_cst);
+int launch_rns32_mfma_phaseA(fhesi_ctx* ctx, const u64* d_a, const u64* d_b, i64 npolys, u32* d_rows, int NP, int prime_bits, const void* d_tab, const void* d_cst, const void* d_fwd);
 bool tensor32_sum_applies(const fhesi_ctx* ctx, u64 p, int nlimbs, int logQ, i64 gmax);
 int tensor32_sum_begin(fhesi_ctx* ctx, u64 p, int nlimbs, int logQ, i64 gmax);
 size_t tensor32_sum_bytes(const fhesi_ctx* ctx, i64 ngroups);
diff --git a/fhe-si_amd/csrc/kernels_conv_mfma.hip b/fhe-si_amd/csrc/kernels_conv_mfma.hip
--- /dev/null
+++ b/fhe-si_amd/csrc/kernels_conv_mfma.hip
@@ -0,0 +1,149 @@
+#include "../../include/fhesi_hip.h"
+#include "fhesi_internal.h"
+#include "ntt32_core.inc"
+#include <vector>
+
+typedef int cm_v4i __attribute__((ext_vector_type(4)));
+struct CmPrime { u32 k0, k2, p, mu; };
+
+static inline int cm_operand_lane(int rc, int k) { return rc + 16 * (k >> 4); }
+
+static __global__ void __launch_bounds__(64) mfma_i8_tile_kernel(const cm_v4i* __restrict__ a, const cm_v4i* __restrict__ b, int* __restrict__ c) {
+  const u32 l = threadIdx.x;
+  cm_v4i acc = {0, 0, 0, 0};
+  acc = __builtin_amdgcn_mfma_i32_16x16x64_i8(a[l], b[l], acc, 0, 0, 0);
+#pragma unroll
+  for (int r = 0; r < 4; ++r) c[(4 * (l >> 4) + r) * 16 + (l & 15)] = acc[r];
+}
+extern "C" int fhesi_mfma_i8_tile(fhesi_ctx* ctx, const int8_t* a, const int8_t* b, int32_t* c) {
+  if (!ctx || !a || !b || !c) FHESI_FAIL("mfma_i8_tile: null argument");
+  HIP_TRY(hipSetDevice(ctx->device));
+  std::vector<int8_t> ha(1024), hb(1024);
+  for (int rc = 0; rc < 16; ++rc)
+    for (int k = 0; k < 64; ++k) {
+      const int at = cm_operand_lane(rc, k) * 16 + (k & 15);
+      ha[at] = a[rc * 64 + k];
+      hb[at] = b[k * 16 + rc];
+    }
+  void *da = nullptr, *db = nullptr, *dc = nullptr;
+  int rc = 1;
+  if (hipMalloc(&da, 1024) == hipSuccess && hipMalloc(&db, 1024) == hipSuccess && hipMalloc(&dc, 1024) == hipSuccess &&
+      hipMemcpy(da, ha.data(), 1024, hipMemcpyHostToDevice) == hipSuccess && hipMemcpy(db, hb.data(), 1024, hipMemcpyHostToDevice) == hipSuccess) {
+    mfma_i8_tile_kernel<<<1, 64, 0, ctx->stream>>>((const cm_v4i*)da, (const cm_v4i*)db, (int*)dc);
+    if (hipGetLastError() == hipSuccess && hipStreamSynchronize(ctx->stream) == hipSuccess && hipMemcpy(c, dc, 1024, hipMemcpyDeviceToHost) == hipSuccess) rc = 0;
+  }
+  hipFree(da); hipFree(db); hipFree(dc);
+  if (rc) FHESI_FAIL("mfma_i8_tile: device call failed");
+  return 0;
+}
+
+int conv_mfma_tables(const u32* primes, int NP, u64 lift, void** d_tab, void** d_cst) {
+  const int ntile = (NP + 3) >> 2;
+  std::vector<int8_t> tab((size_t)2 * ntile * 1024, 0);
+  std::vector<CmPrime> cst((size_t)2 * NP);
+  for (int cls = 0; cls < 2; ++cls)
+    for (int a = 0; a < NP; ++a) {
+      const u64 p = primes[a];
+      u64 cur = cls == 0 ? lift % p : 1, off = 0;
+      for (int j = 0; j < 64; ++j) {
+        i64 v = (i64)cur;
+        for (int pl = 0; pl < 4; ++pl) {
+          const int d = (int)((v + 128) & 255) - 128;
+          v = (v - d) >> 8;
+          const int lane = cm_operand_lane(4 * (a & 3) + pl, j);
+          tab[((size_t)(cls * ntile + (a >> 2)) * 64 + lane) * 16 + (j & 15)] = (int8_t)d;
+        }
+        if (v) FHESI_FAIL("conv_mfma: constant beyond four balanced bytes");
+        if (j < 63) off = (off + 128 * cur) % p;
+        cur = cur * 256 % p;
+      }
+      const u64 K = off + p * ((((u64)1 << 45) + p - 1) / p);
+      const u64 k0 = ((u64)1 << 29) + (K & 0xffff);
+      cst[(size_t)cls * NP + a] = CmPrime{(u32)k0, (u32)((K - k0) >> 16), (u32)p, (u32)(((u64)1 << (32 + t32_shift((u32)p))) / p)};
+    }
+  *d_tab = *d_cst = nullptr;
+  if (hipMalloc(d_tab, tab.size()) != hipSuccess || hipMalloc(d_cst, cst.size() * sizeof(CmPrime)) != hipSuccess ||
+      hipMemcpy(*d_tab, tab.data(), tab.size(), hipMemcpyHostToDevice) != hipSuccess ||
+      hipMemcpy(*d_cst, cst.data(), cst.size() * sizeof(CmPrime), hipMemcpyHostToDevice) != hipSuccess) {
+    hipFree(*d_tab); hipFree(*d_cst);
+    *d_tab = *d_cst = nullptr;
+    FHESI_FAIL("conv_mfma: table upload failed");
+  }
+  return 0;
+}
+
+template <int PB, int NA>
+__global__ void __launch_bounds__(256, 2) rns32_reduce_kernel_mfma(const u64* __restrict__ a, const u64* __restrict__ b, u32* __restrict__ rows, int NP,
+                                                                    const cm_v4i* __restrict__ tabA, const CmPrime* __restrict__ cst, const Tw32* __restrict__ fwd) {
+  const u32 lane = threadIdx.x & 63, wv = threadIdx.x >> 6;
+  const u32 col = lane & 15, grp = lane >> 4;
+  const i64 poly = blockIdx.y;
+  const i64 ct = poly >> 2;
+  const int jp = (int)(poly & 3), cls = jp >> 1;
+  const u32 t = (blockIdx.x * 4 + wv) * 16 + col;
+  const char* __restrict__ src = reinterpret_cast<const char*>((cls ? b : a) + (ct * 2 + (jp & 1)) * (i64)A32_N * 8);
+  u32 soff = (t * 4 + grp) * 16;
+  asm("" : "+v"(soff));
+  cm_v4i B[32];
+#pragma unroll
+  for (int k = 0; k < 32; ++k) B[k] = __builtin_nontemporal_load(reinterpret_cast<const cm_v4i*>(src + (i64)k * (A32_T * 64) + soff));
+  const int mtop = grp == 3 ? 0x00808080 : (int)0x80808080u;
+#pragma unroll
+  for (int k = 0; k < 32; ++k) { B[k].x ^= (int)0x80808080u; B[k].y ^= (int)0x80808080u; B[k].z ^= (int)0x80808080u; B[k].w ^= mtop; }
+  const int ntile = (NP + 3) >> 2;
+  constexpr u32 sh = PB == 29 ? 28u : 29u;
+#pragma unroll 1
+  for (int g = 0; g < ntile; ++g) {
+    const cm_v4i A = tabA[(cls * ntile + g) * 64 + lane];
+    const int prime = 4 * g + (int)grp;
+    const bool live = prime < NP;
+    const int pi = live ? prime : NP - 1;
+    const CmPrime c = cst[cls * NP + pi];
+    const u32 p = c.p;
+    const cm_v4i acc0 = {(int)c.k0, 0, (int)c.k2, 0};
+    const Tw32* __restrict__ tab = fwd + (i64)pi * A32_N;
+    u32 r[32];
+#pragma unroll
+    for (int k = 0; k < 32; ++k) {
+      const cm_v4i acc = __builtin_amdgcn_mfma_i32_16x16x64_i8(A, B[k], acc0, 0, 0, 0);
+      const u32 lo = ((u32)acc.y << 8) + (u32)acc.x, hi = ((u32)acc.w << 8) + (u32)acc.z;
+      const u32 q = __umulhi(hi >> (sh - 16), c.mu);
+      r[k] = (hi << 16) + lo - q * p;
+    }
+#pragma unroll
+    for (int s = 0; s < NA; ++s) {
+      const int h = 16 >> s;
+#pragma unroll
+      for (int i0 = 0; i0 < (1 << s); i0 += 8) {
+        Tw32 tw[8];
+#pragma unroll
+        for (int i = 0; i < 8 && i0 + i < (1 << s); ++i) tw[i] = tab[(1 << s) + i0 + i];
+#pragma unroll
+        for (int bf = 0; bf < 16; ++bf) {
+          const int k = a32_bfly_k(bf, h), i = (k >> (5 - s)) - i0;
+          if (i >= 0 && i < 8) a32_ct<true, false>(r[k], r[k + h], tw[i], p, PB == 29 ? a32_fwd_step29(s) : 1);
+        }
+      }
+    }
+    if (live) {
+      u32* __restrict__ o = rows + poly * NP * (i64)A32_N;
+      const u32 ooff = ((u32)prime * (u32)A32_N + t) * 4;
+      u32 oo = ooff;
+      asm("" : "+v"(oo));
+#pragma unroll
+      for (int k = 0; k < 32; ++k) *(u32*)((char*)(o + k * A32_T) + oo) = r[k];
+    }
+  }
+}
+
+int launch_rns32_mfma_phaseA(fhesi_ctx* ctx, const u64* d_a, const u64* d_b, i64 npolys, u32* d_rows, int NP, int prime_bits, const void* d_tab, const void* d_cst,
+                             const void* d_fwd) {
+  if (npolys > 65535 || (npolys & 3)) FHESI_FAIL("conv_mfma: %lld polynomials per launch", (long long)npolys);
+  const dim3 grid(A32_T / 64, (unsigned)npolys);
+#define CM_GO(PB) do { PROF_KERNEL(ctx, PROF_RNS, (rns32_reduce_kernel_mfma<PB, CONV_MFMA_STAGES>)); \
+    rns32_reduce_kernel_mfma<PB, CONV_MFMA_STAGES><<<grid, 256, 0, ctx->stream>>>(d_a, d_b, d_rows, NP, (const cm_v4i*)d_tab, (const CmPrime*)d_cst, (const Tw32*)d_fwd); } while (0)
+  if (prime_bits == 29) CM_GO(29); else CM_GO(30);
+#undef CM_GO
+  HIP_TRY(hipGetLastError());
+  return 0;
+}
diff --git a/fhe-si_amd/csrc/kernels_tensor32.hip b/fhe-si_amd/csrc/kernels_tensor32.hip
--- a/fhe-si_amd/csrc/kernels_tensor32.hip
+++ b/fhe-si_amd/csrc/kernels_tensor32.hip
@@ -11,7 +11,8 @@
   Tw32* d_cinv = nullptr;
   u32* d_inv57 = nullptr;
   u32* d_Mw = nullptr;
-  ~T32Config() { hipFree(d_rns); hipFree(d_cinv); hipFree(d_inv57); hipFree(d_Mw); }
+  void *d_mfma = nullptr, *d_mfmaK = nullptr;
+  ~T32Config() { hipFree(d_rns); hipFree(d_cinv); hipFree(d_inv57); hipFree(d_Mw); hipFree(d_mfma); hipFree(d_mfmaK); }
 };
 struct fhesi_tensor32 {
   int S = 0;
@@ -270,6 +271,7 @@
     delete c;
     FHESI_FAIL("tensor32: table upload failed");
   }
+  if (nlimbs == 8 && S == 0 && !ctx->lin_q && conv_mfma_tables(primes.data(), NP, lift, &c->d_mfma, &c->d_mfmaK)) { delete c; return 1; }
   x->cfgs.push_back(c);
   *out = c;
   return 0;
@@ -633,8 +635,12 @@
   HIP_TRY(hipGetLastError());
   return 0;
 }
+static bool t32_conv_mfma(const fhesi_ctx* ctx, const T32Config* c, bool paired) {
+  return ctx->opt.conv_mfma && c->d_mfma && paired && !ctx->op_idx && !ctx->tensor32->S && !ctx->lin_q && ctx->phim == A32_N;
+}
 static int t32_rns(fhesi_ctx* ctx, const T32Config* c, const u64* d_a, const u64* d_b, i64 npolys, i64 na2, bool paired, u32* d_r) {
   ProfScope prof(ctx, PROF_RNS, (double)npolys);
+  if (t32_conv_mfma(ctx, c, paired)) return launch_rns32_mfma_phaseA(ctx, d_a, d_b, npolys, d_r, c->NP, ctx->tensor32->bits, c->d_mfma, c->d_mfmaK, ctx->tensor32->d_fwd);
 #define T32_RNS(NL) case NL: return t32_launch_rns<NL>(ctx, c, d_a, d_b, npolys, na2, paired, d_r);
   switch (c->nl) {
     T32_RNS(1) T32_RNS(2) T32_RNS(3) T32_RNS(4) T32_RNS(5) T32_RNS(6) T32_RNS(7) T32_RNS(8) T32_RNS(9) T32_RNS(10) T32_RNS(11) T32_RNS(12)
@@ -644,7 +650,7 @@
 #undef T32_RNS
   FHESI_FAIL("tensor32: %d limbs", c->nl);
 }
-static int t32_fwd(fhesi_ctx* ctx, const T32Config* c, u32* d_r, i64 npolys) {
+static int t32_fwd(fhesi_ctx* ctx, const T32Config* c, u32* d_r, i64 npolys, bool paired) {
   const fhesi_tensor32* x = ctx->tensor32;
   ProfScope prof(ctx, PROF_NTT_FWD, (double)(npolys * c->NP));
   if (npolys > 0x7fffffff) FHESI_FAIL("tensor32: too many rows per launch");
@@ -665,7 +671,11 @@
   }
 #define T32_FWD_S(PB) do { switch (x->S) { case 0: T32_FWD_GO(0, PB); break; case 1: T32_FWD_GO(1, PB); break; case 2: T32_FWD_GO(2, PB); break; case 3: T32_FWD_GO(3, PB); break; \
     case 4: T32_FWD_GO(4, PB); break; case 5: T32_FWD_GO(5, PB); break; default: T32_FWD_GO(6, PB); break; } } while (0)
-  if (x->bits == 29) T32_FWD_S(29); else T32_FWD_S(30);
+#define T32_FWD_SKIPA(PB) do { PROF_KERNEL(ctx, PROF_NTT_FWD, (ntt32_fwd_skipA_kernel3<false, 0, false, T32Primes, true, false, PB, CONV_MFMA_STAGES>)); \
+    ntt32_fwd_skipA_kernel3<false, 0, false, T32Primes, true, false, PB, CONV_MFMA_STAGES><<<grid, A32_T, 0, ctx->stream>>>(d_r, npolys, c->NP, 0, c->pr, x->d_fwd, Dig32Src{}, Aux32Head{}); } while (0)
+  if (t32_conv_mfma(ctx, c, paired)) { if (x->bits == 29) T32_FWD_SKIPA(29); else T32_FWD_SKIPA(30); }
+  else if (x->bits == 29) T32_FWD_S(29); else T32_FWD_S(30);
+#undef T32_FWD_SKIPA
 #undef T32_FWD_S
 #undef T32_FWD_GO
   HIP_TRY(hipGetLastError());
@@ -750,7 +760,7 @@
   FHESI_TRY(ws_reserve(ctx, 5, (size_t)count * 4 * NP * nrow * 4, &d_r));
   FHESI_TRY(ws_reserve(ctx, 1, (size_t)count * 3 * NP * nrow * 4, &d_t));
   FHESI_TRY(t32_rns(ctx, c, d_a, d_b, count * 4, 0, true, (u32*)d_r));
-  FHESI_TRY(t32_fwd(ctx, c, (u32*)d_r, count * 4));
+  FHESI_TRY(t32_fwd(ctx, c, (u32*)d_r, count * 4, true));
   {
     ProfScope prof(ctx, PROF_NTT_INV, (double)(count * 3 * NP));
     const dim3 grid((unsigned)(count >= 8 ? ((count + 7) / 8) * 24 : count * 3), (unsigned)(NP << S));
@@ -780,7 +790,7 @@
   FHESI_TRY(ws_reserve(ctx, 0, (size_t)(nua + nub) * 2 * c->NP * nrow * 4, &d_r));
   const u64* d_b = d_ops + (size_t)nua * 2 * n * c->nl;
   FHESI_TRY(t32_rns(ctx, c, d_ops, d_b, (nua + nub) * 2, nua * 2, false, (u32*)d_r));
-  FHESI_TRY(t32_fwd(ctx, c, (u32*)d_r, (nua + nub) * 2));
+  FHESI_TRY(t32_fwd(ctx, c, (u32*)d_r, (nua + nub) * 2, false));
   const u32* ra = (const u32*)d_r;
   const u32* rb = ra + (size_t)nua * 2 * c->NP * nrow;
   ProfScope prof(ctx, PROF_TENSOR, (double)nterms);
diff --git a/fhe-si_amd/csrc/ntt32_core.inc b/fhe-si_amd/csrc/ntt32_core.inc
--- a/fhe-si_amd/csrc/ntt32_core.inc
+++ b/fhe-si_amd/csrc/ntt32_core.inc
@@ -274,218 +274,26 @@
       tc[i1_ >> (v)][i1_ & ((1 << (v)) - 1)] = Tw32{x_.z, x_.w};                                                  \
     }                                                                                                                       \
   }
-template <bool DIGITS, int S, bool PAD = false, class PR = Aux32Primes, bool NEGW = true, bool WM = false, int PB = 30>
 #ifndef A32_FWD_WAVES
 #define A32_FWD_WAVES 6
 #endif
 #ifndef A32_FWD_WAVES_S1
 #define A32_FWD_WAVES_S1 6
 #endif
-__global__ void __launch_bounds__(A32_T, (DIGITS && ((S == 1 && !PAD) || S == 2)) ? A32_FWD_WAVES_S1 : A32_FWD_WAVES) ntt32_fwd_kernel3(
-    u32* __restrict__ rows, i64 count, int nslots, int a0, PR pr, const Tw32* __restrict__ tabs,
-                                                              Dig32Src ds, Aux32Head hd) {
-  static_assert(PB == 30 || (PB == 29 && !DIGITS && NEGW), "primes below 2^29: plain rows of the tensor half");
-  __shared__ u32 lds[A32_HR * A32_P];
-  __shared__ Tw32 tbl[A32_TBL];
-  const u32 tid = threadIdx.x;
-  i64 c = blockIdx.x;
-  int ps = (int)blockIdx.y;
-  if (DIGITS) {
-    const u32 bid = blockIdx.x;
-    ps = (int)((bid >> 3) & ((4u << S) - 1));
-    c = (i64)(bid >> (5 + S)) * 8 + (bid & 7);
-    if (c >= count) return;
-  }
-  const int slot = ps >> S, h = ps & ((1 << S) - 1);
-  const int a = a0 + slot;
-  const u32 p = pr.p[a];
-  const Tw32* __restrict__ tab = tabs + (((i64)a << S) + h) * A32_N;
-  u32* __restrict__ g = rows + ((((c * nslots + slot)) << S) + h) * A32_N;
-  a32_stage_tbl(tbl, tab, tid);
-  u32 r[32];
-  if constexpr (DIGITS && S >= 3) {
-    const u32* __restrict__ srow = reinterpret_cast<const u32*>(ds.parts) + ((((c * 4 + slot)) << S) + h) * (i64)A32_N;
-#pragma unroll
-    for (int k = 0; k < 32; ++k) r[k] = srow[k * A32_T + tid];
-  } else if (DIGITS) {
-    const i64 poly = div32((u32)c, (u32)ds.nd, ds.nd_inv);
-    const u32 d = (u32)c - (u32)poly * (u32)ds.nd;
-    const u32 bit = d * (u32)ds.digit_bits, g0 = bit >> 5, sh = bit & 31;
-    const u32 nbyt = (u32)ds.digit_bits >> 3, bo = sh >> 3;
-    u32 sel = 0;
-#pragma unroll
-    for (u32 i = 0; i < 4; ++i) sel |= (i < nbyt ? bo + i : 0x0cu) << (8 * i);
-    const u32* __restrict__ p32 = reinterpret_cast<const u32*>(ds.parts);
-    constexpr u32 ES = WM ? 4 : 8;
-    auto wrow = [&](u32 g) -> const u32* { return WM ? p32 + (poly * (2 * ds.nl) + g) * (i64)ds.n_src : p32 + (((poly * ds.nl + (g >> 1)) * (i64)ds.n_src) << 1) + (g & 1); };
-    const u32* __restrict__ w0 = wrow(g0);
-    const bool two = (sh + ds.digit_bits > 32) && (int)((g0 + 1) >> 1) < ds.nl;
-    const u32 ns = ds.n_src;
-    static_assert(!(DIGITS && S >= 2 && !PAD), "digit rows of 2^16 and longer exist for the padded linear-convolution rings only");
-    if (S == 0 || (PAD && S == 1)) {
-      if (two) {
-        const u32* __restrict__ w1 = wrow(g0 + 1);
-#pragma unroll
-        for (int k = 0; k < 32; ++k) {
-          const u32 el = k * A32_T + tid, e = ES * (PAD ? (el < ns ? el : 0u) : el);
-          const u32 v = __builtin_amdgcn_perm(ld32(w1, e), ld32(w0, e), sel);
-          r[k] = (!PAD || el < ns) ? v : 0u;
-        }
-      } else {
-#pragma unroll
-        for (int k = 0; k < 32; ++k) {
-          const u32 el = k * A32_T + tid;
-          const u32 v = __builtin_amdgcn_perm(0u, ld32(w0, ES * (PAD ? (el < ns ? el : 0u) : el)), sel);
-          r[k] = (!PAD || el < ns) ? v : 0u;
-        }
-      }
-    } else {
-      const Tw32 hw = S == 2 ? hd.head1[a][h >> 1] : hd.head[a];
-      const u32* __restrict__ w1 = wrow(g0 + 1);
-      auto body = [&](auto TWO) {
-        constexpr bool two_c = decltype(TWO)::value;
-        constexpr int NB = two_c ? 8 : 16;
-        auto dig = [&](u32 el) -> u32 {
-          const u32 e = ES * (PAD ? (el < ns ? el : 0u) : el);
-          const u32 v = two_c ? __builtin_amdgcn_perm(ld32(w1, e), ld32(w0, e), sel) : __builtin_amdgcn_perm(0u, ld32(w0, e), sel);
-          return (!PAD || el < ns) ? v : 0u;
-        };
-#pragma unroll
-        for (int k0 = 0; k0 < 32; k0 += NB) {
-          u32 y[NB];
-#pragma unroll
-          for (int k = 0; k < NB; ++k) y[k] = dig((k0 + k) * A32_T + tid + A32_N);
-#pragma unroll
-          for (int k = 0; k < NB; ++k) r[k0 + k] = mul_lazy32(y[k], hw, p);
-        }
-#pragma unroll
-        for (int k0 = 0; k0 < 32; k0 += NB) {
-          u32 x[NB];
-#pragma unroll
-          for (int k = 0; k < NB; ++k) x[k] = dig((k0 + k) * A32_T + tid);
-#pragma unroll
-          for (int k = 0; k < NB; ++k) r[k0 + k] = (h & 1) == 0 ? x[k] + r[k0 + k] : x[k] + 2 * p - r[k0 + k];
-        }
-      };
-      if (two) body(std::true_type{}); else body(std::false_type{});
-    }
-  } else {
-#pragma unroll
-    for (int k = 0; k < 32; ++k) r[k] = g[k * A32_T + tid];
-  }
-#pragma unroll
-  for (int s = 0; s < 5; ++s) {
-    const int h = 16 >> s;
-#pragma unroll
-    for (int b = 0; b < 16; ++b) {
-      const int k = a32_bfly_k(b, h);
-      if (DIGITS && (S == 0 || (PAD && S == 1)) && NEGW && s == 0) a32_ct<NEGW, true, true>(r[k], r[k + h], tab[(1 << s) + (k >> (5 - s))], p);
-      else a32_ct<NEGW, true>(r[k], r[k + h], tab[(1 << s) + (k >> (5 - s))], p, PB == 29 ? a32_fwd_step29(s) : 1);
-    }
-  }
-  const u32 kq = tid >> 4, lo = tid & 15;
-  const bool upper = kq >= A32_HR;
-#pragma unroll
-  for (int k = 0; k < 16; ++k) lds[k * A32_P + a32_f(tid)] = r[k];
-  __syncthreads();
-  u32 t[16];
-#pragma unroll
-  for (int k = 0; k < 16; ++k) t[k] = r[16 + k];
-  if (!upper) {
-#pragma unroll
-    for (int k2 = 0; k2 < 32; ++k2) r[k2] = lds[kq * A32_P + a32_f(k2 * 16 + lo)];
-  }
-  __syncthreads();
-#pragma unroll
-  for (int k = 0; k < 16; ++k) lds[k * A32_P + a32_f(tid)] = t[k];
-  __syncthreads();
-  if (upper) {
-#pragma unroll
-    for (int k2 = 0; k2 < 32; ++k2) r[k2] = lds[(kq - A32_HR) * A32_P + a32_f(k2 * 16 + lo)];
-  }
-#pragma unroll
-  for (int u = 0; u < 5; ++u) {
-    const int h = 16 >> u;
-    Tw32 tb[16];
-#pragma unroll
-    for (int i = 0; i < (1 << u); ++i) tb[i] = tbl[a32_tbl_idx(u, kq, i)];
-#pragma unroll
-    for (int b = 0; b < 16; ++b) {
-      const int k2 = a32_bfly_k(b, h);
-      a32_ct<NEGW>(r[k2], r[k2 + h], tb[k2 >> (5 - u)], p, PB == 29 ? a32_fwd_step29(5 + u) : 1);
-    }
-  }
-  const u32 wv = __builtin_amdgcn_readfirstlane(tid >> 6), sub = kq & 3;
-  __syncthreads();
-  u32* __restrict__ row = lds + (2 * wv + (sub & 1)) * A32_P;
-#pragma unroll
-  for (int hh = 0; hh < 2; ++hh) {
-    if ((int)(sub >> 1) == hh) {
-#pragma unroll
-      for (int k2 = 0; k2 < 32; ++k2) row[a32_f(k2 * 16 + lo)] = r[k2];
-    }
-    __builtin_amdgcn_wave_barrier();
-    if ((int)(sub >> 1) == hh) {
-#pragma unroll
-      for (int i = 0; i < 32; ++i) r[i] = row[lo * 36 + i];
-    }
-    __builtin_amdgcn_wave_barrier();
-  }
-  const u32 tcb = (tid & 63) * 16;
-  const __amdgpu_buffer_rsrc_t tabr = __builtin_amdgcn_make_buffer_rsrc(const_cast<Tw32*>(tab), 0, A32_N * 8, 0x00020000);
-#define A32_TABC tabr
-#pragma unroll
-  for (int v = 0; v < 4; ++v) {
-    const int h = 8 >> v;
-    Tw32 tc[2][8];
-    A32_LOAD_TC(tc, A32_TABC, v, tid, wv, tcb);
-#pragma unroll
-    for (int gq = 0; gq < 2; ++gq) {
-#pragma unroll
-      for (int b = 0; b < 8; ++b) {
-        const int x = a32_bfly_k(b, h);
-        a32_ct<NEGW>(r[gq * 16 + x], r[gq * 16 + x + h], tc[gq][x >> (4 - v)], p, PB == 29 ? a32_fwd_step29(10 + v) : 1);
-      }
-    }
-  }
-  const u32 lane = tid & 63;
-  u32* __restrict__ stage = lds + 2 * wv * A32_P;
-#pragma unroll
-  for (int hh = 0; hh < 2; ++hh) {
-    __builtin_amdgcn_wave_barrier();
-    if ((int)(sub >> 1) == hh) {
-      u32* w = stage + ((sub & 1) * 8 + (lo >> 1)) * 72 + (lo & 1) * 36;
-#pragma unroll
-      for (int i = 0; i < 32; ++i) {
-        u32 v = r[i];
-        if (!DIGITS) {
-          const u32 twop = 2 * p;
-          if (PB == 29) v = min(v, v - 2 * twop);
-          v = v >= twop ? v - twop : v; v = v >= p ? v - p : v;
-        }
-        w[i] = v;
-      }
-    }
-    __builtin_amdgcn_wave_barrier();
-    const u32 pos = lane < 32 ? lane : lane + 4;
-    i64 cnt_s = count, c_s = c, base_s = 0;
-    if (DIGITS && ds.sub_units) {
-      const i64 sub = div32((u32)c, ds.sub_units, ds.sub_inv), rest = count - sub * ds.sub_units;
-      c_s = c - sub * ds.sub_units;
-      cnt_s = rest < (i64)ds.sub_units ? rest : (i64)ds.sub_units;
-      base_s = sub * ds.sub_units * (((i64)4 << (A32_LOGN - 6 + S)) * 64);
-    }
-    const i64 stride = DIGITS ? cnt_s * 64 : 64;
-    u32* __restrict__ sp = (DIGITS ? rows + base_s + ((((i64)a << (A32_LOGN - 6 + S)) + ((i64)h << (A32_LOGN - 6)) + (32 * wv + 16 * hh)) * cnt_s + c_s) * 64 : g + (32 * wv + 16 * hh) * 64);
-    const u32 lboff = lane * 4;
-#pragma unroll
-    for (int t = 0; t < 16; ++t) {
-      const u32 v = stage[t * 72 + pos];
-      st32(sp, lboff, v);
-      sp += stride;
-    }
-  }
-}
+#define A32_FWD_KERNEL ntt32_fwd_kernel3
+#define A32_FWD_EXTRA
+#define A32_FWD_FIRST 0
+#include "ntt32_fwd_kernel3.inc"
+#undef A32_FWD_KERNEL
+#undef A32_FWD_EXTRA
+#undef A32_FWD_FIRST
+#define A32_FWD_KERNEL ntt32_fwd_skipA_kernel3
+#define A32_FWD_EXTRA , int SKIPA = 5
+#define A32_FWD_FIRST SKIPA
+#include "ntt32_fwd_kernel3.inc"
+#undef A32_FWD_KERNEL
+#undef A32_FWD_EXTRA
+#undef A32_FWD_FIRST
 
 template <bool MONT, bool TENSOR = false, class PR = Aux32Primes, int PB = 30>
 __global__ void __launch_bounds__(A32_T, A32_INV_WAVES) ntt32_inv_kernel3(u32* __restrict__ rows, i64 count, int nslots, int a0, PR pr, const Tw32* __restrict__ tabs, int S,
diff --git a/fhe-si_amd/csrc/ntt32_fwd_kernel3.inc b/fhe-si_amd/csrc/ntt32_fwd_kernel3.inc
--- /dev/null
+++ b/fhe-si_amd/csrc/ntt32_fwd_kernel3.inc
@@ -0,0 +1,206 @@
+template <bool DIGITS, int S, bool PAD = false, class PR = Aux32Primes, bool NEGW = true, bool WM = false, int PB = 30 A32_FWD_EXTRA>
+__global__ void __launch_bounds__(A32_T, (DIGITS && ((S == 1 && !PAD) || S == 2)) ? A32_FWD_WAVES_S1 : A32_FWD_WAVES) A32_FWD_KERNEL(
+    u32* __restrict__ rows, i64 count, int nslots, int a0, PR pr, const Tw32* __restrict__ tabs,
+                                                              Dig32Src ds, Aux32Head hd) {
+  static_assert(PB == 30 || (PB == 29 && !DIGITS && NEGW), "primes below 2^29: plain rows of the tensor half");
+  __shared__ u32 lds[A32_HR * A32_P];
+  __shared__ Tw32 tbl[A32_TBL];
+  const u32 tid = threadIdx.x;
+  i64 c = blockIdx.x;
+  int ps = (int)blockIdx.y;
+  if (DIGITS) {
+    const u32 bid = blockIdx.x;
+    ps = (int)((bid >> 3) & ((4u << S) - 1));
+    c = (i64)(bid >> (5 + S)) * 8 + (bid & 7);
+    if (c >= count) return;
+  }
+  const int slot = ps >> S, h = ps & ((1 << S) - 1);
+  const int a = a0 + slot;
+  const u32 p = pr.p[a];
+  const Tw32* __restrict__ tab = tabs + (((i64)a << S) + h) * A32_N;
+  u32* __restrict__ g = rows + ((((c * nslots + slot)) << S) + h) * A32_N;
+  a32_stage_tbl(tbl, tab, tid);
+  u32 r[32];
+  if constexpr (DIGITS && S >= 3) {
+    const u32* __restrict__ srow = reinterpret_cast<const u32*>(ds.parts) + ((((c * 4 + slot)) << S) + h) * (i64)A32_N;
+#pragma unroll
+    for (int k = 0; k < 32; ++k) r[k] = srow[k * A32_T + tid];
+  } else if (DIGITS) {
+    const i64 poly = div32((u32)c, (u32)ds.nd, ds.nd_inv);
+    const u32 d = (u32)c - (u32)poly * (u32)ds.nd;
+    const u32 bit = d * (u32)ds.digit_bits, g0 = bit >> 5, sh = bit & 31;
+    const u32 nbyt = (u32)ds.digit_bits >> 3, bo = sh >> 3;
+    u32 sel = 0;
+#pragma unroll
+    for (u32 i = 0; i < 4; ++i) sel |= (i < nbyt ? bo + i : 0x0cu) << (8 * i);
+    const u32* __restrict__ p32 = reinterpret_cast<const u32*>(ds.parts);
+    constexpr u32 ES = WM ? 4 : 8;
+    auto wrow = [&](u32 g) -> const u32* { return WM ? p32 + (poly * (2 * ds.nl) + g) * (i64)ds.n_src : p32 + (((poly * ds.nl + (g >> 1)) * (i64)ds.n_src) << 1) + (g & 1); };
+    const u32* __restrict__ w0 = wrow(g0);
+    const bool two = (sh + ds.digit_bits > 32) && (int)((g0 + 1) >> 1) < ds.nl;
+    const u32 ns = ds.n_src;
+    static_assert(!(DIGITS && S >= 2 && !PAD), "digit rows of 2^16 and longer exist for the padded linear-convolution rings only");
+    if (S == 0 || (PAD && S == 1)) {
+      if (two) {
+        const u32* __restrict__ w1 = wrow(g0 + 1);
+#pragma unroll
+        for (int k = 0; k < 32; ++k) {
+          const u32 el = k * A32_T + tid, e = ES * (PAD ? (el < ns ? el : 0u) : el);
+          const u32 v = __builtin_amdgcn_perm(ld32(w1, e), ld32(w0, e), sel);
+          r[k] = (!PAD || el < ns) ? v : 0u;
+        }
+      } else {
+#pragma unroll
+        for (int k = 0; k < 32; ++k) {
+          const u32 el = k * A32_T + tid;
+          const u32 v = __builtin_amdgcn_perm(0u, ld32(w0, ES * (PAD ? (el < ns ? el : 0u) : el)), sel);
+          r[k] = (!PAD || el < ns) ? v : 0u;
+        }
+      }
+    } else {
+      const Tw32 hw = S == 2 ? hd.head1[a][h >> 1] : hd.head[a];
+      const u32* __restrict__ w1 = wrow(g0 + 1);
+      auto body = [&](auto TWO) {
+        constexpr bool two_c = decltype(TWO)::value;
+        constexpr int NB = two_c ? 8 : 16;
+        auto dig = [&](u32 el) -> u32 {
+          const u32 e = ES * (PAD ? (el < ns ? el : 0u) : el);
+          const u32 v = two_c ? __builtin_amdgcn_perm(ld32(w1, e), ld32(w0, e), sel) : __builtin_amdgcn_perm(0u, ld32(w0, e), sel);
+          return (!PAD || el < ns) ? v : 0u;
+        };
+#pragma unroll
+        for (int k0 = 0; k0 < 32; k0 += NB) {
+          u32 y[NB];
+#pragma unroll
+          for (int k = 0; k < NB; ++k) y[k] = dig((k0 + k) * A32_T + tid + A32_N);
+#pragma unroll
+          for (int k = 0; k < NB; ++k) r[k0 + k] = mul_lazy32(y[k], hw, p);
+        }
+#pragma unroll
+        for (int k0 = 0; k0 < 32; k0 += NB) {
+          u32 x[NB];
+#pragma unroll
+          for (int k = 0; k < NB; ++k) x[k] = dig((k0 + k) * A32_T + tid);
+#pragma unroll
+          for (int k = 0; k < NB; ++k) r[k0 + k] = (h & 1) == 0 ? x[k] + r[k0 + k] : x[k] + 2 * p - r[k0 + k];
+        }
+      };
+      if (two) body(std::true_type{}); else body(std::false_type{});
+    }
+  } else {
+#pragma unroll
+    for (int k = 0; k < 32; ++k) r[k] = g[k * A32_T + tid];
+  }
+#pragma unroll
+  for (int s = A32_FWD_FIRST; s < 5; ++s) {
+    const int h = 16 >> s;
+#pragma unroll
+    for (int b = 0; b < 16; ++b) {
+      const int k = a32_bfly_k(b, h);
+      if (DIGITS && (S == 0 || (PAD && S == 1)) && NEGW && s == 0) a32_ct<NEGW, true, true>(r[k], r[k + h], tab[(1 << s) + (k >> (5 - s))], p);
+      else a32_ct<NEGW, true>(r[k], r[k + h], tab[(1 << s) + (k >> (5 - s))], p, PB == 29 ? a32_fwd_step29(s) : 1);
+    }
+  }
+  const u32 kq = tid >> 4, lo = tid & 15;
+  const bool upper = kq >= A32_HR;
+#pragma unroll
+  for (int k = 0; k < 16; ++k) lds[k * A32_P + a32_f(tid)] = r[k];
+  __syncthreads();
+  u32 t[16];
+#pragma unroll
+  for (int k = 0; k < 16; ++k) t[k] = r[16 + k];
+  if (!upper) {
+#pragma unroll
+    for (int k2 = 0; k2 < 32; ++k2) r[k2] = lds[kq * A32_P + a32_f(k2 * 16 + lo)];
+  }
+  __syncthreads();
+#pragma unroll
+  for (int k = 0; k < 16; ++k) lds[k * A32_P + a32_f(tid)] = t[k];
+  __syncthreads();
+  if (upper) {
+#pragma unroll
+    for (int k2 = 0; k2 < 32; ++k2) r[k2] = lds[(kq - A32_HR) * A32_P + a32_f(k2 * 16 + lo)];
+  }
+#pragma unroll
+  for (int u = 0; u < 5; ++u) {
+    const int h = 16 >> u;
+    Tw32 tb[16];
+#pragma unroll
+    for (int i = 0; i < (1 << u); ++i) tb[i] = tbl[a32_tbl_idx(u, kq, i)];
+#pragma unroll
+    for (int b = 0; b < 16; ++b) {
+      const int k2 = a32_bfly_k(b, h);
+      a32_ct<NEGW>(r[k2], r[k2 + h], tb[k2 >> (5 - u)], p, PB == 29 ? a32_fwd_step29(5 + u) : 1);
+    }
+  }
+  const u32 wv = __builtin_amdgcn_readfirstlane(tid >> 6), sub = kq & 3;
+  __syncthreads();
+  u32* __restrict__ row = lds + (2 * wv + (sub & 1)) * A32_P;
+#pragma unroll
+  for (int hh = 0; hh < 2; ++hh) {
+    if ((int)(sub >> 1) == hh) {
+#pragma unroll
+      for (int k2 = 0; k2 < 32; ++k2) row[a32_f(k2 * 16 + lo)] = r[k2];
+    }
+    __builtin_amdgcn_wave_barrier();
+    if ((int)(sub >> 1) == hh) {
+#pragma unroll
+      for (int i = 0; i < 32; ++i) r[i] = row[lo * 36 + i];
+    }
+    __builtin_amdgcn_wave_barrier();
+  }
+  const u32 tcb = (tid & 63) * 16;
+  const __amdgpu_buffer_rsrc_t tabr = __builtin_amdgcn_make_buffer_rsrc(const_cast<Tw32*>(tab), 0, A32_N * 8, 0x00020000);
+#define A32_TABC tabr
+#pragma unroll
+  for (int v = 0; v < 4; ++v) {
+    const int h = 8 >> v;
+    Tw32 tc[2][8];
+    A32_LOAD_TC(tc, A32_TABC, v, tid, wv, tcb);
+#pragma unroll
+    for (int gq = 0; gq < 2; ++gq) {
+#pragma unroll
+      for (int b = 0; b < 8; ++b) {
+        const int x = a32_bfly_k(b, h);
+        a32_ct<NEGW>(r[gq * 16 + x], r[gq * 16 + x + h], tc[gq][x >> (4 - v)], p, PB == 29 ? a32_fwd_step29(10 + v) : 1);
+      }
+    }
+  }
+  const u32 lane = tid & 63;
+  u32* __restrict__ stage = lds + 2 * wv * A32_P;
+#pragma unroll
+  for (int hh = 0; hh < 2; ++hh) {
+    __builtin_amdgcn_wave_barrier();
+    if ((int)(sub >> 1) == hh) {
+      u32* w = stage + ((sub & 1) * 8 + (lo >> 1)) * 72 + (lo & 1) * 36;
+#pragma unroll
+      for (int i = 0; i < 32; ++i) {
+        u32 v = r[i];
+        if (!DIGITS) {
+          const u32 twop = 2 * p;
+          if (PB == 29) v = min(v, v - 2 * twop);
+          v = v >= twop ? v - twop : v; v = v >= p ? v - p : v;
+        }
+        w[i] = v;
+      }
+    }
+    __builtin_amdgcn_wave_barrier();
+    const u32 pos = lane < 32 ? lane : lane + 4;
+    i64 cnt_s = count, c_s = c, base_s = 0;
+    if (DIGITS && ds.sub_units) {
+      const i64 sub = div32((u32)c, ds.sub_units, ds.sub_inv), rest = count - sub * ds.sub_units;
+      c_s = c - sub * ds.sub_units;
+      cnt_s = rest < (i64)ds.sub_units ? rest : (i64)ds.sub_units;
+      base_s = sub * ds.sub_units * (((i64)4 << (A32_LOGN - 6 + S)) * 64);
+    }
+    const i64 stride = DIGITS ? cnt_s * 64 : 64;
+    u32* __restrict__ sp = (DIGITS ? rows + base_s + ((((i64)a << (A32_LOGN - 6 + S)) + ((i64)h << (A32_LOGN - 6)) + (32 * wv + 16 * hh)) * cnt_s + c_s) * 64 : g + (32 * wv + 16 * hh) * 64);
+    const u32 lboff = lane * 4;
+#pragma unroll
+    for (int t = 0; t < 16; ++t) {
+      const u32 v = stage[t * 72 + pos];
+      st32(sp, lboff, v);
+      sp += stride;
+    }
+  }
+}
diff --git a/include/fhesi_hip.h b/include/fhesi_hip.h
--- a/include/fhesi_hip.h
+++ b/include/fhesi_hip.h
@@ -90,6 +90,7 @@
 int fhesi_ksk_form(const fhesi_ksk* k, int32_t* form, int32_t* rows, int32_t* limb_bits);
 int fhesi_ksk_key_bits(const fhesi_ksk* k, int32_t* centred, int32_t* key_bits);
 
+int fhesi_mfma_i8_tile(fhesi_ctx* ctx, const int8_t* a, const int8_t* b, int32_t* c);
 int fhesi_selftest_aux32(fhesi_ctx* c);
 
 int fhesi_ct_mul_relin_batch(fhesi_ctx* ctx, const fhesi_ksk* k, int32_t logQ, uint64_t p, int32_t decomp_bytes,
```
